# Kim-Dongjun/Soft-Truncation

Hardware: AMD Instinct MI355X
Metric: training images/sec (DDPM++ CIFAR-10 32x32) (higher is better)
Workload: dtype f32; 1 GPU; DDPM++ (VP) CIFAR-10 32x32, configs/vp/CIFAR10/ddpmpp_nll_st.py (BASELINE configs[1]); per_gpu_batch=128, global_batch=128, parallelism=dp1

## Files before the change

soft-truncation_amd/csrc/conv.hip:

```cpp
#include "igemm.h"
#include "stk_fp16.h"
#include "stk_fp16_train.h"

namespace {

using igemm::Cfg;
using igemm::MnMajor;
using igemm::keep_if;
using igemm::strip_row;

typedef __attribute__((address_space(1))) float gfloat;

struct ConvP {
  const float* x1; const float* x2; int C1, C2;
  const float* w; int w_layout;
  const float* bias; const float* temb; int temb_stride; const float* res; float inv_div; int use_div;
  float* y;
  const float* dy; float* dx1; float* dx2; float beta1, beta2, alpha;
  float* part; long part_stride;
  int N, H, W, Cin, Cout, OH, OW, KH, KW, stride, pad, sshift;
  int HW, OHW, taps;
  int ohw_shift, ow_shift;
};


template <int B, int KC, int LD>
struct RowChunk {
  static constexpr int PERQ = KC / 4, PASSES = B / 64, PER = PASSES * PERQ;
  static_assert(KC % 4 == 0 && B % 64 == 0 && PER <= 32, "bad RowChunk tile");
  const float* rowp[PASSES];
  unsigned rowbits;
  unsigned okm;
  int q, tid, Ktot;
  __device__ __forceinline__ void init(const float* base, long ld, int row0, int R, int Ktot_, int tid_) {
    tid = tid_; q = tid & 3; Ktot = Ktot_; rowbits = 0; okm = 0;
#pragma unroll
    for (int ps = 0; ps < PASSES; ++ps) {
      const int row = row0 + (tid >> 2) + 64 * ps;
      const bool ok = row < R;
      rowbits |= (ok ? 1u : 0u) << ps;
      rowp[ps] = base + (ok ? (long)row * ld : 0);
    }
  }
  __device__ __forceinline__ void load(int k0, float (&r)[PER]) {
    const int kb = k0 + q * PERQ;
    const bool kin = kb + PERQ <= Ktot;
    const int ko = kin ? kb : 0;
    okm = 0;
#pragma unroll
    for (int ps = 0; ps < PASSES; ++ps) {
      const float* s = rowp[ps] + ko;
#pragma unroll
      for (int j = 0; j < PERQ; ++j) r[ps * PERQ + j] = s[j];
      okm |= ((kin && ((rowbits >> ps) & 1u)) ? ((1u << PERQ) - 1u) : 0u) << (ps * PERQ);
    }
  }
  __device__ __forceinline__ void store(const float (&r)[PER], float* t) {
    if (okm == (PER == 32 ? 0xffffffffu : (1u << PER) - 1u)) {
#pragma unroll
      for (int ps = 0; ps < PASSES; ++ps)
#pragma unroll
        for (int j = 0; j < PERQ; ++j) t[(q * PERQ + j) * LD + (tid >> 2) + 64 * ps] = r[ps * PERQ + j];
    } else {
#pragma unroll
      for (int ps = 0; ps < PASSES; ++ps)
#pragma unroll
        for (int j = 0; j < PERQ; ++j)
          t[(q * PERQ + j) * LD + (tid >> 2) + 64 * ps] = keep_if(r[ps * PERQ + j], okm, ps * PERQ + j);
    }
  }
};

template <int B, int KC, int LD>
struct MnStrided {
  using Mp = MnMajor<B, KC>;
  static constexpr int PER = Mp::PER;
  const float* pm; long sk; int kg, tid, Ktot; bool ok;
  unsigned okm;
  __device__ __forceinline__ void init(const float* base, long smn, long sk_, int o0, int lim, int Ktot_, int tid_) {
    tid = tid_; sk = sk_; Ktot = Ktot_; okm = 0;
    const int mn = o0 + Mp::mn(tid);
    ok = mn < lim;
    pm = base + (ok ? (long)mn * smn : 0);
    kg = Mp::kgroup(tid) * PER;
  }
  __device__ __forceinline__ void load(int k0, float (&r)[PER]) {
    okm = 0;
#pragma unroll
    for (int i = 0; i < PER; ++i) {
      const int k = k0 + kg + i;
      const bool v = ok && k < Ktot;
      r[i] = pm[v ? (long)k * sk : 0];
      okm |= (v ? 1u : 0u) << i;
    }
  }
  __device__ __forceinline__ void store(const float (&r)[PER], float* t) {
#pragma unroll
    for (int i = 0; i < PER; ++i) t[(kg + i) * LD + Mp::mn(tid)] = keep_if(r[i], okm, i);
  }
};

template <class C>
struct AFwdK {
  RowChunk<C::BM, C::KC, C::LDA> rc;
  __device__ void init(const ConvP& p, int m0, int tid, int) { rc.init(p.w, (long)p.Cin * p.taps, m0, p.Cout, p.Cin * p.taps, tid); }
  __device__ void load(const ConvP&, int k0, float (&r)[C::NA]) { rc.load(k0, r); }
  __device__ void store(const float (&r)[C::NA], float* t) { rc.store(r, t); }
};
template <class C>
struct AFwdGen {
  MnStrided<C::BM, C::KC, C::LDA> ms;
  __device__ void init(const ConvP& p, int m0, int tid, int) { ms.init(p.w, (long)p.Cin * p.taps, 1, m0, p.Cout, p.Cin * p.taps, tid); }
  __device__ void load(const ConvP&, int k0, float (&r)[C::NA]) { ms.load(k0, r); }
  __device__ void store(const float (&r)[C::NA], float* t) { ms.store(r, t); }
};
template <class C>
struct AFwdNin {
  MnStrided<C::BM, C::KC, C::LDA> ms;
  __device__ void init(const ConvP& p, int m0, int tid, int) { ms.init(p.w, 1, p.Cout, m0, p.Cout, p.Cin, tid); }
  __device__ void load(const ConvP&, int k0, float (&r)[C::NA]) { ms.load(k0, r); }
  __device__ void store(const float (&r)[C::NA], float* t) { ms.store(r, t); }
};
template <class C>
struct ADgradNin {
  RowChunk<C::BM, C::KC, C::LDA> rc;
  __device__ void init(const ConvP& p, int m0, int tid, int) { rc.init(p.w, p.Cout, m0, p.Cin, p.Cout, tid); }
  __device__ void load(const ConvP&, int k0, float (&r)[C::NA]) { rc.load(k0, r); }
  __device__ void store(const float (&r)[C::NA], float* t) { rc.store(r, t); }
};
template <class C>
struct ADgradNinGen {
  MnStrided<C::BM, C::KC, C::LDA> ms;
  __device__ void init(const ConvP& p, int m0, int tid, int) { ms.init(p.w, p.Cout, 1, m0, p.Cin, p.Cout, tid); }
  __device__ void load(const ConvP&, int k0, float (&r)[C::NA]) { ms.load(k0, r); }
  __device__ void store(const float (&r)[C::NA], float* t) { ms.store(r, t); }
};
template <class C>
struct ADgrad1 {
  MnStrided<C::BM, C::KC, C::LDA> ms;
  __device__ void init(const ConvP& p, int m0, int tid, int) { ms.init(p.w, 1, p.Cin, m0, p.Cin, p.Cout, tid); }
  __device__ void load(const ConvP&, int k0, float (&r)[C::NA]) { ms.load(k0, r); }
  __device__ void store(const float (&r)[C::NA], float* t) { ms.store(r, t); }
};
template <class C>
struct ADgrad9 {
  static_assert(C::KC == 36, "3x3 chunks are 4 channels x 9 taps");
  static constexpr int PASSES = C::BM / 64;
  int m0, tid; unsigned okp;
  __device__ void init(const ConvP&, int m0_, int tid_, int) { m0 = m0_; tid = tid_; okp = 0; }
  __device__ void load(const ConvP& p, int k0, float (&r)[C::NA]) {
    const int co = k0 / 9 + (tid & 3);
    okp = 0;
#pragma unroll
    for (int ps = 0; ps < PASSES; ++ps) {
      const int m = m0 + (tid >> 2) + 64 * ps;
// ... 78 lines not shown
    cig = __builtin_amdgcn_readfirstlane(Mp::kgroup(tid) * (Mp::PER / TAPS));
    mask = 0; okm = 0; tb = 0; yp = 0; xp = 0;
    if (n < p.N * p.HW) {
      const int b = n / p.HW, hw = n - b * p.HW;
      const int y = hw / p.W, x = hw - y * p.W;
      yp = y + p.pad; xp = x + p.pad;
      const int KW = TAPS == 9 ? 3 : 1;
      const int sm = p.stride - 1;
#pragma unroll
      for (int t = 0; t < TAPS; ++t) {
        const int ty = yp - t / KW, tx = xp - t % KW;
        if (ty >= 0 && tx >= 0 && !(ty & sm) && !(tx & sm) && (ty >> p.sshift) < p.OH && (tx >> p.sshift) < p.OW)
          mask |= 1u << t;
      }
      tb = b * p.Cout * p.OHW;
    }
  }
  __device__ void load(const ConvP& p, int k0, float (&r)[C::NB]) {
    const int co0 = k0 / TAPS + cig;
    const int KW = TAPS == 9 ? 3 : 1;
    okm = 0;
#pragma unroll
    for (int c = 0; c < NCH; ++c) {
      const int co = co0 + c;
      const unsigned cm = co < p.Cout ? mask : 0u;
      const int cb = tb + co * p.OHW;
      okm |= cm << (c * TAPS);
#pragma unroll
      for (int t = 0; t < TAPS; ++t) {
        const int off = cb + ((yp - t / KW) >> p.sshift) * p.OW + ((xp - t % KW) >> p.sshift);
        r[c * TAPS + t] = p.dy[((cm >> t) & 1u) ? off : 0];
      }
    }
  }
  __device__ void store(const float (&r)[C::NB], float* t) {
    const int kg = Mp::kgroup(tid) * Mp::PER, mn = Mp::mn(tid);
#pragma unroll
    for (int i = 0; i < C::NB; ++i) t[(kg + i) * C::LDB + mn] = keep_if(r[i], okm, i);
  }
};

__device__ __forceinline__ void split_pixel(const ConvP& p, int k, int& b, int& ohw) {
  if (p.ohw_shift >= 0) { b = k >> p.ohw_shift; ohw = k & (p.OHW - 1); }
  else { b = k / p.OHW; ohw = k - b * p.OHW; }
}
__device__ __forceinline__ void split_row(const ConvP& p, int ohw, int& oy, int& ox) {
  if (p.ow_shift >= 0) { oy = ohw >> p.ow_shift; ox = ohw & (p.OW - 1); }
  else { oy = ohw / p.OW; ox = ohw - oy * p.OW; }
}

template <class C>
struct AWgrad {
  static_assert(C::KC == 32 && C::NA <= 32, "wgrad uses 32-pixel chunks");
  int roff[C::NA];
  int tid; unsigned okrows, okm;
  __device__ void init(const ConvP& p, int m0, int tid_, int) {
    tid = tid_; okm = 0; okrows = 0;
#pragma unroll
    for (int i = 0; i < C::NA; ++i) {
      const int m = m0 + (tid >> 5) + 8 * i;
      okrows |= (m < p.Cout ? 1u : 0u) << i;
      roff[i] = min(m, p.Cout - 1) * p.OHW;
    }
  }
  __device__ void load(const ConvP& p, int k0, float (&r)[C::NA]) {
    const int k = k0 + (tid & 31);
    const bool kv = k < p.N * p.OHW;
    int b, ohw;
    split_pixel(p, kv ? k : 0, b, ohw);
    const int base = b * p.Cout * p.OHW + ohw;
    okm = kv ? okrows : 0u;
#pragma unroll
    for (int i = 0; i < C::NA; ++i) r[i] = p.dy[base + roff[i]];
  }
  __device__ void store(const float (&r)[C::NA], float* t) {
#pragma unroll
    for (int i = 0; i < C::NA; ++i) t[(tid & 31) * C::LDA + (tid >> 5) + 8 * i] = keep_if(r[i], okm, i);
  }
};
template <class C, bool DUAL>
struct BWgrad {
  static_assert(C::KC == 32 && C::NB <= 32, "wgrad uses 32-pixel chunks");
  int roff[C::NB];
  int tid, kh, kw; unsigned okrows, okm, first;
  __device__ void init(const ConvP& p, int n0, int tid_, int zb) {
    tid = tid_; okm = 0; okrows = 0; first = 0;
    kh = zb / p.KW; kw = zb - kh * p.KW;
#pragma unroll
    for (int i = 0; i < C::NB; ++i) {
      const int ci = min(n0 + (tid >> 5) + 8 * i, p.Cin - 1);
      okrows |= (n0 + (tid >> 5) + 8 * i < p.Cin ? 1u : 0u) << i;
      const bool f = !DUAL || ci < p.C1;
      first |= (f ? 1u : 0u) << i;
      roff[i] = (f ? ci : ci - p.C1) * p.HW;
    }
  }
  __device__ void load(const ConvP& p, int k0, float (&r)[C::NB]) {
    const int k = k0 + (tid & 31);
    bool kv = k < p.N * p.OHW;
    int b, ohw, oy, ox;
    split_pixel(p, kv ? k : 0, b, ohw);
    split_row(p, ohw, oy, ox);
    const int iy = oy * p.stride + kh - p.pad, ix = ox * p.stride + kw - p.pad;
    kv = kv && iy >= 0 && iy < p.H && ix >= 0 && ix < p.W;
    const int pix = kv ? iy * p.W + ix : 0;
    const int b1 = b * p.C1 * p.HW + pix, b2 = b * p.C2 * p.HW + pix;
    okm = kv ? okrows : 0u;
#pragma unroll
    for (int i = 0; i < C::NB; ++i) {
      if (DUAL) {
        const bool f = (first >> i) & 1u;
        const uintptr_t tensor = f ? (uintptr_t)p.x1 : (uintptr_t)p.x2;
        r[i] = ((const gfloat*)tensor)[(f ? b1 : b2) + roff[i]];
      } else {
        r[i] = p.x1[b1 + roff[i]];
      }
    }
  }
  __device__ void store(const float (&r)[C::NB], float* t) {
#pragma unroll
    for (int i = 0; i < C::NB; ++i) t[(tid & 31) * C::LDB + (tid >> 5) + 8 * i] = keep_if(r[i], okm, i);
  }
};

struct EpFwd {
  int b; int col_off;
  static constexpr int TEMB_IMGS = 9;
  float rb; float rt[5]; int m0 = 0, b0 = 0, nimg = 0, tb = 0;
  const float* sb = nullptr; const float* stm = nullptr;
  __device__ void preload(const ConvP& p, int m0_, int n0, int tn, int M, int Nn, int tid) {
    m0 = m0_; sb = nullptr; stm = nullptr;
    b0 = n0 / p.OHW;
    nimg = min(n0 + tn - 1, Nn - 1) / p.OHW - b0 + 1;
    rb = (p.bias && tid < 128 && m0 + tid < M) ? p.bias[m0 + tid] : 0.f;
#pragma unroll
    for (int k = 0; k < 5; ++k) {
      const int idx = tid + 256 * k, img = idx >> 7, r = idx & 127;
      rt[k] = (p.temb && nimg <= TEMB_IMGS && img < nimg && m0 + r < M) ? p.temb[(long)(b0 + img) * p.temb_stride + m0 + r] : 0.f;
    }
  }
  __device__ void stage(unsigned char* lds, int tid) {
    __syncthreads();
    float* s = reinterpret_cast<float*>(lds);
    if (tid < 128) s[tid] = rb;
#pragma unroll
    for (int k = 0; k < 5; ++k) {
      const int idx = tid + 256 * k;
      if (idx < TEMB_IMGS * 128) s[128 + idx] = rt[k];
    }
    __syncthreads();
    sb = s; stm = s + 128;
  }
  __device__ void init(const ConvP&, int, int) {}
  __device__ void finish(const ConvP&, unsigned char*, int) {}
  __device__ void col(const ConvP& p, int n) {
    b = n / p.OHW;
    col_off = b * p.Cout * p.OHW + (n - b * p.OHW);
    tb = (b - b0) * 128;
  }
  __device__ void strip(const ConvP& p, int mbase, int M, bool nok, int, const floatx16& acc) {
    if (sb && (!p.temb || nimg <= TEMB_IMGS)) {
      const int ml = mbase - m0;
      float rv[16]; int idx[16];
#pragma unroll
      for (int e = 0; e < 16; ++e) {
        const int m = mbase + strip_row(e);
        const bool ok = nok && m < M;
        idx[e] = ok ? col_off + m * p.OHW : -1;
        rv[e] = (p.res && ok) ? p.res[idx[e]] : 0.f;
      }
#pragma unroll
      for (int g = 0; g < 4; ++g) {
        const float4 bb = *reinterpret_cast<const float4*>(sb + ml + 8 * g);
        const float4 tt = *reinterpret_cast<const float4*>(stm + tb + ml + 8 * g);
        const float bv[4] = {bb.x, bb.y, bb.z, bb.w}, tv[4] = {tt.x, tt.y, tt.z, tt.w};
#pragma unroll
        for (int u = 0; u < 4; ++u) {
          float v = acc[4 * g + u];
          if (p.bias) v += bv[u];
          if (p.temb) v += tv[u];
          if (p.res) v += rv[4 * g + u];
          if (p.use_div) v *= p.inv_div;
          if (idx[4 * g + u] >= 0) p.y[idx[4 * g + u]] = v;
        }
      }
      return;
    }
#pragma unroll
    for (int g = 0; g < 4; ++g) {
      float bv[4], tv[4], rv[4];
      int idx[4]; bool ok[4];
#pragma unroll
      for (int u = 0; u < 4; ++u) {
        const int m = mbase + strip_row(4 * g + u);
        ok[u] = nok && m < M;
        idx[u] = ok[u] ? col_off + m * p.OHW : 0;
        const int ms = ok[u] ? m : 0;
        bv[u] = p.bias ? p.bias[ms] : 0.f;
        tv[u] = p.temb ? p.temb[ok[u] ? (long)b * p.temb_stride + m : 0] : 0.f;
        rv[u] = p.res ? p.res[idx[u]] : 0.f;
      }
#pragma unroll
      for (int u = 0; u < 4; ++u) {
        float v = acc[4 * g + u];
        if (p.bias) v += bv[u];
        if (p.temb) v += tv[u];
        if (p.res) v += rv[u];
        if (p.use_div) v *= p.inv_div;
        if (ok[u]) p.y[idx[u]] = v;
      }
    }
  }
};
struct EpDgrad {
  int b, hw;
  __device__ void preload(const ConvP&, int, int, int, int, int, int) {}
  __device__ void stage(unsigned char*, int) {}
  __device__ void init(const ConvP&, int, int) {}
  __device__ void col(const ConvP& p, int n) { b = n / p.HW; hw = n - b * p.HW; }
  __device__ void strip(const ConvP& p, int mbase, int M, bool nok, int, const floatx16& acc) {
    const bool acc1 = p.beta1 != 0.f, acc2 = p.beta2 != 0.f;
#pragma unroll
    for (int e0 = 0; e0 < 16; e0 += 4) {
      float* d[4]; float old[4];
#pragma unroll
      for (int u = 0; u < 4; ++u) {
        const int m = mbase + strip_row(e0 + u);
        float* q = nullptr;
        if (nok && m < M) {
          if (m < p.C1) { if (p.dx1) q = p.dx1 + ((long)b * p.C1 + m) * p.HW + hw; }
          else if (p.dx2) q = p.dx2 + ((long)b * p.C2 + (m - p.C1)) * p.HW + hw;
        }
        d[u] = q;
        old[u] = 0.f;
        if (acc1 || acc2) {
          const float beta = m < p.C1 ? p.beta1 : p.beta2;
          if (q && beta != 0.f) old[u] = beta * *q;
        }
      }
#pragma unroll
      for (int u = 0; u < 4; ++u)
        if (d[u]) *d[u] = old[u] + p.alpha * acc[e0 + u];
    }
  }
  __device__ void finish(const ConvP&, unsigned char*, int) {}
};
struct EpWgrad {
  float* slab; int tap;
  __device__ void init(const ConvP& p, int zb, int zs) { slab = p.part + (long)zs * p.part_stride; tap = zb; }
  __device__ void col(const ConvP&, int) {}
  __device__ void strip(const ConvP& p, int mbase, int M, bool nok, int n, const floatx16& acc) {
#pragma unroll
    for (int e = 0; e < 16; ++e) {
      const int m = mbase + strip_row(e);
      if (nok && m < M) {
        slab[((long)tap * p.Cout + m) * p.Cin + n] = acc[e];
      }
    }
  }
};

struct EpSlab {
  float* slab; int Nn;
  __device__ void preload(const ConvP&, int, int, int, int, int, int) {}
  __device__ void stage(unsigned char*, int) {}
  __device__ void init(const ConvP& p, int, int zs) { slab = p.part + (long)zs * p.part_stride; Nn = p.N * p.HW; }
  __device__ void finish(const ConvP&, unsigned char*, int) {}
  __device__ void col(const ConvP&, int) {}
  __device__ void strip(const ConvP&, int mbase, int M, bool nok, int n, const floatx16& acc) {
#pragma unroll
    for (int e = 0; e < 16; ++e) {
      const int m = mbase + strip_row(e);
      if (nok && m < M) slab[(long)m * Nn + n] = acc[e];
    }
  }
};
template <class EP> struct OneProduct : EP {};
template <class EP> struct is_x1 { static constexpr bool value = false; };
template <class EP> struct is_x1<OneProduct<EP>> { static constexpr bool value = true; };
template <int VEC>
__global__ __launch_bounds__(256) void slab_fwd_kernel(ConvP p, int splits, int M, int Nn) {
  const long total = (long)M * Nn / VEC, gstride = (long)gridDim.x * 256;
  for (long iv = (long)blockIdx.x * 256 + threadIdx.x; iv < total; iv += gstride) {
    const long i = iv * VEC;
    const int m = (int)(i / Nn), n = (int)(i - (long)m * Nn);
    float v[VEC];
#pragma unroll
    for (int u = 0; u < VEC; ++u) v[u] = 0.f;
    for (int z = 0; z < splits; ++z) {
      const float* q = p.part + (long)z * p.part_stride + i;
      if constexpr (VEC == 4) {
        const float4 t = *reinterpret_cast<const float4*>(q);
        v[0] += t.x; v[1] += t.y; v[2] += t.z; v[3] += t.w;
      } else {
        v[0] += q[0];
      }
    }
    const int b = n / p.OHW;
    const long idx = ((long)b * p.Cout + m) * p.OHW + (n - b * p.OHW);
    float r[VEC];
#pragma unroll
    for (int u = 0; u < VEC; ++u) r[u] = 0.f;
    if (p.res) {
      if constexpr (VEC == 4) { const float4 t = *reinterpret_cast<const float4*>(p.res + idx); r[0] = t.x; r[1] = t.y; r[2] = t.z; r[3] = t.w; }
      else r[0] = p.res[idx];
    }
#pragma unroll
    for (int u = 0; u < VEC; ++u) {
      float w = v[u];
      if (p.bias) w += p.bias[m];
      if (p.temb) w += p.temb[(long)b * p.temb_stride + m];
      if (p.res) w += r[u];
      if (p.use_div) w *= p.inv_div;
      v[u] = w;
    }
    if constexpr (VEC == 4) *reinterpret_cast<float4*>(p.y + idx) = make_float4(v[0], v[1], v[2], v[3]);
    else p.y[idx] = v[0];
  }
}
template <int VEC>
__global__ __launch_bounds__(256) void slab_dgrad_kernel(ConvP p, int splits, int M, int Nn) {
  const long total = (long)M * Nn / VEC, gstride = (long)gridDim.x * 256;
  for (long iv = (long)blockIdx.x * 256 + threadIdx.x; iv < total; iv += gstride) {
    const long i = iv * VEC;
    const int m = (int)(i / Nn), n = (int)(i - (long)m * Nn);
    float v[VEC];
#pragma unroll
    for (int u = 0; u < VEC; ++u) v[u] = 0.f;
    for (int z = 0; z < splits; ++z) {
      const float* q = p.part + (long)z * p.part_stride + i;
      if constexpr (VEC == 4) {
        const float4 t = *reinterpret_cast<const float4*>(q);
        v[0] += t.x; v[1] += t.y; v[2] += t.z; v[3] += t.w;
      } else {
        v[0] += q[0];
      }
    }
    const int b = n / p.HW, hw = n - b * p.HW;
    float* d; float beta;
    if (m < p.C1) { d = p.dx1 ? p.dx1 + ((long)b * p.C1 + m) * p.HW + hw : nullptr; beta = p.beta1; }
    else { d = p.dx2 ? p.dx2 + ((long)b * p.C2 + (m - p.C1)) * p.HW + hw : nullptr; beta = p.beta2; }
    if (!d) continue;
    if constexpr (VEC == 4) {
      float4 o = make_float4(0.f, 0.f, 0.f, 0.f);
      if (beta != 0.f) { const float4 t = *reinterpret_cast<const float4*>(d); o = make_float4(beta * t.x, beta * t.y, beta * t.z, beta * t.w); }
      *reinterpret_cast<float4*>(d) = make_float4(o.x + p.alpha * v[0], o.y + p.alpha * v[1], o.z + p.alpha * v[2], o.w + p.alpha * v[3]);
    } else {
      *d = (beta != 0.f ? beta * *d : 0.f) + p.alpha * v[0];
    }
  }
}
inline void launch_slab_sum(const ConvP& p, int splits, int M, long Ng, int dgrad, hipStream_t s) {
  const bool al = stk_aligned16(p.part) && p.part_stride % 4 == 0 &&
                  (dgrad ? (p.HW % 4 == 0 && (!p.dx1 || stk_aligned16(p.dx1)) && (!p.dx2 || stk_aligned16(p.dx2)))
                         : (p.OHW % 4 == 0 && stk_aligned16(p.y) && (!p.res || stk_aligned16(p.res))));
  if (al && Ng % 4 == 0) {
    const dim3 rgrid((unsigned)stk_ew_grid((long)M * Ng / 4));
    if (dgrad) hipLaunchKernelGGL(slab_dgrad_kernel<4>, rgrid, dim3(256), 0, s, p, splits, M, (int)Ng);
    else hipLaunchKernelGGL(slab_fwd_kernel<4>, rgrid, dim3(256), 0, s, p, splits, M, (int)Ng);
  } else {
    const dim3 rgrid((unsigned)stk_ew_grid((long)M * Ng));
    if (dgrad) hipLaunchKernelGGL(slab_dgrad_kernel<1>, rgrid, dim3(256), 0, s, p, splits, M, (int)Ng);
    else hipLaunchKernelGGL(slab_fwd_kernel<1>, rgrid, dim3(256), 0, s, p, splits, M, (int)Ng);
  }
}

#include "conv_thin.h"
#include "conv_x2.h"
#include "conv_pl.h"
#include "conv_x2d.h"
#include "conv_x2w.h"

__device__ __forceinline__ long splitk_dst(long j, int layout, long CC, int Cout, int Cin, int taps) {
  if (layout == 0) {
    const int tap = (int)(j / CC);
    return (j - (long)tap * CC) * taps + tap;
  }
  const int co = (int)(j / Cin), ci = (int)(j - (long)co * Cin);
  return (long)ci * Cout + co;
}
__global__ __launch_bounds__(256) void splitk_reduce_kernel(const float* __restrict__ part, float* __restrict__ dw,
                                                            long n, int splits, long stride, float alpha, int layout,
                                                            int Cout, int Cin, int taps) {
  const long gstride = (long)gridDim.x * 256;
  const long CC = (long)Cout * Cin;
  const long n4 = ((n | stride) & 3) == 0 ? n / 4 : 0;
  for (long v = (long)blockIdx.x * 256 + threadIdx.x; v < n4; v += gstride) {
    const float4* src = reinterpret_cast<const float4*>(part) + v;
    float4 acc = {0.f, 0.f, 0.f, 0.f};
#pragma unroll 8
    for (int z = 0; z < splits; ++z) {
      const float4 t = src[(long)z * (stride / 4)];
      acc.x += t.x; acc.y += t.y; acc.z += t.z; acc.w += t.w;
    }
    const float a4[4] = {acc.x, acc.y, acc.z, acc.w};
#pragma unroll
    for (int e = 0; e < 4; ++e) dw[splitk_dst(4 * v + e, layout, CC, Cout, Cin, taps)] += alpha * a4[e];
  }
  for (long j = 4 * n4 + (long)blockIdx.x * 256 + threadIdx.x; j < n; j += gstride) {
    float sum = 0.f;
    for (int z = 0; z < splits; ++z) sum += part[(long)z * stride + j];
    dw[splitk_dst(j, layout, CC, Cout, Cin, taps)] += alpha * sum;
  }
}

__global__ __launch_bounds__(256) void splitk_reduce9_kernel(const float* __restrict__ part, float* __restrict__ dw, long CC,
                                                             int splits, long stride, float alpha) {
  __shared__ float s[256 * 9];
  const long q0 = (long)blockIdx.x * 256;
  const long q = q0 + threadIdx.x;
  const bool live = q < CC;
  float acc[9];
#pragma unroll
  for (int t = 0; t < 9; ++t) acc[t] = 0.f;
  const float* src = part + (live ? q : 0);
  int z = 0;
  for (; z + 4 <= splits; z += 4) {
    float v[4][9];
#pragma unroll
    for (int u = 0; u < 4; ++u)
// ... 159 lines not shown
  __device__ void load(const GemmP&, int k0, float (&r)[C::NB]) {
    if (K_CONTIG) rc.load(k0, r); else ms.load(k0, r);
  }
  __device__ void store(const float (&r)[C::NB], float* t) {
    if (K_CONTIG) rc.store(r, t); else ms.store(r, t);
  }
};
struct EpGemm {
  float* base;
  __device__ void init(const GemmP& p, int zb, int) { base = p.C + (long)zb * p.scb; }
  __device__ void col(const GemmP&, int) {}
  __device__ void strip(const GemmP& p, int mbase, int M, bool nok, int n, const floatx16& acc) {
    float old[16];
    if (p.beta != 0.f) {
#pragma unroll
      for (int e = 0; e < 16; ++e) {
        const int m = mbase + strip_row(e);
        const bool ok = nok && m < M;
        old[e] = base[ok ? (long)m * p.scm + (long)n * p.scn : 0];
      }
    }
#pragma unroll
    for (int e = 0; e < 16; ++e) {
      const int m = mbase + strip_row(e);
      if (nok && m < M) {
        float v = p.alpha * acc[e];
        if (p.bias_mode == 1) v += p.bias[m];
        else if (p.bias_mode == 2) v += p.bias[n];
        base[(long)m * p.scm + (long)n * p.scn] = (p.beta != 0.f ? p.beta * old[e] : 0.f) + v;
      }
    }
  }
};

inline bool use_big_tile(int M, long N, int z) {
  const long t = (long)stk_cdiv(M, 128) * stk_cdiv(N, 128) * z;
  return M >= 96 && N >= 96 && t >= 192;
}

template <class C, class P, class AL, class BL, class EP>
int launch(const P& p, int M, long Nl, int K, int k_per_split, int splits, int batch, hipStream_t s,
           bool flat = false) {
  if (Nl > 0x7fffffffL) return STK_EUNSUPPORTED;
  const int N = (int)Nl;
  const int tm = stk_cdiv(M, C::BM), tn = stk_cdiv(N, C::BN);
  if (flat) {
    const long total = (long)tm * tn * splits * batch;
    if (total > 0x7fffffffL) return STK_EUNSUPPORTED;
    hipLaunchKernelGGL((igemm::kernel<C, P, AL, BL, EP>), dim3((unsigned)total), dim3(256), 0, s, p, M, N, K, tm, tn,
                       k_per_split, batch);
  } else {
    dim3 grid((unsigned)(tm * tn), (unsigned)splits, (unsigned)batch);
    hipLaunchKernelGGL((igemm::kernel<C, P, AL, BL, EP>), grid, dim3(256), 0, s, p, M, N, K, tm, tn, k_per_split, 0);
  }
  STK_CHECK_LAUNCH();
  return STK_OK;
}

inline int fill_common(ConvP& p, int N, int H, int W, int C1, int C2, int Cout, int OH, int OW, int KH, int KW,
                       int stride, int pad) {
  if (N <= 0 || H <= 0 || W <= 0 || C1 <= 0 || C2 < 0 || Cout <= 0 || OH <= 0 || OW <= 0) return STK_EINVAL;
  if (!((KH == 3 && KW == 3) || (KH == 1 && KW == 1))) return STK_EUNSUPPORTED;
  if (stride != 1 && stride != 2) return STK_EUNSUPPORTED;
  const long lim = 0x7fffffffL;
  if ((long)N * (C1 > C2 ? C1 : C2) * H * W >= lim || (long)N * Cout * OH * OW >= lim) return STK_EUNSUPPORTED;
  p.N = N; p.H = H; p.W = W; p.C1 = C1; p.C2 = C2; p.Cin = C1 + C2; p.Cout = Cout; p.OH = OH; p.OW = OW;
  p.KH = KH; p.KW = KW; p.stride = stride; p.pad = pad; p.sshift = stride == 2 ? 1 : 0;
  p.HW = H * W; p.OHW = OH * OW; p.taps = KH * KW;
  p.ohw_shift = -1; p.ow_shift = -1;
  for (int sft = 0; sft < 31; ++sft) {
    if ((1 << sft) == p.OHW) p.ohw_shift = sft;
    if ((1 << sft) == p.OW) p.ow_shift = sft;
  }
  return STK_OK;
}

struct SplitPlan { int ok; int splits; int chunks_per_split; long slab; int t64; int gps; };
inline SplitPlan split_plan(const ConvP& p, int Kc, int S1, int S2, int M, long Ng) {
  SplitPlan r = {0, 1, 0, 0, 0, 0};
  const long big = (long)p.N * p.HW * 4 * (S1 > S2 ? S1 : S2);
  const bool geom = (p.taps == 9 && p.pad == 1) || (p.taps == 1 && p.pad == 0);
  if (!(big < 0x7fffffffL && geom && p.stride == 1 && p.OH == p.H && p.OW == p.W && Kc % 32 == 0 &&
        (S2 == 0 || S1 % 32 == 0) && M >= 96 && Ng <= 0x7fffffffL))
    return r;
  const long tiles = (long)stk_cdiv(M, 128) * stk_cdiv(Ng, 128);
  const int nch = p.taps * (Kc / 32);
  r.chunks_per_split = nch;
  if (tiles >= 192) { r.ok = 1; return r; }
  static const long target = [] { const char* e = getenv("STK_KSPLIT_WGS"); return e && atol(e) > 0 ? atol(e) : 512L; }();
  constexpr long minch = 12;
  long splits = target / tiles;
  const long mc = p.taps == 9 ? minch : (minch < 6 ? minch : 6);
  if (splits > nch / mc) splits = nch / mc;
  if ((tiles < 16 && p.taps != 9) || splits < 2) return r;
  r.chunks_per_split = (int)((nch + splits - 1) / splits);
  r.splits = (nch + r.chunks_per_split - 1) / r.chunks_per_split;
  r.slab = (long)M * Ng;
  r.ok = 1;
  return r;
}
inline SplitPlan fwd_split_plan(const ConvP& p) { return split_plan(p, p.Cin, p.C1, p.C2, p.Cout, (long)p.N * p.OHW); }
inline SplitPlan dgrad_split_plan(const ConvP& p) { return split_plan(p, p.Cout, p.Cout, 0, p.Cin, (long)p.N * p.HW); }
struct SplitWs { long xpart, part, bytes; };
inline long align256(long v) { return (v + 255) & ~255L; }
inline SplitWs split_ws(const SplitPlan& r, int M, int Kc, int taps) {
  SplitWs o;
  o.xpart = align256(x2::wp_bytes(M, Kc, taps));
  o.part = align256(o.xpart + 2L * x2::NPART * 4);
  o.bytes = r.ok ? 255 + o.part + (r.splits > 1 ? r.splits * r.slab * 4 : 0) : 0;
  return o;
}
inline void split_weight_strides(const ConvP& p, int dgrad, long& sm, long& sk) {
  if (p.w_layout == 0) { sm = dgrad ? p.taps : (long)p.Cin * p.taps; sk = dgrad ? (long)p.Cin * p.taps : p.taps; }
  else { sm = dgrad ? p.Cout : 1; sk = dgrad ? 1 : p.Cout; }
}
inline SplitPlan x1_plan(const SplitPlan& r, int nch1) {
  SplitPlan r1 = r;
  r1.chunks_per_split = (nch1 + r.splits - 1) / r.splits;
  r1.splits = (nch1 + r1.chunks_per_split - 1) / r1.chunks_per_split;
  return r1;
}

struct SplitGemm {
  ConvP p; x2::Src q; int M, Ng, tm, tn, nch, chunks_per_split; const float* xpart; int nx;
  bool dual, planes, halo; dim3 grid; hipStream_t s;
};
template <class E, int TAPS>
void split_gemm_taps(const SplitGemm& g) {
  constexpr bool X1 = is_x1<E>::value;
  if (!g.planes) {
    using A1 = std::conditional_t<X1, x2::ActLoader16<false, TAPS>, x2::ActLoader<false, TAPS>>;
    using A2 = std::conditional_t<X1, x2::ActLoader16<true, TAPS>, x2::ActLoader<true, TAPS>>;
    if (g.dual) hipLaunchKernelGGL((x2::gemm_kernel<A2, E>), g.grid, dim3(256), 0, g.s, g.p, g.q, g.M, g.Ng, g.tm, g.tn, g.nch,
                                   g.chunks_per_split, g.xpart, g.nx);
    else hipLaunchKernelGGL((x2::gemm_kernel<A1, E>), g.grid, dim3(256), 0, g.s, g.p, g.q, g.M, g.Ng, g.tm, g.tn, g.nch,
                            g.chunks_per_split, g.xpart, g.nx);
  } else if (g.halo) {
    if (g.p.W == 64)
      hipLaunchKernelGGL((x2d::gemm_halo_kernel<64, E, 1>), g.grid, dim3(256), 0, g.s, g.p, g.q, g.M, g.Ng, g.tm, g.tn, g.nch / 9, g.xpart, g.nx);
    else if (g.p.W == 32)
      hipLaunchKernelGGL((x2d::gemm_halo_kernel<32, E, 1>), g.grid, dim3(256), 0, g.s, g.p, g.q, g.M, g.Ng, g.tm, g.tn, g.nch / 9, g.xpart, g.nx);
    else
      hipLaunchKernelGGL((x2d::gemm_halo_kernel<16, E, 1>), g.grid, dim3(256), 0, g.s, g.p, g.q, g.M, g.Ng, g.tm, g.tn, g.nch / 9, g.xpart, g.nx);
  } else {
    hipLaunchKernelGGL((x2d::gemm_kernel<TAPS, 128, E>), g.grid, dim3(256), 0, g.s, g.p, g.q, g.M, g.Ng, g.tm, g.tn, g.nch,
                       g.chunks_per_split, g.xpart, g.nx);
  }
}
template <class E>
void split_gemm(const SplitGemm& g) {
  if (g.p.taps == 9) split_gemm_taps<E, 9>(g);
  else split_gemm_taps<E, 1>(g);
}

template <class EP>
int launch_split(ConvP p, const SplitPlan& r0, const float* s1, int S1, const float* s2, int S2, int M, long Ng, int dgrad,
                 void* ws, hipStream_t s, const void* wp_ready, float* amax, const void* planes, const float* planes_amax,
                 bool amax_valid, bool x1) {
  x2::Src q;
  q.s1 = s1; q.s2 = S2 > 0 ? s2 : s1; q.S1 = S1; q.S2 = S2; q.Kc = S1 + S2; q.Mpad = x2::pad128(M); q.taps = p.taps;
  q.pl = static_cast<const unsigned char*>(planes); q.pl_stride = planes ? pl::plane_bytes(p.N, S1, p.HW) : 0;
  const SplitWs lay = split_ws(r0, M, q.Kc, p.taps);
  unsigned char* base = reinterpret_cast<unsigned char*>(((uintptr_t)ws + 255) & ~(uintptr_t)255);
  float* xpart = reinterpret_cast<float*>(base + lay.xpart);
  p.part = reinterpret_cast<float*>(base + lay.part);
  p.part_stride = r0.slab;
  if (amax) xpart = amax + (dgrad ? 2 * x2::NPART : 0);
  if (planes) {
    xpart = const_cast<float*>(planes_amax);
  } else if (!(amax_valid && amax)) {
    hipLaunchKernelGGL(x2::amax_partial_kernel, dim3(x2::NPART), dim3(x2::AMAX_THREADS), 0, s, s1, (long)p.N * S1 * p.HW, xpart);
    if (S2 > 0)
      hipLaunchKernelGGL(x2::amax_partial_kernel, dim3(x2::NPART), dim3(x2::AMAX_THREADS), 0, s, s2, (long)p.N * S2 * p.HW,
                         xpart + x2::NPART);
    STK_CHECK_LAUNCH();
  }
  if (wp_ready) {
    q.wp = static_cast<const unsigned short*>(wp_ready);
  } else {
    x2::WprepDesc one = {};
    one.w = p.w; one.wp = base; one.M = M; one.Kc = q.Kc; one.Mpad = q.Mpad;
    one.taps = p.taps; one.flip = dgrad;
    split_weight_strides(p, dgrad, one.sm, one.sk);
    hipLaunchKernelGGL(x2::wamax_kernel, dim3(x2::WPART, 1), dim3(256), 0, s, nullptr, one);
    hipLaunchKernelGGL(x2::wprep_kernel, dim3((unsigned)stk_cdiv((long)q.Mpad * q.Kc, 256L)), dim3(256), 0, s, nullptr, one);
    STK_CHECK_LAUNCH();
    q.wp = reinterpret_cast<const unsigned short*>(base);
  }
  const int nch = planes && x1 ? p.taps * ((q.Kc / x2::KC + 1) / 2) : p.taps * (q.Kc / x2::KC);
  const SplitPlan r = planes && x1 ? x1_plan(r0, nch) : r0;
  SplitGemm g = {p, q, M, (int)Ng, q.Mpad / 128, stk_cdiv((int)Ng, 128), nch, r.chunks_per_split, xpart,
                 S2 > 0 ? 2 * x2::NPART : x2::NPART, S2 > 0, planes != nullptr, planes && x2d::halo_ok(p, p.taps, r0.splits),
                 dim3(), s};
  g.grid = dim3((unsigned)(g.tm * g.tn * r.splits));
  if (r0.splits == 1) {
    if (x1) split_gemm<OneProduct<EP>>(g);
    else split_gemm<EP>(g);
    STK_CHECK_LAUNCH();
    return STK_OK;
  }
  if (x1) split_gemm<OneProduct<EpSlab>>(g);
  else split_gemm<EpSlab>(g);
  STK_CHECK_LAUNCH();
  launch_slab_sum(p, r.splits, M, Ng, dgrad, s);
  STK_CHECK_LAUNCH();
  return STK_OK;
}

struct SplitWgradPlan { int ok; int splits; int chunks_per_split; long slab; int rows3; };
inline SplitWgradPlan split_wgrad_plan(int C1, int C2, int N, int Cout, int H, int W, int OH, int OW, int KH, int KW,
                                       int stride, int pad) {
  SplitWgradPlan q = {0, 0, 0, 0, 0};
  const int Cin = C1 + C2;
  const long K = (long)N * H * W;
  const int cmax = Cout > C1 ? (Cout > C2 ? Cout : C2) : (C1 > C2 ? C1 : C2);
  if (K * cmax * 4 >= 0x7fffffffL || (C2 > 0 && C1 % 32)) return q;
  const bool pow2 = (W & (W - 1)) == 0 && ((H * W) & (H * W - 1)) == 0;
  const bool geom = (KH == 3 && KW == 3 && pad == 1) || (KH == 1 && KW == 1 && pad == 0);
  if (!geom || stride != 1 || OH != H || OW != W || !pow2 || W < 4 || H * W < 16 || Cin < 64 || Cout < 64 ||
      K > 0x7fffffffL || K % 32)
    return q;
  const int taps = KH * KW;
  q.rows3 = (taps == 9 && W >= 8 && (C2 == 0 || C1 % 16 == 0)) ? 1 : 0;
  const long tiles = q.rows3 ? 3L * stk_cdiv(Cout, 128) * stk_cdiv(Cin, 64)
                             : (long)taps * stk_cdiv(Cout, 128) * stk_cdiv(Cin, 128);
  if (taps == 1 && tiles < 2) return q;
  const long chunks = K / 32;
  constexpr long w1_wgs = 256;
  long splits = (taps == 1 && tiles < 6 ? w1_wgs : 512) / tiles;
  if (splits > chunks / 8) splits = chunks / 8;
  if (splits < 1) splits = 1;
  q.chunks_per_split = (int)((chunks + splits - 1) / splits);
  q.splits = (int)((chunks + q.chunks_per_split - 1) / q.chunks_per_split);
  q.slab = (long)Cout * Cin * taps;
  q.ok = 1;
  return q;
}
template <int FORM>
void launch_x2w(const x2w::Args& a, int W, dim3 grid, hipStream_t s) {
  const dim3 block(256 * (FORM & 15));
  if (W >= 32) hipLaunchKernelGGL((x2w::wgrad_kernel<32, FORM>), grid, block, 0, s, a);
  else if (W == 16) hipLaunchKernelGGL((x2w::wgrad_kernel<16, FORM>), grid, block, 0, s, a);
  else if (W == 8) hipLaunchKernelGGL((x2w::wgrad_kernel<8, FORM>), grid, block, 0, s, a);
  else hipLaunchKernelGGL((x2w::wgrad_kernel<4, FORM>), grid, block, 0, s, a);
}
struct WgemmArgs {
  ConvP p; int tm, tn, nch, chunks_per_split; const float* dyp; const float* xp; int nx; dim3 grid; hipStream_t s;
};
template <bool X1, class BL>
void launch_wgemm_rows(const WgemmArgs& g) {
  using AL = std::conditional_t<X1, x2::RowsU16<false, false>, x2::RowsU<false, false>>;
  using E = std::conditional_t<X1, OneProduct<EpWgrad>, EpWgrad>;
  hipLaunchKernelGGL((x2::wgemm_kernel<AL, BL, E, !X1>), g.grid, dim3(256), 0, g.s, g.p, g.p.Cout, g.p.Cin, g.tm, g.tn, g.nch,
                     g.chunks_per_split, g.p.taps, g.dyp, g.xp, g.nx);
}
template <bool X1, bool DUAL>
void launch_wgemm_src(const WgemmArgs& g) {
  if (g.p.taps == 1)
    launch_wgemm_rows<X1, std::conditional_t<X1, x2::RowsU16<true, DUAL>, x2::RowsU<true, DUAL>>>(g);
  else if (g.p.W >= 16)
    launch_wgemm_rows<X1, std::conditional_t<X1, x2::RowsB16<DUAL, 16>, x2::RowsB<DUAL, 16>>>(g);
  else if (g.p.W == 8)
    launch_wgemm_rows<X1, std::conditional_t<X1, x2::RowsB16<DUAL, 8>, x2::RowsB<DUAL, 8>>>(g);
  else
    launch_wgemm_rows<X1, std::conditional_t<X1, x2::RowsB16<DUAL, 4>, x2::RowsB<DUAL, 4>>>(g);
}
template <bool X1>
void launch_wgemm(const WgemmArgs& g) {
  if (g.p.C2 > 0) launch_wgemm_src<X1, true>(g);
  else launch_wgemm_src<X1, false>(g);
}

struct WgradPlan { int big; int splits; int k_per_split; long slab; int mode9; };
inline int wgrad9_cols(int OH, int OW, int KH, int KW) {
  if (KH != 3 || KW != 3 || ((long)OH * OW) % 32 != 0) return 0;
  if (OW % 32 == 0) return 32;
  if (OW == 16 || OW == 8) return OW;
  return 0;
}
inline WgradPlan wgrad_plan(int Cin, int N, int Cout, int OH, int OW, int KH, int KW, bool allow9 = true) {
  WgradPlan q;
  q.mode9 = allow9 ? wgrad9_cols(OH, OW, KH, KW) : 0;
  if (q.mode9) {
    const long K = (long)N * OH * OW;
    const long tiles = (long)stk_cdiv(Cout, 128) * stk_cdiv(Cin, 32);
    const long chunks = K / 32;
    long splits = 256 / tiles;
    if (splits > chunks / 16) splits = chunks / 16;
    if (splits < 1) splits = 1;
    const long cps = (chunks + splits - 1) / splits;
    q.big = 1;
    q.k_per_split = (int)(cps * 32);
    q.splits = (int)((K + q.k_per_split - 1) / q.k_per_split);
    q.slab = (long)Cout * Cin * 9;
    return q;
  }
  const int taps = KH * KW;
  const long K = (long)N * OH * OW;
  const long tiles128 = (long)stk_cdiv(Cout, 128) * stk_cdiv(Cin, 128) * taps;
  q.big = (Cout >= 96 && Cin >= 96 && tiles128 >= 9) ? 1 : 0;
  const int T = q.big ? 128 : 64;
  const long tiles = (long)stk_cdiv(Cout, T) * stk_cdiv(Cin, T) * taps;
  const long chunks = (K + 31) / 32;
  long splits = (512 + tiles - 1) / tiles;
  if (splits > chunks / 16) splits = chunks / 16;
  if (splits < 1) splits = 1;
  const long cps = (chunks + splits - 1) / splits;
  q.k_per_split = (int)(cps * 32);
  q.splits = (int)((K + q.k_per_split - 1) / q.k_per_split);
  q.slab = (long)Cout * Cin * taps;
  return q;
}

}

extern "C" {

static int fwd_impl(const float* x1, int C1, const float* x2, int C2, const float* w, int w_layout,
                    const float* bias, const float* temb, int temb_stride, const float* res, float out_div,
                    float* y, int N, int H, int W, int Cout, int OH, int OW, int KH, int KW, int stride, int pad,
                    const void* wp, float* amax, void* ws, long ws_bytes, void* stream, bool x_rec_valid, bool f16x1) {
  if (!x1 || !w || !y || (C2 > 0 && !x2) || out_div == 0.f || (w_layout != 0 && w_layout != 1) ||
      (w_layout == 1 && (KH != 1 || KW != 1)))
    return STK_EINVAL;
  ConvP p = {};
  int rc = fill_common(p, N, H, W, C1, C2, Cout, OH, OW, KH, KW, stride, pad);
  if (rc) return rc;
  p.x1 = x1; p.x2 = C2 > 0 ? x2 : x1; p.w = w; p.w_layout = w_layout; p.bias = bias; p.temb = temb;
  p.temb_stride = temb_stride; p.res = res; p.inv_div = 1.f / out_div; p.use_div = out_div != 1.f; p.y = y;
  const int K = p.Cin * p.taps;
  const long Ng = (long)N * p.OHW;
  const bool big = use_big_tile(Cout, Ng, 1);
  hipStream_t s = (hipStream_t)stream;
  if (thin::geometry_ok(p) && Ng <= 0x7fffffffL) {
    const unsigned nblk = (unsigned)stk_cdiv(Ng, 256L);
    if (C2 == 0 && p.Cin <= 4) {
      thin::Args a = {x1, w, (long)p.Cin * p.taps, (long)p.taps, 0, p.Cin, Cout, p.taps, 0};
      const dim3 grid(nblk, (unsigned)stk_cdiv(Cout, thin::OB));
      if (p.taps == 9) hipLaunchKernelGGL((thin::thin_in_kernel<9>), grid, dim3(256), 0, s, p, a);
      else hipLaunchKernelGGL((thin::thin_in_kernel<1>), grid, dim3(256), 0, s, p, a);
      STK_CHECK_LAUNCH();
      return STK_OK;
    }
    if (Cout <= 4) {
      const unsigned nblk64 = (unsigned)stk_cdiv(Ng, 64L);
      if (p.taps == 9) hipLaunchKernelGGL((thin::thin_out_kernel<9>), dim3(nblk64), dim3(256), 0, s, p, Cout);
      else hipLaunchKernelGGL((thin::thin_out_kernel<1>), dim3(nblk64), dim3(256), 0, s, p, Cout);
      STK_CHECK_LAUNCH();
// ... 174 lines not shown
    if (p.taps == 9) {
      if (a.CT == 3) hipLaunchKernelGGL((thin::thin_wgrad_kernel<9, 3>), grid, dim3(256), 0, s, p, a);
      else hipLaunchKernelGGL((thin::thin_wgrad_kernel<9, 4>), grid, dim3(256), 0, s, p, a);
    } else {
      hipLaunchKernelGGL((thin::thin_wgrad_kernel<1, 4>), grid, dim3(256), 0, s, p, a);
    }
    STK_CHECK_LAUNCH();
    hipLaunchKernelGGL(splitk_reduce_kernel, dim3(stk_ew_grid((a.slab + 3) / 4)), dim3(256), 0, s, ws, dw, a.slab, S, a.slab,
                       alpha, 0, Cout, p.Cin, p.taps);
    STK_CHECK_LAUNCH();
    return STK_OK;
  }
  const SplitWgradPlan xq = split_wgrad_plan(C1, C2, N, Cout, H, W, OH, OW, KH, KW, stride, pad);
  if (xq.ok && ws_bytes >= (long)xq.splits * xq.slab * 4 + 256 + 3L * x2::NPART * 4) {
    p.x1 = x1; p.x2 = C2 > 0 ? x2 : x1; p.dy = dy; p.w_layout = w_layout; p.part = ws; p.part_stride = xq.slab;
    float* parts = reinterpret_cast<float*>(((uintptr_t)(ws + (long)xq.splits * xq.slab) + 255) & ~(uintptr_t)255);
    const dim3 ab(x2::NPART), at(x2::AMAX_THREADS);
    const float* dyp = parts;
    const float* xp = parts + x2::NPART;
    if (amax && (have & 2)) dyp = amax + 2 * x2::NPART;
    else hipLaunchKernelGGL(x2::amax_partial_kernel, ab, at, 0, s, dy, (long)N * Cout * p.OHW, parts);
    if (amax && (have & 1)) {
      xp = amax;
    } else {
      hipLaunchKernelGGL(x2::amax_partial_kernel, ab, at, 0, s, x1, (long)N * C1 * p.HW, parts + x2::NPART);
      if (C2 > 0) hipLaunchKernelGGL(x2::amax_partial_kernel, ab, at, 0, s, x2, (long)N * C2 * p.HW, parts + 2 * x2::NPART);
    }
    const int nx = C2 > 0 ? 2 * x2::NPART : x2::NPART;
    const int tm = stk_cdiv(Cout, 128), nch = (int)((long)N * p.HW / 32);
    if (xq.rows3 && !f16x1) {
      const int tn64 = stk_cdiv(p.Cin, 64);
      const dim3 grid3((unsigned)(3 * tm * tn64 * xq.splits));
      if (C2 > 0) hipLaunchKernelGGL((x2::wgrad3_kernel<true>), grid3, dim3(256), 0, s, p, tm, tn64, nch, xq.chunks_per_split,
                                     dyp, xp, nx);
      else hipLaunchKernelGGL((x2::wgrad3_kernel<false>), grid3, dim3(256), 0, s, p, tm, tn64, nch, xq.chunks_per_split,
                              dyp, xp, nx);
    } else {
      const int tn = stk_cdiv(p.Cin, 128);
      const WgemmArgs g = {p, tm, tn, nch, xq.chunks_per_split, dyp, xp, nx, dim3((unsigned)(p.taps * tm * tn * xq.splits)), s};
      if (f16x1) launch_wgemm<true>(g);
      else launch_wgemm<false>(g);
    }
    STK_CHECK_LAUNCH();
    hipLaunchKernelGGL(splitk_reduce_kernel, dim3(stk_ew_grid((xq.slab + 3) / 4)), dim3(256), 0, s, ws, dw, xq.slab, xq.splits,
                       xq.slab, alpha, w_layout, Cout, p.Cin, p.taps);
    STK_CHECK_LAUNCH();
    return STK_OK;
  }
  const bool can9 = stride == 1 && pad == 1 && C2 == 0 && OH == H && OW == W && w_layout == 0;
  const WgradPlan q = wgrad_plan(p.Cin, N, Cout, OH, OW, KH, KW, can9);
  if (ws_bytes < (long)q.splits * q.slab * 4) return STK_EINVAL;
  p.x1 = x1; p.x2 = C2 > 0 ? x2 : x1; p.dy = dy; p.w_layout = w_layout; p.part = ws; p.part_stride = q.slab;
  const long Kl = (long)N * p.OHW;
  if (Kl > 0x7fffffffL) return STK_EUNSUPPORTED;
  const int K = (int)Kl;
  using CB = Cfg<128, 128, 32>; using CS = Cfg<64, 64, 32>;
  if (q.mode9) {
    const int tm = stk_cdiv(Cout, 128), tn = stk_cdiv(p.Cin, 32);
    const dim3 grid((unsigned)(tm * tn * q.splits));
    if (q.mode9 == 32) hipLaunchKernelGGL((wgrad9_kernel<32>), grid, dim3(256), 0, s, p, tm, tn, q.k_per_split);
    else if (q.mode9 == 16) hipLaunchKernelGGL((wgrad9_kernel<16>), grid, dim3(256), 0, s, p, tm, tn, q.k_per_split);
    else hipLaunchKernelGGL((wgrad9_kernel<8>), grid, dim3(256), 0, s, p, tm, tn, q.k_per_split);
    STK_CHECK_LAUNCH();
    rc = STK_OK;
  } else if (C2 > 0) {
    if (q.big) rc = launch<CB, ConvP, AWgrad<CB>, BWgrad<CB, true>, EpWgrad>(p, Cout, p.Cin, K, q.k_per_split, q.splits, p.taps, s, true);
    else rc = launch<CS, ConvP, AWgrad<CS>, BWgrad<CS, true>, EpWgrad>(p, Cout, p.Cin, K, q.k_per_split, q.splits, p.taps, s, true);
  } else {
    if (q.big) rc = launch<CB, ConvP, AWgrad<CB>, BWgrad<CB, false>, EpWgrad>(p, Cout, p.Cin, K, q.k_per_split, q.splits, p.taps, s, true);
    else rc = launch<CS, ConvP, AWgrad<CS>, BWgrad<CS, false>, EpWgrad>(p, Cout, p.Cin, K, q.k_per_split, q.splits, p.taps, s, true);
  }
  if (rc) return rc;
  hipLaunchKernelGGL(splitk_reduce_kernel, dim3(stk_ew_grid((q.slab + 3) / 4)), dim3(256), 0, s, ws, dw, q.slab, q.splits,
                     q.slab, alpha, w_layout, Cout, p.Cin, p.taps);
  STK_CHECK_LAUNCH();
  return STK_OK;
}

int stk_conv2d_wgrad_f32(const float* x1, int C1, const float* x2, int C2, const float* dy, float* dw, int w_layout,
                         float alpha, float* ws, long ws_bytes, int N, int H, int W, int Cout, int OH, int OW, int KH,
                         int KW, int stride, int pad, void* stream) {
  return stk_conv2d_wgrad_amax_f32(x1, C1, x2, C2, dy, dw, w_layout, alpha, ws, ws_bytes, N, H, W, Cout, OH, OW, KH, KW, stride,
                                   pad, nullptr, 0, stream);
}

int stk_conv2d_wgrad_amax_f32(const float* x1, int C1, const float* x2, int C2, const float* dy, float* dw, int w_layout,
                              float alpha, float* ws, long ws_bytes, int N, int H, int W, int Cout, int OH, int OW, int KH,
                              int KW, int stride, int pad, const float* amax, int have, void* stream) {
  return wgrad_amax_impl(x1, C1, x2, C2, dy, dw, w_layout, alpha, ws, ws_bytes, N, H, W, Cout, OH, OW, KH, KW, stride, pad, amax,
                         have, stream, false);
}

int stk_conv2d_wgrad_amax_f16x1(const float* x1, int C1, const float* x2, int C2, const float* dy, float* dw, int w_layout,
                                float alpha, float* ws, long ws_bytes, int N, int H, int W, int Cout, int OH, int OW, int KH,
                                int KW, int stride, int pad, const float* amax, int have, void* stream) {
  return wgrad_amax_impl(x1, C1, x2, C2, dy, dw, w_layout, alpha, ws, ws_bytes, N, H, W, Cout, OH, OW, KH, KW, stride, pad, amax,
                         have, stream, true);
}

long stk_planes_bytes(int N, int C, int HW) {
  if (N <= 0 || C <= 0 || HW <= 0) return 0;
  return 2 * pl::plane_bytes(N, C, HW);
}

int stk_amax_partial_f32(const float* x, long n, float* part, void* stream) {
  if (!x || !part || n <= 0) return STK_EINVAL;
  hipLaunchKernelGGL(x2::amax_partial_kernel, dim3(x2::NPART), dim3(x2::AMAX_THREADS), 0, (hipStream_t)stream, x, n, part);
  STK_CHECK_LAUNCH();
  return STK_OK;
}

int stk_split_planes_f32(const float* x, int N, int C, int HW, const float* amax, int namax, void* planes, void* stream) {
  if (!x || !amax || !planes || N <= 0 || C <= 0 || HW <= 0 || namax <= 0) return STK_EINVAL;
  if (2 * pl::plane_bytes(N, C, HW) >= 0x7fffffffL) return STK_EUNSUPPORTED;
  const long blocks = (long)N * ((C + 31) / 32) * stk_cdiv(HW, pl::SP_PIX);
  hipLaunchKernelGGL(pl::split_planes_kernel, dim3((unsigned)blocks), dim3(256), 0, (hipStream_t)stream, x, N, C, HW, amax,
                     namax, static_cast<unsigned char*>(planes), pl::plane_bytes(N, C, HW));
  STK_CHECK_LAUNCH();
  return STK_OK;
}

int stk_conv2d_pl_ok(int dir, int C1, int C2, int N, int H, int W, int Cout, int KH, int KW, int stride, int pad) {
  ConvP p = {};
  if (fill_common(p, N, H, W, C1, C2, Cout, H, W, KH, KW, stride, pad)) return 0;
  if (stride != 1 || pad != KH / 2) return 0;
  if (dir == 0) {
    if (C2 > 0 || p.Cin <= 4 || Cout <= 4) return 0;
    return fwd_split_plan(p).ok;
  }
  if (dir == 1) {
    if (Cout <= 4 || p.Cin <= 4) return 0;
    return dgrad_split_plan(p).ok;
  }
  return 0;
}

int stk_conv2d_pl_ksplit(int dir, int C1, int C2, int N, int H, int W, int Cout, int KH, int KW) {
  if (!stk_conv2d_pl_ok(dir, C1, C2, N, H, W, Cout, KH, KW, 1, KH / 2)) return 0;
  ConvP p = {};
  if (fill_common(p, N, H, W, C1, C2, Cout, H, W, KH, KW, 1, KH / 2)) return 0;
  return dir == 0 ? fwd_split_plan(p).splits : dgrad_split_plan(p).splits;
}

int stk_conv2d_pl_halo(int dir, int C1, int C2, int N, int H, int W, int Cout, int KH, int KW) {
  const int ks = stk_conv2d_pl_ksplit(dir, C1, C2, N, H, W, Cout, KH, KW);
  if (ks <= 0) return 0;
  ConvP p = {};
  if (fill_common(p, N, H, W, C1, C2, Cout, H, W, KH, KW, 1, KH / 2)) return 0;
  return x2d::halo_ok(p, p.taps, ks) ? x2d::halo_cols(W) : 0;
}

static int fwd_pl_impl(const void* xpl, const float* xamax, int C, const float* w, int w_layout, const float* bias,
                       const float* temb, int temb_stride, const float* res, float out_div, float* y, int N, int H,
                       int W, int Cout, int KH, int KW, const void* wp, void* ws, long ws_bytes, void* stream, bool f16x1) {
  if (!xpl || !xamax || !w || !y || out_div == 0.f || (w_layout != 0 && w_layout != 1) || (w_layout == 1 && KH != 1))
    return STK_EINVAL;
  if (!stk_conv2d_pl_ok(0, C, 0, N, H, W, Cout, KH, KW, 1, KH / 2)) return STK_EUNSUPPORTED;
  ConvP p = {};
  fill_common(p, N, H, W, C, 0, Cout, H, W, KH, KW, 1, KH / 2);
  p.w = w; p.w_layout = w_layout; p.bias = bias; p.temb = temb; p.temb_stride = temb_stride; p.res = res;
  p.inv_div = 1.f / out_div; p.use_div = out_div != 1.f; p.y = y;
  const long Ng = (long)N * p.HW;
  const SplitPlan xr = fwd_split_plan(p);
  if (!ws || ws_bytes < split_ws(xr, Cout, C, p.taps).bytes) return STK_EINVAL;
  return launch_split<EpFwd>(p, xr, nullptr, C, nullptr, 0, Cout, Ng, 0, ws, (hipStream_t)stream, wp, nullptr, xpl, xamax, false,
                             f16x1);
}

int stk_conv2d_fwd_pl_f32(const void* xpl, const float* xamax, int C, const float* w, int w_layout, const float* bias,
                          const float* temb, int temb_stride, const float* res, float out_div, float* y, int N, int H,
                          int W, int Cout, int KH, int KW, const void* wp, void* ws, long ws_bytes, void* stream) {
  return fwd_pl_impl(xpl, xamax, C, w, w_layout, bias, temb, temb_stride, res, out_div, y, N, H, W, Cout, KH, KW, wp, ws,
                     ws_bytes, stream, false);
}

int stk_conv2d_fwd_pl_f16x1(const void* xpl, const float* xamax, int C, const float* w, int w_layout, const float* bias,
                            const float* temb, int temb_stride, const float* res, float out_div, float* y, int N, int H,
                            int W, int Cout, int KH, int KW, const void* wp, void* ws, long ws_bytes, void* stream) {
  return fwd_pl_impl(xpl, xamax, C, w, w_layout, bias, temb, temb_stride, res, out_div, y, N, H, W, Cout, KH, KW, wp, ws,
                     ws_bytes, stream, true);
}

static int dgrad_pl_impl(const void* dypl, const float* dyamax, const float* w, int w_layout, float* dx1, int C1,
                         float beta1, float* dx2, int C2, float beta2, float alpha, int N, int H, int W, int Cout,
                         int KH, int KW, const void* wp, void* ws, long ws_bytes, void* stream, bool f16x1) {
  if (!dypl || !dyamax || !w || (!dx1 && !dx2) || (w_layout != 0 && w_layout != 1) || (w_layout == 1 && KH != 1))
    return STK_EINVAL;
  if (!stk_conv2d_pl_ok(1, C1, C2, N, H, W, Cout, KH, KW, 1, KH / 2)) return STK_EUNSUPPORTED;
  ConvP p = {};
  fill_common(p, N, H, W, C1, C2, Cout, H, W, KH, KW, 1, KH / 2);
  p.w = w; p.w_layout = w_layout; p.dx1 = dx1; p.dx2 = C2 > 0 ? dx2 : nullptr;
  p.beta1 = beta1; p.beta2 = beta2; p.alpha = alpha;
  const long Ng = (long)N * p.HW;
  const SplitPlan xr = dgrad_split_plan(p);
  if (!ws || ws_bytes < split_ws(xr, p.Cin, Cout, p.taps).bytes) return STK_EINVAL;
  return launch_split<EpDgrad>(p, xr, nullptr, Cout, nullptr, 0, p.Cin, Ng, 1, ws, (hipStream_t)stream, wp, nullptr, dypl, dyamax,
                               false, f16x1);
}

int stk_conv2d_dgrad_pl_f32(const void* dypl, const float* dyamax, const float* w, int w_layout, float* dx1, int C1,
                            float beta1, float* dx2, int C2, float beta2, float alpha, int N, int H, int W, int Cout,
                            int KH, int KW, const void* wp, void* ws, long ws_bytes, void* stream) {
  return dgrad_pl_impl(dypl, dyamax, w, w_layout, dx1, C1, beta1, dx2, C2, beta2, alpha, N, H, W, Cout, KH, KW, wp, ws, ws_bytes,
                       stream, false);
}

int stk_conv2d_dgrad_pl_f16x1(const void* dypl, const float* dyamax, const float* w, int w_layout, float* dx1, int C1,
                              float beta1, float* dx2, int C2, float beta2, float alpha, int N, int H, int W, int Cout,
                              int KH, int KW, const void* wp, void* ws, long ws_bytes, void* stream) {
  return dgrad_pl_impl(dypl, dyamax, w, w_layout, dx1, C1, beta1, dx2, C2, beta2, alpha, N, H, W, Cout, KH, KW, wp, ws, ws_bytes,
                       stream, true);
}

int stk_conv2d_wgrad_pl_ok(int N, int H, int W, int Cin, int Cout) { return x2w::plan(N, H, W, Cin, Cout).ok; }

long stk_conv2d_wgrad_pl_ws_bytes(int N, int H, int W, int Cin, int Cout) {
  long m = 0;
  for (int wgs : {0, 256, 512, 768, 1024}) {
    const x2w::Plan q = x2w::plan(N, H, W, Cin, Cout, wgs);
    if (q.ok && (long)q.splits * q.slab > m) m = (long)q.splits * q.slab;
  }
  return m ? m * 4 + 256 : 0;
}

static int wgrad_pl_impl(const void* xpl, const float* xrec, const void* dypl, const float* dyrec, float* dw, float alpha,
                         float* ws, long ws_bytes, int N, int H, int W, int Cin, int Cout, int wgs, void* stream, bool f16x1) {
  if (!xpl || !xrec || !dypl || !dyrec || !dw || !ws || wgs < 0 || wgs > 1024) return STK_EINVAL;
  const x2w::Plan q = x2w::plan(N, H, W, Cin, Cout, wgs);
  if (!q.ok) return STK_EUNSUPPORTED;
  if (ws_bytes < (long)q.splits * q.slab * 4) return STK_EINVAL;
  x2w::Args a = {};
  a.dypl = static_cast<const unsigned char*>(dypl); a.dyrec = dyrec; a.dy_ps = pl::plane_bytes(N, Cout, H * W);
  a.xpl = static_cast<const unsigned char*>(xpl); a.xrec = xrec; a.x_ps = pl::plane_bytes(N, Cin, H * W);
  if (2 * a.dy_ps >= 0x7fffffffL || 2 * a.x_ps >= 0x7fffffffL) return STK_EUNSUPPORTED;
  a.part = ws; a.part_stride = q.slab;
  a.N = N; a.H = H; a.W = W; a.HW = H * W; a.Cin = Cin; a.Cout = Cout; a.Cob = Cout / 32; a.Cib = Cin / 32;
  a.tiles_co = stk_cdiv(Cout, 128); a.tiles_ci = Cin / 32;
  a.nchunks_total = (int)((long)N * H * W / 32); a.chunks_per_split = q.chunks_per_split;
  hipStream_t s = (hipStream_t)stream;
  const dim3 grid((unsigned)(a.tiles_co * a.tiles_ci * q.splits));
  if (f16x1) {
    if (q.groups == 2) launch_x2w<2 | x2w::X1_FORM>(a, W, grid, s);
    else launch_x2w<1 | x2w::X1_FORM>(a, W, grid, s);
  } else if (q.groups == 2) {
    launch_x2w<2>(a, W, grid, s);
  } else {
    launch_x2w<1>(a, W, grid, s);
  }
  STK_CHECK_LAUNCH();
  if (q.splits <= 64)
    hipLaunchKernelGGL(splitk_reduce9_kernel, dim3((unsigned)stk_cdiv((long)Cout * Cin, 256L)), dim3(256), 0, s, ws, dw, (long)Cout * Cin,
                       q.splits, q.slab, alpha);
  else
    hipLaunchKernelGGL(splitk_reduce_kernel, dim3(stk_ew_grid((q.slab + 3) / 4)), dim3(256), 0, s, ws, dw, q.slab, q.splits,
                       q.slab, alpha, 0, Cout, Cin, 9);
  STK_CHECK_LAUNCH();
  return STK_OK;
}

int stk_conv2d_wgrad_pl_f32(const void* xpl, const float* xrec, const void* dypl, const float* dyrec, float* dw,
                            float alpha, float* ws, long ws_bytes, int N, int H, int W, int Cin, int Cout, void* stream) {
  return stk_conv2d_wgrad_pl_wgs_f32(xpl, xrec, dypl, dyrec, dw, alpha, ws, ws_bytes, N, H, W, Cin, Cout, 0, stream);
}

int stk_conv2d_wgrad_pl_wgs_f32(const void* xpl, const float* xrec, const void* dypl, const float* dyrec, float* dw,
                                float alpha, float* ws, long ws_bytes, int N, int H, int W, int Cin, int Cout, int wgs, void* stream) {
  return wgrad_pl_impl(xpl, xrec, dypl, dyrec, dw, alpha, ws, ws_bytes, N, H, W, Cin, Cout, wgs, stream, false);
}

int stk_conv2d_wgrad_pl_f16x1(const void* xpl, const float* xrec, const void* dypl, const float* dyrec, float* dw,
                              float alpha, float* ws, long ws_bytes, int N, int H, int W, int Cin, int Cout, void* stream) {
  return wgrad_pl_impl(xpl, xrec, dypl, dyrec, dw, alpha, ws, ws_bytes, N, H, W, Cin, Cout, 0, stream, true);
}

int stk_conv2d_wgrad_pl_wgs_f16x1(const void* xpl, const float* xrec, const void* dypl, const float* dyrec, float* dw,
                                  float alpha, float* ws, long ws_bytes, int N, int H, int W, int Cin, int Cout, int wgs,
                                  void* stream) {
  return wgrad_pl_impl(xpl, xrec, dypl, dyrec, dw, alpha, ws, ws_bytes, N, H, W, Cin, Cout, wgs, stream, true);
}

int stk_conv2d_variant(int dir, int C1, int C2, int N, int H, int W, int Cout, int OH, int OW, int KH, int KW,
                       int stride, int pad, int w_layout) {
  ConvP p = {};
  if (fill_common(p, N, H, W, C1, C2, Cout, OH, OW, KH, KW, stride, pad)) return -1;
  const int Cin = C1 + C2;
  p.w_layout = w_layout;
  if (dir == 0) {
    const long Ng = (long)N * p.OHW;
    if (thin::geometry_ok(p) && ((C2 == 0 && Cin <= 4) || Cout <= 4)) return 4;
    if (fwd_split_plan(p).ok) return 5;
    return use_big_tile(Cout, Ng, 1) && !(p.taps == 1 && w_layout == 0 && (Cin % 8)) ? 1 : 0;
  }
  if (dir == 1) {
    const long Ng = (long)N * p.HW;
    if (thin::geometry_ok(p) && Cout <= 4) return 4;
    if (dgrad_split_plan(p).ok) return 5;
    return use_big_tile(Cin, Ng, 1) && !(p.taps == 1 && w_layout == 1 && (Cout % 8)) ? 1 : 0;
  }
  if (thin::geometry_ok(p) && ((C2 == 0 && Cin <= 4) || Cout <= 4)) return 4;
  if (split_wgrad_plan(C1, C2, N, Cout, H, W, OH, OW, KH, KW, stride, pad).ok) return 5;
  const bool can9 = stride == 1 && pad == 1 && C2 == 0 && OH == H && OW == W && w_layout == 0;
  const WgradPlan q = wgrad_plan(Cin, N, Cout, OH, OW, KH, KW, can9);
  return q.mode9 ? 3 : q.big;
}

long stk_conv2d_wp_bytes(int dir, int C1, int C2, int N, int H, int W, int Cout, int KH, int KW, int stride, int pad) {
  if (dir != 0 && dir != 1) return 0;
  if (stk_conv2d_variant(dir, C1, C2, N, H, W, Cout, H, W, KH, KW, stride, pad, 0) != 5) return 0;
  const int Cin = C1 + C2;
  return dir == 0 ? x2::wp_bytes(Cout, Cin, KH * KW) : x2::wp_bytes(Cin, Cout, KH * KW);
}

long stk_conv2d_wp_desc(int dir, const float* w, int w_layout, int Cin, int Cout, int KH, int KW, void* wp,
                        StkWprepDesc* out) {
  if (!w || !wp || !out || (dir != 0 && dir != 1) || (w_layout != 0 && w_layout != 1) || Cin <= 0 || Cout <= 0 ||
      (KH * KW != 9 && KH * KW != 1) || (w_layout == 1 && KH * KW != 1) || ((uintptr_t)wp & 255))
    return STK_EINVAL;
  ConvP p = {};
  p.Cin = Cin; p.Cout = Cout; p.taps = KH * KW; p.w_layout = w_layout;
// ... 72 lines not shown
```

soft-truncation_amd/csrc/conv_x2d.h:

```cpp
#pragma once

namespace x2d {

using x2::KC;
typedef __attribute__((address_space(3))) void lds_void;

template <int TN>
struct Geo {
  static constexpr int A_PLANE = 128 * 64, A_BYTES = 2 * A_PLANE;
  static constexpr int B_PLANE = TN * 64, B_BYTES = 2 * B_PLANE;
  static constexpr int LDS = A_BYTES + B_BYTES;
  static constexpr int NJ = TN / 64;
  static constexpr int BBLK = TN / 64;
};

__device__ __forceinline__ void dma16(__amdgpu_buffer_rsrc_t rs, unsigned char* dst, unsigned voff, unsigned soff) {
  __builtin_amdgcn_raw_ptr_buffer_load_lds(rs, (lds_void*)dst, 16, (int)voff, (int)soff, 0, 0);
}

template <int TAPS, int TN, class EP, int NBUF = 1, int ABL = 0>
__global__ __launch_bounds__(256, 2) void gemm_kernel(ConvP p, x2::Src q, int M, int Nn, int tiles_m, int tiles_n,
                                                      int nchunks_total, int chunks_per_split,
                                                      const float* __restrict__ xpart, int nxpart) {
  using G = Geo<TN>;
// ... 11 lines not shown
  const int id = xcd_remap(blockIdx.x, gridDim.x);
  const int tile = id % ntiles, zs = id / ntiles;
  const int tm = tile % tiles_m, tn = tile / tiles_m;
  const int m0 = tm * 128, n0 = tn * TN;
  const int c_begin = zs * chunks_per_split;
  const int c_last = min(nchunks_total, c_begin + chunks_per_split) - 1;

  const unsigned seg_src = (unsigned)((lane & 3) ^ ((lane >> 4) & 3)) * 16u;
  const unsigned a_plane2 = (unsigned)q.taps * q.Mpad * q.Kc * 2u;
  const unsigned a_chunk2 = (unsigned)q.Mpad * KC * 2u;
  const __amdgpu_buffer_rsrc_t a_rs = x2::make_rsrc(reinterpret_cast<const unsigned char*>(q.wp) + x2::HEADER, 2L * a_plane2);
  const unsigned a_voff = (unsigned)(m0 + 32 * wid + (lane >> 2)) * 64u + seg_src;
  const __amdgpu_buffer_rsrc_t b_rs = x2::make_rsrc(q.pl, 2L * q.pl_stride);
  const unsigned b_ps = (unsigned)q.pl_stride;
  const int Cb = q.Kc >> 5;
  unsigned b_base[G::BBLK], b_mask[G::BBLK];
  {
#pragma unroll
    for (int jb = 0; jb < G::BBLK; ++jb) {
      const int n = n0 + (TN / 4) * wid + 16 * jb + (lane >> 2);
      b_mask[jb] = 0; b_base[jb] = 0;
      if (n < Nn) {
        const int b = n / p.HW, hw = n - b * p.HW;
        const int y = hw / p.W, x = hw - y * p.W;
        if (TAPS == 1) b_mask[jb] = 1u;
#pragma unroll
        for (int t = 0; t < (TAPS == 9 ? 9 : 0); ++t) {
          const int iy = y + t / 3 - 1, ix = x + t % 3 - 1;
          if (iy >= 0 && iy < p.H && ix >= 0 && ix < p.W) b_mask[jb] |= 1u << t;
        }
        b_base[jb] = ((unsigned)(b * Cb) * p.HW + hw) * 64u + seg_src;
      }
    }
  }
  auto stage = [&](int c, int buf = 0) {
    const int cc = TAPS == 9 ? c / 9 : c, tap = c - cc * TAPS;
    const unsigned a_soff = (unsigned)c * a_chunk2;
    unsigned char* const As = lds + buf * G::LDS;
    unsigned char* const Bs = As + G::A_BYTES;
    if (X1) {
#pragma unroll
      for (int s = 0; s < 2; ++s) {
        const unsigned dead = (2 * cc + s >= Cb) ? 0x80000000u : 0u;
#pragma unroll
        for (int h = 0; h < 2; ++h)
          dma16(a_rs, As + s * G::A_PLANE + (32 * wid + 16 * h) * 64, (a_voff + h * 1024u) | dead,
                (unsigned)((2 * cc + s) * TAPS + tap) * a_chunk2);
      }
    } else if (!(ABL & 2) || c == c_begin) {
#pragma unroll
    for (int s = 0; s < 2; ++s)
#pragma unroll
      for (int h = 0; h < 2; ++h)
        dma16(a_rs, As + s * G::A_PLANE + (32 * wid + 16 * h) * 64, a_voff + h * 1024u, a_soff + s * a_plane2);
    }
    const int shift = TAPS == 9 ? ((tap / 3 - 1) * p.W + (tap % 3 - 1)) * 64 : 0;
    const unsigned b_soff = (unsigned)cc * (unsigned)p.HW * 64u;
    if ((ABL & 1) && tap != 0) return;
#pragma unroll
    for (int jb = 0; jb < G::BBLK; ++jb) {
      const unsigned dead = (((b_mask[jb] >> tap) & 1u) ^ 1u) << 31;
      const unsigned vo = (b_base[jb] + (unsigned)shift) | dead;
#pragma unroll
      for (int s = 0; s < 2; ++s) {
        if (X1)
          dma16(b_rs, Bs + s * G::B_PLANE + ((TN / 4) * wid + 16 * jb) * 64, vo | (2 * cc + s >= Cb ? 0x80000000u : 0u),
                (unsigned)(2 * cc + s) * (unsigned)p.HW * 64u);
        else
          dma16(b_rs, Bs + s * G::B_PLANE + ((TN / 4) * wid + 16 * jb) * 64, vo, b_soff + s * b_ps);
      }
    }
  };

  EP ep;
  ep.preload(p, m0, n0, TN, M, Nn, tid);

  floatx16 acc[2][G::NJ];
#pragma unroll
  for (int i = 0; i < 2; ++i)
#pragma unroll
    for (int j = 0; j < G::NJ; ++j)
#pragma unroll
      for (int e = 0; e < 16; ++e) acc[i][j][e] = 0.f;

  const int wm0 = (wid & 1) * 64, wn0 = (wid >> 1) * (TN / 2);
  const int fk = lane >> 5, fc = lane & 31;
  const int fsw = (fc >> 2) & 3;
  const unsigned char* a_rd = As + (wm0 + fc) * 64;
  const unsigned char* b_rd = Bs + (wn0 + fc) * 64;
  const int ko0 = ((0 + fk) ^ fsw) * 16, ko1 = ((2 + fk) ^ fsw) * 16;

#define STK_D_FRAGS_AT(KO, OFF)                                                                           \
  _Pragma("unroll") for (int s = 0; s < 2; ++s) {                                                          \
    _Pragma("unroll") for (int i = 0; i < 2; ++i)                                                           \
      a[i][s] = *reinterpret_cast<const halfx8*>(a_rd + (OFF) + s * G::A_PLANE + i * 32 * 64 + (KO));      \
    _Pragma("unroll") for (int j = 0; j < G::NJ; ++j)                                                       \
      b[j][s] = *reinterpret_cast<const halfx8*>(b_rd + (OFF) + s * G::B_PLANE + j * 32 * 64 + (KO));      \
  }
#define STK_D_FRAGS(KO) STK_D_FRAGS_AT(KO, 0)
  constexpr int SA[3] = {1, 0, 0}, SB[3] = {0, 1, 0};
  constexpr int NPR = X1 ? 2 : 3;
#define STK_D_MFMAS                                                                                        \
  _Pragma("unroll") for (int pr = 0; pr < NPR; ++pr) _Pragma("unroll") for (int i = 0; i < 2; ++i)           \
    _Pragma("unroll") for (int j = 0; j < G::NJ; ++j) {                                                     \
      acc[i][j] = __builtin_amdgcn_mfma_f32_32x32x16_f16(a[i][X1 ? pr : SA[pr]], b[j][X1 ? pr : SB[pr]], acc[i][j], 0, 0, 0); \
    }

  halfx8 a[2][2], b[G::NJ][2];
  stage(c_begin);
  if constexpr (NBUF == 2) {
    int cur = 0;
    for (int c = c_begin; c <= c_last; ++c) {
      asm volatile("s_waitcnt vmcnt(0)" ::: "memory");
      __syncthreads();
      if (c < c_last) stage(c + 1, cur ^ 1);
      const int off = cur * G::LDS;
      STK_D_FRAGS_AT(ko0, off)
      STK_D_MFMAS
      STK_D_FRAGS_AT(ko1, off)
      STK_D_MFMAS
      cur ^= 1;
    }
  } else {
    for (int c = c_begin; c <= c_last; ++c) {
      asm volatile("s_waitcnt vmcnt(0)" ::: "memory");
      __syncthreads();
      if (!(ABL & 4) || c == c_begin) { STK_D_FRAGS(ko0) }
      STK_D_MFMAS
      if (!(ABL & 4) || c == c_begin) { STK_D_FRAGS(ko1) }
      __syncthreads();
      if (c < c_last) stage(c + 1);
      STK_D_MFMAS
    }
  }
#undef STK_D_MFMAS
#undef STK_D_FRAGS
#undef STK_D_FRAGS_AT

  const float unscale = 1.f / (sw * x2::pow2_scale_of(xmax.reduce(red_amax, tid)));
  ep.stage(lds, tid);
  ep.init(p, 0, zs);
#pragma unroll
  for (int j = 0; j < G::NJ; ++j) {
    const int n = n0 + wn0 + j * 32 + fc;
    const bool nok = n < Nn;
    ep.col(p, nok ? n : 0);
#pragma unroll
    for (int i = 0; i < 2; ++i) {
#pragma unroll
      for (int e = 0; e < 16; ++e) acc[i][j][e] *= unscale;
      ep.strip(p, m0 + wm0 + i * 32 + 4 * fk, M, nok, nok ? n : 0, acc[i][j]);
    }
  }
  ep.finish(p, lds, tid);
}

template <int W, class EP, int NB>
__global__ __launch_bounds__(256, 2) void gemm_halo_kernel(ConvP p, x2::Src q, int M, int Nn, int tiles_m, int tiles_n,
                                                           int ngroups, const float* __restrict__ xpart, int nxpart) {
  constexpr int TN = 128, R = TN / W, TP = W + 2, HR = (R + 2) * TP, NI = (HR + 15) / 16, HRP = NI * 16;
  constexpr bool X1 = is_x1<EP>::value;
  constexpr int A_PLANE = 128 * 64, A_BYTES = 2 * A_PLANE, B_PLANE = HRP * 64, B_BYTES = 2 * B_PLANE;
  constexpr int NK = (NI + 3) / 4;
  static_assert(NB == 1 || 2 * NK <= 8, "the B pieces of a group are issued one per chunk over taps 0..7");
  __shared__ __attribute__((aligned(1024))) unsigned char lds[A_BYTES + NB * B_BYTES];
  unsigned char* const As = lds;
  unsigned char* const Bs = lds + A_BYTES;
  const int tid = threadIdx.x;
  const int lane = tid & 63, wid = __builtin_amdgcn_readfirstlane(tid >> 6);
  __shared__ float red_amax[4];
  x2::LateAmax xmax;
  xmax.load(xpart, nxpart, threadIdx.x);
  const float sw = x2::weight_scale(q.wp);
  const int ntiles = tiles_m * tiles_n;
  const int id = xcd_remap(blockIdx.x, gridDim.x);
  const int tile = id % ntiles;
  const int tm = tile % tiles_m, tn = tile / tiles_m;
  const int m0 = tm * 128, n0 = tn * TN;
  const int nchunks = 9 * ngroups;

  const unsigned seg_src = (unsigned)((lane & 3) ^ ((lane >> 4) & 3)) * 16u;
  const unsigned a_plane2 = (unsigned)q.taps * q.Mpad * q.Kc * 2u;
  const unsigned a_chunk2 = (unsigned)q.Mpad * KC * 2u;
  const __amdgpu_buffer_rsrc_t a_rs = x2::make_rsrc(reinterpret_cast<const unsigned char*>(q.wp) + x2::HEADER, 2L * a_plane2);
  const unsigned a_voff = (unsigned)(m0 + 32 * wid + (lane >> 2)) * 64u + seg_src;
  const __amdgpu_buffer_rsrc_t b_rs = x2::make_rsrc(q.pl, 2L * q.pl_stride);
  const unsigned b_ps = (unsigned)q.pl_stride;
  const int Cb = q.Kc >> 5;
  unsigned b_voff[NK];
  {
    const int b = n0 / p.HW, hw0 = n0 - b * p.HW, y0 = hw0 / p.W, x0 = hw0 - y0 * p.W;
#pragma unroll
    for (int k = 0; k < NK; ++k) {
      const int row = 16 * (wid + 4 * k) + (lane >> 2);
      const int ty = row / TP, tx = row - ty * TP;
      const int y = y0 - 1 + ty, x = x0 + tx - 1;
      const bool ok = row < HR && y >= 0 && y < p.H && x >= 0 && x < p.W;
      b_voff[k] = ok ? ((unsigned)(b * Cb) * p.HW + (unsigned)(y * p.W + x)) * 64u + seg_src : 0x80000000u;
    }
  }
  auto stage_a = [&](int c) {
    if (X1) {
      const int cc = c / 9, tap = c - 9 * cc;
#pragma unroll
      for (int s = 0; s < 2; ++s) {
        const unsigned dead = (2 * cc + s >= Cb) ? 0x80000000u : 0u;
#pragma unroll
        for (int h = 0; h < 2; ++h)
          dma16(a_rs, As + s * A_PLANE + (32 * wid + 16 * h) * 64, (a_voff + h * 1024u) | dead,
                (unsigned)((2 * cc + s) * 9 + tap) * a_chunk2);
      }
      return;
    }
    const unsigned a_soff = (unsigned)c * a_chunk2;
#pragma unroll
    for (int s = 0; s < 2; ++s)
#pragma unroll
      for (int h = 0; h < 2; ++h)
        dma16(a_rs, As + s * A_PLANE + (32 * wid + 16 * h) * 64, a_voff + h * 1024u, a_soff + s * a_plane2);
  };
  auto stage_b = [&](int cc, int buf, int k, int s) {
    if (wid + 4 * k >= NI) return;
    if (X1) {
      dma16(b_rs, Bs + buf * B_BYTES + s * B_PLANE + (wid + 4 * k) * 1024, b_voff[k] | (2 * cc + s >= Cb ? 0x80000000u : 0u),
            (unsigned)(2 * cc + s) * (unsigned)p.HW * 64u);
      return;
    }
    dma16(b_rs, Bs + buf * B_BYTES + s * B_PLANE + (wid + 4 * k) * 1024, b_voff[k],
          (unsigned)cc * (unsigned)p.HW * 64u + s * b_ps);
  };

  EP ep;
  ep.preload(p, m0, n0, TN, M, Nn, tid);

  floatx16 acc[2][2];
#pragma unroll
  for (int i = 0; i < 2; ++i)
#pragma unroll
    for (int j = 0; j < 2; ++j)
#pragma unroll
      for (int e = 0; e < 16; ++e) acc[i][j][e] = 0.f;

  const int wm0 = (wid & 1) * 64, wn0 = (wid >> 1) * 64;
  const int fk = lane >> 5, fc = lane & 31;
  const int fsw = (fc >> 2) & 3;
  const unsigned char* a_rd = As + (wm0 + fc) * 64;
  const int ka0 = ((0 + fk) ^ fsw) * 16, ka1 = ((2 + fk) ^ fsw) * 16;
  int b_row[2];
#pragma unroll
  for (int j = 0; j < 2; ++j) {
    const int pt = wn0 + 32 * j + fc;
    b_row[j] = (pt / W + 1) * TP + (pt % W) + 1;
  }

  halfx8 a[2][2], b[2][2];
  constexpr int SA[3] = {1, 0, 0}, SB[3] = {0, 1, 0};
  constexpr int NPR = X1 ? 2 : 3;
#define STK_H_MFMAS                                                                                        \
  _Pragma("unroll") for (int pr = 0; pr < NPR; ++pr) _Pragma("unroll") for (int i = 0; i < 2; ++i)           \
    _Pragma("unroll") for (int j = 0; j < 2; ++j) {                                                         \
      acc[i][j] = __builtin_amdgcn_mfma_f32_32x32x16_f16(a[i][X1 ? pr : SA[pr]], b[j][X1 ? pr : SB[pr]], acc[i][j], 0, 0, 0); \
    }
#define STK_H_FRAGS(KA, KSEG)                                                                              \
  _Pragma("unroll") for (int s = 0; s < 2; ++s) {                                                          \
    _Pragma("unroll") for (int i = 0; i < 2; ++i)                                                           \
      a[i][s] = *reinterpret_cast<const halfx8*>(a_rd + s * A_PLANE + i * 32 * 64 + (KA));                 \
    _Pragma("unroll") for (int j = 0; j < 2; ++j)                                                           \
      b[j][s] = *reinterpret_cast<const halfx8*>(bbase + s * B_PLANE + brow[j] * 64 + ((((KSEG) + fk) ^ (brow[j] >> 2)) & 3) * 16); \
  }

#pragma unroll
  for (int k = 0; k < NK; ++k)
#pragma unroll
    for (int s = 0; s < 2; ++s) stage_b(0, 0, k, s);
  stage_a(0);
  int c = 0;
  for (int cc = 0; cc < ngroups; ++cc) {
    const unsigned char* bbase = Bs + (NB == 2 ? (cc & 1) * B_BYTES : 0);
    const bool more = cc + 1 < ngroups;
#pragma unroll
    for (int tap = 0; tap < 9; ++tap, ++c) {
      const int toff = (tap / 3 - 1) * TP + (tap % 3 - 1);
      int brow[2] = {b_row[0] + toff, b_row[1] + toff};
      asm volatile("s_waitcnt vmcnt(0)" ::: "memory");
      __syncthreads();
      STK_H_FRAGS(ka0, 0)
      STK_H_MFMAS
      STK_H_FRAGS(ka1, 2)
      __syncthreads();
      if (c + 1 < nchunks) stage_a(c + 1);
      if (NB == 2) {
        if (tap < 2 * NK && more) stage_b(cc + 1, (cc + 1) & 1, tap >> 1, tap & 1);
      } else if (tap == 8 && more) {
#pragma unroll
        for (int k = 0; k < NK; ++k)
#pragma unroll
          for (int s = 0; s < 2; ++s) stage_b(cc + 1, 0, k, s);
      }
      STK_H_MFMAS
    }
  }
#undef STK_H_MFMAS
#undef STK_H_FRAGS

  const float unscale = 1.f / (sw * x2::pow2_scale_of(xmax.reduce(red_amax, tid)));
  ep.stage(lds, tid);
  ep.init(p, 0, 0);
#pragma unroll
  for (int j = 0; j < 2; ++j) {
    const int n = n0 + wn0 + j * 32 + fc;
    ep.col(p, n);
#pragma unroll
    for (int i = 0; i < 2; ++i) {
#pragma unroll
      for (int e = 0; e < 16; ++e) acc[i][j][e] *= unscale;
      ep.strip(p, m0 + wm0 + i * 32 + 4 * fk, M, true, n, acc[i][j]);
    }
  }
  ep.finish(p, lds, tid);
}

inline int halo_cols(int W) { return (W == 16 || W == 32 || W == 64) ? W : 0; }
inline bool halo_ok(const ConvP& p, int taps, int splits) {
  return taps == 9 && splits == 1 && halo_cols(p.W) != 0 && p.HW % 128 == 0 && p.H * p.W == p.HW;
}

}
```

soft-truncation_amd/csrc/groupnorm.hip:

```cpp
#include "common.h"

namespace {

struct GnArgs {
  const float* x1; const float* x2;
  int C1, C2;
  const float* gamma; const float* beta;
  int N, HW, G, cpg;
  int act; float drop_p; float keep_scale; unsigned drop_thr;
  unsigned long long seed; const unsigned long long* seed_dev;
};

struct GnBwdOut {
  float* sum; float* temb; int temb_stride; float scale; float* amax;
  const float* add; float add_scale;
};

struct Seg {
  const float* p; int len; int c_first;
};
__device__ __forceinline__ void group_segments(const GnArgs& a, int n, int g, Seg (&s)[2]) {
  const int c0 = g * a.cpg, c1 = c0 + a.cpg;
  const int e1 = min(c1, a.C1);
  if (c0 < a.C1) {
    s[0].p = a.x1 + ((long)n * a.C1 + c0) * a.HW;
    s[0].len = (e1 - c0) * a.HW;
    s[0].c_first = c0;
  } else {
    s[0].p = nullptr; s[0].len = 0; s[0].c_first = c0;
  }
  const int b2 = max(c0, a.C1);
  if (c1 > a.C1) {
    s[1].p = a.x2 + ((long)n * a.C2 + (b2 - a.C1)) * a.HW;
    s[1].len = (c1 - b2) * a.HW;
    s[1].c_first = b2;
  } else {
    s[1].p = nullptr; s[1].len = 0; s[1].c_first = c1;
  }
}

__device__ __forceinline__ float silu_f(float u) {
#ifdef STK_SILU_LIBM
  return u / (1.f + expf(-u));
#else
  const float NL2E_HI = -1.44269502162933349609375f, NL2E_LO = -1.925963033500011e-8f;
  const float t = u * NL2E_HI;
  float r = __fmaf_rn(u, NL2E_HI, -t);
  r = __fmaf_rn(u, NL2E_LO, r);
  const float p = __builtin_amdgcn_exp2f(t);
  const float e = fminf(__fmaf_rn(p, r * 0.693147182464599609375f, p), 3.0e38f);
  const float d = 1.f + e;
  float rc = __builtin_amdgcn_rcpf(d);
  rc = __fmaf_rn(rc, __fmaf_rn(-d, rc, 1.f), rc);
  const float q = u * rc;
  return __fmaf_rn(__fmaf_rn(-q, d, u), rc, q);
#endif
}

__device__ __forceinline__ float sigmoid_f(float u) {
#ifdef STK_SILU_LIBM
  return 1.f / (1.f + expf(-u));
#else
  const float NL2E_HI = -1.44269502162933349609375f, NL2E_LO = -1.925963033500011e-8f;
  const float t = u * NL2E_HI;
  float r = __fmaf_rn(u, NL2E_HI, -t);
  r = __fmaf_rn(u, NL2E_LO, r);
  const float p = __builtin_amdgcn_exp2f(t);
  const float e = fminf(__fmaf_rn(p, r * 0.693147182464599609375f, p), 3.0e38f);
  const float d = 1.f + e;
  float rc = __builtin_amdgcn_rcpf(d);
  return __fmaf_rn(rc, __fmaf_rn(-d, rc, 1.f), rc);
#endif
}

__device__ __forceinline__ float act_f(int act, float u) {
  if (act == STK_ACT_SILU) return silu_f(u);
  if (act == STK_ACT_RELU) return u > 0.f ? u : 0.f;
  if (act == STK_ACT_LRELU) return u > 0.f ? u : 0.2f * u;
  if (act == STK_ACT_ELU) return u > 0.f ? u : expm1f(u);
  return u;
}
__device__ __forceinline__ float act_slope_f(int act, float u) {
  if (act == STK_ACT_SILU) { const float sg = sigmoid_f(u); return sg * (1.f + u * (1.f - sg)); }
  if (act == STK_ACT_RELU) return u > 0.f ? 1.f : 0.f;
  if (act == STK_ACT_LRELU) return u > 0.f ? 1.f : 0.2f;
  if (act == STK_ACT_ELU) return u > 0.f ? 1.f : expf(u);
  return 1.f;
}

template <int IPT>
__global__ __launch_bounds__(1024) void gn_fwd_flat_kernel(GnArgs a, float* __restrict__ y, float* __restrict__ mean_out,
                                                           float* __restrict__ rstd_out, float eps) {
  __shared__ float red[32];
  const int ng = blockIdx.x;
  const int n = ng / a.G, g = ng - n * a.G;
  Seg seg[2];
  group_segments(a, n, g, seg);
  const int L = a.cpg * a.HW, L4 = L >> 2, n0 = seg[0].len >> 2;
  const float shift = seg[0].len ? seg[0].p[0] : seg[1].p[0];
  const float4* p0 = reinterpret_cast<const float4*>(seg[0].p);
  const float4* p1 = reinterpret_cast<const float4*>(seg[1].p);
  float4 v[IPT];
  float s[2] = {0.f, 0.f};
#pragma unroll
  for (int k = 0; k < IPT; ++k) {
    const int idx = threadIdx.x + k * blockDim.x;
    v[k] = make_float4(shift, shift, shift, shift);
    if (idx < L4) v[k] = idx < n0 ? p0[idx] : p1[idx - n0];
    const float d0 = v[k].x - shift, d1 = v[k].y - shift, d2 = v[k].z - shift, d3 = v[k].w - shift;
    s[0] += (d0 + d1) + (d2 + d3);
    s[1] += (d0 * d0 + d1 * d1) + (d2 * d2 + d3 * d3);
  }
  block_sum<2>(s, red);
  const float inv_l = 1.f / (float)L;
  const float md = s[0] * inv_l;
  const float var = fmaxf(s[1] * inv_l - md * md, 0.f);
  const float mean = shift + md;
  const float rstd = 1.f / sqrtf(var + eps);
  if (threadIdx.x == 0) {
    mean_out[ng] = mean;
    rstd_out[ng] = rstd;
  }
  unsigned long long seed = a.seed;
  if (a.drop_p > 0.f && a.seed_dev) seed += *a.seed_dev;
  const int C = a.C1 + a.C2;
#pragma unroll
  for (int k = 0; k < IPT; ++k) {
    const int idx = threadIdx.x + k * blockDim.x;
    if (idx >= L4) continue;
    const int q = idx < n0 ? 0 : 1, i = idx < n0 ? idx : idx - n0;
    const int c_first = q ? seg[1].c_first : seg[0].c_first;
    float4* o4 = reinterpret_cast<float4*>(y + ((long)n * C + c_first) * a.HW);
    const unsigned long long flat0 = ((unsigned long long)n * C + c_first) * a.HW;
    const int c = c_first + (i * 4) / a.HW;
    const float ga = a.gamma[c], be = a.beta[c];
    float r[4] = {v[k].x, v[k].y, v[k].z, v[k].w};
#pragma unroll
    for (int j = 0; j < 4; ++j) {
      float u = ga * ((r[j] - mean) * rstd) + be;
      float t = a.act ? act_f(a.act, u) : u;
      if (a.drop_p > 0.f) t = stk_drop_field(stk_mix64(seed, (flat0 + (unsigned long long)(i * 4)) >> 2), j) >= a.drop_thr ? t * a.keep_scale : 0.f;
      r[j] = t;
    }
    o4[i] = make_float4(r[0], r[1], r[2], r[3]);
  }
}

template <int VEC>
__global__ __launch_bounds__(256) void gn_fwd_kernel(GnArgs a, float* __restrict__ y, float* __restrict__ mean_out,
                                                     float* __restrict__ rstd_out, float eps) {
  __shared__ float red[16];
  const int ng = blockIdx.x;
  const int n = ng / a.G, g = ng - n * a.G;
// ... 532 lines not shown
#pragma unroll
    for (int k = 0; k < PASSES; ++k)
#pragma unroll
      for (int j = 0; j < 8; ++j) m = fmaxf(m, fabsf(v[k][j]));
    m = wave_max(m);
    if (lane == 0) xm[wave] = m;
  }
  __syncthreads();
  if (xmax1 && tid == 0) {
    float m = 0.f;
    for (int w = 0; w < nw; ++w) m = fmaxf(m, xm[w]);
    float* rec = c0 < a.C1 ? xmax1 : xmax2;
    if (rec) atomicMax(reinterpret_cast<unsigned*>(rec) + (blockIdx.x & 255), __float_as_uint(m));
  }
  if (tid < gb) {
    float s0 = 0.f, s1 = 0.f;
    for (int qq = 0; qq < 4; ++qq)
      for (int h = 0; h < 2; ++h)
        if ((8 * qq + 4 * h) / a.cpg == tid)
          for (int w = 0; w < nw; ++w) { s0 += red[(w * 4 + qq) * 4 + 2 * h]; s1 += red[(w * 4 + qq) * 4 + 2 * h + 1]; }
    const float inv_l = 1.f / ((float)a.cpg * (float)a.HW);
    const float shift = src[(long)(tid * a.cpg) * a.HW];
    const float md = s0 * inv_l;
    const float var = fmaxf(s1 * inv_l - md * md, 0.f);
    const float mean = shift + md, rstd = 1.f / sqrtf(var + eps);
    gst[2 * tid] = mean; gst[2 * tid + 1] = rstd;
    const int g = (c0 / a.cpg) + tid;
    mean_out[n * a.G + g] = mean;
    rstd_out[n * a.G + g] = rstd;
  }
  __syncthreads();
  float gmax = 0.f, bmax = 0.f;
  for (int w = 0; w < nw; ++w) { gmax = fmaxf(gmax, bnd[w]); bmax = fmaxf(bmax, bnd[16 + w]); }
  const float bound = __fmaf_rn(gmax, sqrt_lm1, bmax) * a.keep_scale;
  if (blockIdx.x == 0)
    for (int i = tid; i < 256; i += T) rec[i] = i == 0 ? bound : 0.f;
  float sc = 1.f;
  {
    const int be = (int)((__float_as_uint(bound) >> 23) & 0xffu);
    if (be != 0) sc = __uint_as_float((unsigned)min(max(127 + 13 - (be - 127), 1), 254) << 23);
  }
  const float m_lo = gst[2 * g_lo], r_lo = gst[2 * g_lo + 1], m_hi = gst[2 * g_hi], r_hi = gst[2 * g_hi + 1];
  float ga[8], be8[8];
#pragma unroll
  for (int j = 0; j < 8; ++j) { ga[j] = a.gamma[c0 + 8 * q + j]; be8[j] = a.beta[c0 + 8 * q + j]; }
  unsigned long long seed = a.seed;
  if (a.drop_p > 0.f && a.seed_dev) seed += *a.seed_dev;
  float* yo = y ? y + ((long)n * C + c0) * a.HW : nullptr;
  unsigned char* po = planes + ((long)n * Cb + cb) * a.HW * 64 + q * 16;
#pragma unroll
  for (int k = 0; k < PASSES; ++k) {
    const int px = (tid + T * k) >> 2;
    unsigned keep = 0xffu;
    if (a.drop_p > 0.f) {
      const int r = (tid >> 2) & 3;
      const unsigned long long fa = ((unsigned long long)n * C + (c0 + 8 * q + 2 * r)) * a.HW + px;
      const unsigned long long za = stk_mix64(seed, fa >> 2), zb = stk_mix64(seed, (fa + a.HW) >> 2);
      keep = 0u;
#pragma unroll
      for (int rot = 0; rot < 4; ++rot) {
        const unsigned rd = (unsigned)((r - rot) & 3);
        const unsigned send = stk_drop_field(za, rd) | (stk_drop_field(zb, rd) << 16);
        const int pr = (r + rot) & 3;
        const unsigned got = rot == 0 ? send : (unsigned)__shfl((int)send, (lane & ~12) | (pr << 2), 64);
        keep |= ((got & 0xffffu) >= a.drop_thr ? 1u : 0u) << (2 * pr);
        keep |= ((got >> 16) >= a.drop_thr ? 1u : 0u) << (2 * pr + 1);
      }
    }
    float t[8];
#pragma unroll
    for (int j = 0; j < 8; ++j) {
      const float mean = j < 4 ? m_lo : m_hi, rstd = j < 4 ? r_lo : r_hi;
      const float u = ga[j] * ((v[k][j] - mean) * rstd) + be8[j];
      float r = a.act ? act_f(a.act, u) : u;
      if (a.drop_p > 0.f) r = ((keep >> j) & 1u) ? r * a.keep_scale : 0.f;
      t[j] = r;
      if (yo) yo[(long)(8 * q + j) * a.HW + px] = r;
    }
    unsigned hi[4], lo[4];
#pragma unroll
    for (int j = 0; j < 4; ++j) {
      const float v0 = sc * t[2 * j], v1 = sc * t[2 * j + 1];
      const _Float16 h0 = (_Float16)v0, h1 = (_Float16)v1;
      const _Float16 l0 = (_Float16)(v0 - (float)h0), l1 = (_Float16)(v1 - (float)h1);
      typedef _Float16 h2 __attribute__((ext_vector_type(2)));
      hi[j] = __builtin_bit_cast(unsigned, h2{h0, h1});
      lo[j] = __builtin_bit_cast(unsigned, h2{l0, l1});
    }
    typedef unsigned u4 __attribute__((ext_vector_type(4)));
    *reinterpret_cast<u4*>(po + (long)px * 64) = u4{hi[0], hi[1], hi[2], hi[3]};
    *reinterpret_cast<u4*>(po + plane_stride + (long)px * 64) = u4{lo[0], lo[1], lo[2], lo[3]};
  }
}

__global__ __launch_bounds__(256) void gn_stats_kernel(GnArgs a, float* __restrict__ mean_out, float* __restrict__ rstd_out,
                                                       float eps, float sqrt_lm1, float* __restrict__ rec) {
  __shared__ float red[16];
  const int ng = blockIdx.x;
  const int n = ng / a.G, g = ng - n * a.G;
  Seg seg[2];
  group_segments(a, n, g, seg);
  const float* p = seg[0].len ? seg[0].p : seg[1].p;
  const int L = a.cpg * a.HW, L4 = L >> 2;
  const float shift = p[0];
  const float4* p4 = reinterpret_cast<const float4*>(p);
  float s[2] = {0.f, 0.f};
  for (int i = threadIdx.x; i < L4; i += 256) {
    const float4 v = p4[i];
    const float d0 = v.x - shift, d1 = v.y - shift, d2 = v.z - shift, d3 = v.w - shift;
    s[0] += (d0 + d1) + (d2 + d3);
    s[1] += (d0 * d0 + d1 * d1) + (d2 * d2 + d3 * d3);
  }
  block_sum<2>(s, red);
  const float inv_l = 1.f / (float)L;
  const float md = s[0] * inv_l;
  const float var = fmaxf(s[1] * inv_l - md * md, 0.f);
  const float rstd_v = 1.f / sqrtf(var + eps);
  if (threadIdx.x == 0) {
    mean_out[ng] = shift + md;
    rstd_out[ng] = rstd_v;
  }
  if (rec && ng == 0) {
    const int C = a.C1 + a.C2;
    float gm = 0.f, bm = 0.f;
    for (int c = threadIdx.x; c < C; c += 256) { gm = fmaxf(gm, fabsf(a.gamma[c])); bm = fmaxf(bm, fabsf(a.beta[c])); }
    gm = wave_max(gm); bm = wave_max(bm);
    if ((threadIdx.x & 63) == 0) { red[threadIdx.x >> 6] = gm; red[4 + (threadIdx.x >> 6)] = bm; }
    __syncthreads();
    gm = fmaxf(fmaxf(red[0], red[1]), fmaxf(red[2], red[3]));
    bm = fmaxf(fmaxf(red[4], red[5]), fmaxf(red[6], red[7]));
    rec[threadIdx.x] = threadIdx.x == 0 ? __fmaf_rn(gm, sqrt_lm1, bm) * a.keep_scale : 0.f;
  }
}

__global__ __launch_bounds__(256) void gn_fold_stats_kernel(GnArgs a, const float* __restrict__ part, int Sc,
                                                            float* __restrict__ mean_out, float* __restrict__ rstd_out,
                                                            float eps) {
  __shared__ float red[16];
  const int ng = blockIdx.x;
  const int n = ng / a.G, g = ng - n * a.G;
  const int C = a.C1 + a.C2;
  const float shift = gn_chan(a, n, g * a.cpg)[0];
  float s[2] = {0.f, 0.f};
  const long pbase = ((long)n * C + g * a.cpg) * Sc;
  for (int i = threadIdx.x; i < a.cpg * Sc; i += 256) { s[0] += part[(pbase + i) * 2]; s[1] += part[(pbase + i) * 2 + 1]; }
  block_sum<2>(s, red);
  const float inv_l = 1.f / ((float)a.cpg * (float)a.HW);
  const float md = s[0] * inv_l;
  const float var = fmaxf(s[1] * inv_l - md * md, 0.f);
  if (threadIdx.x == 0) { mean_out[ng] = shift + md; rstd_out[ng] = 1.f / sqrtf(var + eps); }
}

constexpr int AP_PIX = 128;
__global__ __launch_bounds__(256) void gn_apply_pl_kernel(GnArgs a, const float* __restrict__ mean_in,
                                                          const float* __restrict__ rstd_in, const float* __restrict__ rec,
                                                          float* __restrict__ y, unsigned char* __restrict__ planes,
                                                          long plane_stride, float* __restrict__ xmax1,
                                                          float* __restrict__ xmax2) {
  __shared__ float t[32 * 129];
  __shared__ float xm[4];
  const int tid = threadIdx.x;
  const int C = a.C1 + a.C2, Cb = C >> 5;
  const int tiles = a.HW / AP_PIX;
  const int tile = blockIdx.x % tiles, rest = blockIdx.x / tiles;
  const int cb = rest % Cb, n = rest / Cb;
  const int c0 = cb * 32, p0 = tile * AP_PIX;
  const float* src = c0 < a.C1 ? a.x1 + ((long)n * a.C1 + c0) * a.HW : a.x2 + ((long)n * a.C2 + (c0 - a.C1)) * a.HW;
  float sc = 1.f;
  {
    const int be = (int)((__float_as_uint(rec[0]) >> 23) & 0xffu);
    if (be != 0) sc = __uint_as_float((unsigned)min(max(127 + 13 - (be - 127), 1), 254) << 23);
  }
  unsigned long long seed = a.seed;
  if (a.drop_p > 0.f && a.seed_dev) seed += *a.seed_dev;
  float amax_l = 0.f;
#pragma unroll
  for (int k = 0; k < 4; ++k) {
    const int i = tid + 256 * k;
    const int c = i >> 5, q4 = i & 31;
    const int ch = c0 + c, px = p0 + 4 * q4;
    const float4 v = *reinterpret_cast<const float4*>(src + (long)c * a.HW + px);
    const int g = ch / a.cpg;
    const float mean = mean_in[n * a.G + g], rstd = rstd_in[n * a.G + g];
    const float ga = a.gamma[ch], be = a.beta[ch];
    float r[4] = {v.x, v.y, v.z, v.w};
    if (xmax1) amax_l = fmaxf(amax_l, fmaxf(fmaxf(fabsf(r[0]), fabsf(r[1])), fmaxf(fabsf(r[2]), fabsf(r[3]))));
    const unsigned long long flat = ((unsigned long long)n * C + ch) * a.HW + px;
    unsigned long long z = 0;
    if (a.drop_p > 0.f) z = stk_mix64(seed, flat >> 2);
#pragma unroll
    for (int j = 0; j < 4; ++j) {
      const float u = ga * ((r[j] - mean) * rstd) + be;
      float o = a.act ? act_f(a.act, u) : u;
      if (a.drop_p > 0.f) o = stk_drop_field(z, j) >= a.drop_thr ? o * a.keep_scale : 0.f;
      r[j] = o;
    }
    if (y) *reinterpret_cast<float4*>(y + ((long)n * C + ch) * a.HW + px) = make_float4(r[0], r[1], r[2], r[3]);
    float* d = t + c * 129 + 4 * q4;
    d[0] = sc * r[0]; d[1] = sc * r[1]; d[2] = sc * r[2]; d[3] = sc * r[3];
  }
  if (xmax1) {
    const float m = wave_max(amax_l);
    if ((tid & 63) == 0) xm[tid >> 6] = m;
  }
  __syncthreads();
  if (xmax1 && tid == 0) {
    float* dst = c0 < a.C1 ? xmax1 : xmax2;
    if (dst) atomicMax(reinterpret_cast<unsigned*>(dst) + (blockIdx.x & 255),
                       __float_as_uint(fmaxf(fmaxf(xm[0], xm[1]), fmaxf(xm[2], xm[3]))));
  }
#pragma unroll
  for (int r2 = 0; r2 < 2; ++r2) {
    const int id = tid + 256 * r2;
    const int px = id >> 2, q = id & 3;
    unsigned hi[4], lo[4];
#pragma unroll
    for (int j = 0; j < 4; ++j) {
      const float v0 = t[(8 * q + 2 * j) * 129 + px], v1 = t[(8 * q + 2 * j + 1) * 129 + px];
      const _Float16 h0 = (_Float16)v0, h1 = (_Float16)v1;
      const _Float16 l0 = (_Float16)(v0 - (float)h0), l1 = (_Float16)(v1 - (float)h1);
      typedef _Float16 h2 __attribute__((ext_vector_type(2)));
      hi[j] = __builtin_bit_cast(unsigned, h2{h0, h1});
      lo[j] = __builtin_bit_cast(unsigned, h2{l0, l1});
    }
    typedef unsigned u4 __attribute__((ext_vector_type(4)));
    unsigned char* o = planes + (((long)n * Cb + cb) * a.HW + p0 + px) * 64 + q * 16;
    *reinterpret_cast<u4*>(o) = u4{hi[0], hi[1], hi[2], hi[3]};
    *reinterpret_cast<u4*>(o + plane_stride) = u4{lo[0], lo[1], lo[2], lo[3]};
  }
}

static inline bool gn_pl_2k_ok(int C1, int C2, int HW, int G) {
  const int C = C1 + C2;
  if (C % 32 || C1 % 32 || C % G || HW % AP_PIX) return false;
  const int cpg = C / G;
  if (cpg > 32 || 32 % cpg) return false;
  const long L = (long)cpg * HW;
  return L <= 16384 || gn_split_ok(HW, cpg);
}

static inline bool gn_pl_fused_ok(int C1, int C2, int HW, int G) {
  const int C = C1 + C2;
  if (C % 32 || C1 % 32 || C % G) return false;
  const int cpg = C / G;
  if (cpg > 32 || 32 % cpg || cpg < 4) return false;
  return HW == 16 || HW == 64 || HW == 256 || HW == 1024;
}

static inline float gn_bound_sqrt(long L) { return sqrtf((float)L - 1.f) * (1.f + 0x1p-16f); }

extern "C" {

int stk_gn_bound_f32(const float* gamma, const float* beta, int C, int G, int HW, float drop_p, float* rec, void* stream) {
  if (!gamma || !beta || !rec || C <= 0 || G <= 0 || C % G || HW <= 0 || drop_p < 0.f || drop_p >= 1.f) return STK_EINVAL;
  hipLaunchKernelGGL(gn_bound_kernel, dim3(1), dim3(256), 0, (hipStream_t)stream, gamma, beta, C, gn_bound_sqrt((long)(C / G) * HW),
                     1.f / (1.f - drop_p), rec);
  STK_CHECK_LAUNCH();
  return STK_OK;
}

int stk_gn_fwd_f32(const float* x1, int C1, const float* x2, int C2, const float* gamma, const float* beta, float* y,
                   float* mean, float* rstd, int N, int HW, int G, float eps, int act, float drop_p,
                   unsigned long long seed, const unsigned long long* seed_dev, float* ws, void* stream) {
  const int C = C1 + C2;
  if (!x1 || !gamma || !beta || !y || !mean || !rstd || N <= 0 || HW <= 0 || G <= 0 || C1 <= 0 || C2 < 0 || C % G ||
      (C2 > 0 && !x2) || drop_p < 0.f || drop_p >= 1.f || act < 0 || act > STK_ACT_ELU)
    return STK_EINVAL;
  GnArgs a;
  a.x1 = x1; a.x2 = x2; a.C1 = C1; a.C2 = C2; a.gamma = gamma; a.beta = beta;
  a.N = N; a.HW = HW; a.G = G; a.cpg = C / G; a.act = act; a.drop_p = drop_p; a.keep_scale = 1.f / (1.f - drop_p); a.drop_thr = stk_drop_threshold(drop_p);
  a.seed = seed; a.seed_dev = seed_dev;
  const bool vec = (HW & 3) == 0 && stk_aligned16(x1) && stk_aligned16(y) && (!x2 || stk_aligned16(x2));
  if (ws && vec && gn_split_ok(HW, a.cpg)) {
    const int Sc = HW / GN_CHUNK;
    const dim3 grid((unsigned)((long)N * C * Sc));
    hipLaunchKernelGGL(gn_split_stats_kernel, grid, dim3(256), 0, (hipStream_t)stream, a, ws, Sc);
    STK_CHECK_LAUNCH();
    hipLaunchKernelGGL(gn_split_fwd_kernel, grid, dim3(256), 0, (hipStream_t)stream, a, ws, Sc, y, mean, rstd, eps);
    STK_CHECK_LAUNCH();
    return STK_OK;
  }
  const long L = (long)a.cpg * HW;
  if (vec && L <= 16384) {
    const int L4 = (int)(L >> 2);
    int T = 64;
    while (T < 1024 && T * 4 < L4) T <<= 1;
    const int ipt = stk_cdiv(L4, T);
#define STK_GN_FWD_FLAT(IPT)                                                                                     \
  hipLaunchKernelGGL((gn_fwd_flat_kernel<IPT>), dim3(N * G), dim3(T), 0, (hipStream_t)stream, a, y, mean, rstd, eps)
    if (ipt <= 1) STK_GN_FWD_FLAT(1);
    else if (ipt <= 2) STK_GN_FWD_FLAT(2);
    else if (ipt <= 3) STK_GN_FWD_FLAT(3);
    else STK_GN_FWD_FLAT(4);
#undef STK_GN_FWD_FLAT
  } else if (vec)
    hipLaunchKernelGGL((gn_fwd_kernel<4>), dim3(N * G), dim3(256), 0, (hipStream_t)stream, a, y, mean, rstd, eps);
  else
    hipLaunchKernelGGL((gn_fwd_kernel<1>), dim3(N * G), dim3(256), 0, (hipStream_t)stream, a, y, mean, rstd, eps);
  STK_CHECK_LAUNCH();
  return STK_OK;
}

static int gn_fwd_pl_impl(const float* x1, int C1, const float* x2, int C2, const float* gamma, const float* beta, float* y,
                          void* planes, float* rec, float* mean, float* rstd, int N, int HW, int G, float eps, int act,
                          float drop_p, unsigned long long seed, const unsigned long long* seed_dev, float* ws, void* stream,
                          float* xmax1, float* xmax2);

int stk_gn_fwd_pl_f32(const float* x1, int C1, const float* x2, int C2, const float* gamma, const float* beta, float* y,
                      void* planes, float* rec, float* mean, float* rstd, int N, int HW, int G, float eps, int act,
                      float drop_p, unsigned long long seed, const unsigned long long* seed_dev, float* ws, void* stream) {
  return gn_fwd_pl_impl(x1, C1, x2, C2, gamma, beta, y, planes, rec, mean, rstd, N, HW, G, eps, act, drop_p, seed, seed_dev, ws,
                        stream, nullptr, nullptr);
}

int stk_gn_fwd_pl_max_f32(const float* x1, int C1, const float* x2, int C2, const float* gamma, const float* beta, float* y,
                          void* planes, float* rec, float* mean, float* rstd, int N, int HW, int G, float eps, int act,
                          float drop_p, unsigned long long seed, const unsigned long long* seed_dev, float* ws,
                          float* xmax1, float* xmax2, void* stream) {
  if (!xmax1 || (C2 > 0 && !xmax2) || !(gn_pl_fused_ok(C1, C2, HW, G) || gn_pl_2k_ok(C1, C2, HW, G))) return STK_EINVAL;
  return gn_fwd_pl_impl(x1, C1, x2, C2, gamma, beta, y, planes, rec, mean, rstd, N, HW, G, eps, act, drop_p, seed, seed_dev, ws,
                        stream, xmax1, xmax2);
}

static int gn_fwd_pl_impl(const float* x1, int C1, const float* x2, int C2, const float* gamma, const float* beta, float* y,
                          void* planes, float* rec, float* mean, float* rstd, int N, int HW, int G, float eps, int act,
                          float drop_p, unsigned long long seed, const unsigned long long* seed_dev, float* ws, void* stream,
                          float* xmax1, float* xmax2) {
  const int C = C1 + C2;
  if (!x1 || !gamma || !beta || !planes || !rec || !mean || !rstd || N <= 0 || HW <= 0 || G <= 0 || C1 <= 0 || C2 < 0 ||
      C % G || (C2 > 0 && !x2) || drop_p < 0.f || drop_p >= 1.f || act < 0 || act > STK_ACT_ELU)
    return STK_EINVAL;
  const long plane_stride = (long)N * ((C + 31) / 32) * HW * 64;
  if (2 * plane_stride >= 0x7fffffffL) return STK_EUNSUPPORTED;
  if (gn_pl_2k_ok(C1, C2, HW, G) && stk_aligned16(x1) && (!x2 || stk_aligned16(x2)) && (!y || stk_aligned16(y))) {
    GnArgs a;
    a.x1 = x1; a.x2 = x2; a.C1 = C1; a.C2 = C2; a.gamma = gamma; a.beta = beta;
    a.N = N; a.HW = HW; a.G = G; a.cpg = C / G; a.act = act; a.drop_p = drop_p; a.keep_scale = 1.f / (1.f - drop_p); a.drop_thr = stk_drop_threshold(drop_p);
    a.seed = seed; a.seed_dev = seed_dev;
    const float sq = gn_bound_sqrt((long)a.cpg * HW);
    hipStream_t s = (hipStream_t)stream;
    if ((long)a.cpg * HW <= 16384) {
      hipLaunchKernelGGL(gn_stats_kernel, dim3(N * G), dim3(256), 0, s, a, mean, rstd, eps, sq, rec);
    } else {
      if (!ws) return STK_EINVAL;
      const int Sc = HW / GN_CHUNK;
      hipLaunchKernelGGL(gn_split_stats_kernel, dim3((unsigned)((long)N * C * Sc)), dim3(256), 0, s, a, ws, Sc);
      hipLaunchKernelGGL(gn_fold_stats_kernel, dim3(N * G), dim3(256), 0, s, a, ws, Sc, mean, rstd, eps);
      hipLaunchKernelGGL(gn_bound_kernel, dim3(1), dim3(256), 0, s, gamma, beta, C, sq, a.keep_scale, rec);
    }
    STK_CHECK_LAUNCH();
    hipLaunchKernelGGL(gn_apply_pl_kernel, dim3((unsigned)((long)N * (C / 32) * (HW / AP_PIX))), dim3(256), 0, s, a, mean, rstd, rec, y,
                       static_cast<unsigned char*>(planes), plane_stride, xmax1, xmax2);
    STK_CHECK_LAUNCH();
    return STK_OK;
  }
  if (gn_pl_fused_ok(C1, C2, HW, G)) {
    GnArgs a;
    a.x1 = x1; a.x2 = x2; a.C1 = C1; a.C2 = C2; a.gamma = gamma; a.beta = beta;
    a.N = N; a.HW = HW; a.G = G; a.cpg = C / G; a.act = act; a.drop_p = drop_p; a.keep_scale = 1.f / (1.f - drop_p); a.drop_thr = stk_drop_threshold(drop_p);
    a.seed = seed; a.seed_dev = seed_dev;
    constexpr int tmax = 512;
    int T = HW * 4 < 1024 ? HW * 4 : 1024;
    if (HW * 4 > 1024 && tmax < T) T = tmax;
    const int items = HW * 4, passes = items / T;
    const float sq = gn_bound_sqrt((long)a.cpg * HW);
    const dim3 grid((unsigned)(N * (C / 32)));
#define STK_GN_PL(P)                                                                                               \
  hipLaunchKernelGGL((gn_fwd_pl_kernel<P>), grid, dim3(T), 0, (hipStream_t)stream, a, y, static_cast<unsigned char*>(planes), \
                     plane_stride, rec, mean, rstd, eps, sq, xmax1, xmax2)
    if (passes == 1) STK_GN_PL(1); else if (passes == 2) STK_GN_PL(2); else if (passes == 4) STK_GN_PL(4); else if (passes == 8) STK_GN_PL(8); else return STK_EUNSUPPORTED;
#undef STK_GN_PL
    STK_CHECK_LAUNCH();
    return STK_OK;
  }
  if (!y || xmax1 || xmax2) return STK_EINVAL;
  int rc = stk_gn_fwd_f32(x1, C1, x2, C2, gamma, beta, y, mean, rstd, N, HW, G, eps, act, drop_p, seed, seed_dev, ws, stream);
  if (rc) return rc;
  rc = stk_gn_bound_f32(gamma, beta, C, G, HW, drop_p, rec, stream);
  if (rc) return rc;
  return stk_split_planes_f32(y, N, C, HW, rec, 256, planes, stream);
}

int stk_gn_fwd_pl_fused(int C1, int C2, int HW, int G) { return gn_pl_fused_ok(C1, C2, HW, G) || gn_pl_2k_ok(C1, C2, HW, G) ? 1 : 0; }

static inline bool gn_bwd_flat_shape(int C, int HW, int G) {
  if (C <= 0 || G <= 0 || C % G || HW < 16 || (HW & (HW - 1))) return false;
  const long L = (long)(C / G) * HW;
  return L <= 16384 && C / G <= 512 && !gn_split_ok(HW, C / G);
}
int stk_gn_bwd_out_ok(int C1, int C2, int HW, int G) { return C1 > 0 && C2 >= 0 && gn_bwd_flat_shape(C1 + C2, HW, G) ? 1 : 0; }

static int gn_bwd_impl(const float* dy, const float* x1, int C1, const float* x2, int C2, const float* gamma,
                       const float* beta, const float* mean, const float* rstd, float* dx1, float dx1_beta, float* dx2,
                       float dx2_beta, float* dgamma, float* dbeta, float* ws, int N, int HW, int G, int act, float drop_p,
                       unsigned long long seed, const unsigned long long* seed_dev, void* stream, GnBwdOut out);

int stk_gn_bwd_f32(const float* dy, const float* x1, int C1, const float* x2, int C2, const float* gamma,
                   const float* beta, const float* mean, const float* rstd, float* dx1, float dx1_beta, float* dx2,
                   float dx2_beta, float* dgamma, float* dbeta, float* ws, int N, int HW, int G, int act, float drop_p,
                   unsigned long long seed, const unsigned long long* seed_dev, void* stream) {
  const GnBwdOut none = {nullptr, nullptr, 0, 1.f, nullptr, nullptr, 0.f};
  return gn_bwd_impl(dy, x1, C1, x2, C2, gamma, beta, mean, rstd, dx1, dx1_beta, dx2, dx2_beta, dgamma, dbeta, ws, N, HW, G, act,
                     drop_p, seed, seed_dev, stream, none);
}

int stk_gn_bwd_out_f32(const float* dy, const float* x1, int C1, const float* x2, int C2, const float* gamma,
                       const float* beta, const float* mean, const float* rstd, float* dx1, float dx1_beta, float* dx2,
                       float dx2_beta, float* dgamma, float* dbeta, float* ws, int N, int HW, int G, int act, float drop_p,
                       unsigned long long seed, const unsigned long long* seed_dev, const float* dx1_add, float add_scale,
                       float* dx_sum, float out_scale, float* dtemb, int temb_stride, float* dx_amax, void* stream) {
  if (!dx1 || !stk_gn_bwd_out_ok(C1, C2, HW, G) || (dtemb && temb_stride < C1) || (C2 > 0 && !x2)) return STK_EINVAL;
  if (!(stk_aligned16(x1) && stk_aligned16(dy) && stk_aligned16(dx1) && (!x2 || stk_aligned16(x2)) &&
        (!dx2 || stk_aligned16(dx2)) && (!dx1_add || stk_aligned16(dx1_add))))
    return STK_EUNSUPPORTED;
  const GnBwdOut out = {dx_sum, dtemb, temb_stride, out_scale, dx_amax, dx1_add, add_scale};
  return gn_bwd_impl(dy, x1, C1, x2, C2, gamma, beta, mean, rstd, dx1, dx1_beta, dx2, dx2_beta, dgamma, dbeta, ws, N, HW, G,
                     act, drop_p, seed, seed_dev, stream, out);
}

static int gn_bwd_impl(const float* dy, const float* x1, int C1, const float* x2, int C2, const float* gamma,
                       const float* beta, const float* mean, const float* rstd, float* dx1, float dx1_beta, float* dx2,
                       float dx2_beta, float* dgamma, float* dbeta, float* ws, int N, int HW, int G, int act, float drop_p,
                       unsigned long long seed, const unsigned long long* seed_dev, void* stream, GnBwdOut out) {
  const int C = C1 + C2;
  if (!dy || !x1 || !gamma || !beta || !mean || !rstd || !ws || N <= 0 || HW <= 0 || G <= 0 || C1 <= 0 || C2 < 0 ||
      C % G || (C2 > 0 && !x2) || drop_p < 0.f || drop_p >= 1.f || act < 0 || act > STK_ACT_ELU)
    return STK_EINVAL;
  GnArgs a;
  a.x1 = x1; a.x2 = x2; a.C1 = C1; a.C2 = C2; a.gamma = gamma; a.beta = beta;
  a.N = N; a.HW = HW; a.G = G; a.cpg = C / G; a.act = act; a.drop_p = drop_p; a.keep_scale = 1.f / (1.f - drop_p); a.drop_thr = stk_drop_threshold(drop_p);
  a.seed = seed; a.seed_dev = seed_dev;
  const long L = (long)a.cpg * HW;
  int hw_log2 = 0;
  while ((1 << hw_log2) < HW) ++hw_log2;
  const bool flat = (1 << hw_log2) == HW && HW >= 16 && L <= 16384 && a.cpg <= 512 && stk_aligned16(x1) &&
                    stk_aligned16(dy) && (!x2 || stk_aligned16(x2)) && (!dx1 || stk_aligned16(dx1)) &&
                    (!dx2 || stk_aligned16(dx2));
  const bool al16 = stk_aligned16(x1) && stk_aligned16(dy) && (!x2 || stk_aligned16(x2)) && (!dx1 || stk_aligned16(dx1)) &&
                    (!dx2 || stk_aligned16(dx2));
  if (al16 && gn_split_ok(HW, a.cpg)) {
    const int Sc = HW / GN_CHUNK;
    float* part = ws + 2L * N * C;
    const dim3 grid((unsigned)((long)N * C * Sc));
    hipLaunchKernelGGL(gn_split_bwd_part_kernel, grid, dim3(256), 0, (hipStream_t)stream, a, dy, mean, rstd, part, Sc);
    STK_CHECK_LAUNCH();
    hipLaunchKernelGGL(gn_split_bwd_kernel, grid, dim3(256), 0, (hipStream_t)stream, a, dy, mean, rstd, part, Sc, dx1,
                       dx1_beta, dx2, dx2_beta, ws);
  } else if (flat) {
    const int L4 = (int)(L >> 2);
    const int tgt = 4;
    int T = 64;
    while (T < 1024 && T * tgt < L4) T <<= 1;
    const int ipt = stk_cdiv(L4, T);
#define STK_GN_FLAT(IPT)                                                                                          \
  do {                                                                                                            \
    if (out.sum || out.temb || out.amax || out.add)                                                               \
      hipLaunchKernelGGL((gn_bwd_flat_kernel<IPT, true>), dim3(N * G), dim3(T), 0, (hipStream_t)stream, a, dy, mean, rstd, dx1, \
                         dx1_beta, dx2, dx2_beta, ws, hw_log2, out);                                               \
    else                                                                                                          \
      hipLaunchKernelGGL((gn_bwd_flat_kernel<IPT, false>), dim3(N * G), dim3(T), 0, (hipStream_t)stream, a, dy, mean, rstd, dx1, \
                         dx1_beta, dx2, dx2_beta, ws, hw_log2, out);                                               \
  } while (0)
    if (ipt <= 1) STK_GN_FLAT(1);
    else if (ipt <= 2) STK_GN_FLAT(2);
    else if (ipt <= 3) STK_GN_FLAT(3);
    else STK_GN_FLAT(4);
#undef STK_GN_FLAT
  } else {
    hipLaunchKernelGGL(gn_bwd_kernel, dim3(N * G), dim3(256), 0, (hipStream_t)stream, a, dy, mean, rstd, dx1, dx1_beta,
                       dx2, dx2_beta, ws);
  }
  STK_CHECK_LAUNCH();
  if (dgamma || dbeta) {
    hipLaunchKernelGGL(gn_param_grad_kernel, dim3(stk_cdiv(C, 32)), dim3(256), 0, (hipStream_t)stream, ws, dgamma,
                       dbeta, N, C, (const StkGnFoldDesc*)nullptr);
    STK_CHECK_LAUNCH();
  }
  return STK_OK;
}

int stk_gn_param_grad_batch(const StkGnFoldDesc* descs_dev, int count, int max_C, void* stream) {
  if (!descs_dev || count <= 0 || max_C <= 0) return STK_EINVAL;
  hipLaunchKernelGGL(gn_param_grad_kernel, dim3(stk_cdiv(max_C, 32), (unsigned)count), dim3(256), 0, (hipStream_t)stream,
                     (const float*)nullptr, (float*)nullptr, (float*)nullptr, 0, 0, descs_dev);
  STK_CHECK_LAUNCH();
  return STK_OK;
}

long stk_gn_ws_bytes(int N, int C, int HW, int G) {
  if (N <= 0 || C <= 0 || HW <= 0 || G <= 0 || C % G) return 0;
  long f = 2L * N * C;
  if (gn_split_ok(HW, C / G)) f += 2L * N * C * (HW / GN_CHUNK);
  return f * 4;
}

}
```

soft-truncation_amd/engine/graph.py:

```python
import math
import os

import numpy as np

SQRT2 = float(np.float32(np.sqrt(2.)))
_X2W_WGS_ALONE = int(os.environ.get('STK_X2W_WGS_ALONE', '0'))
_SIDE_DELAY = 0
_SIDE_DELAY_FILTER = None
_ALIGN = 64
AMAX = 768


def _round_up(n, a=_ALIGN):
  return (n + a - 1) // a * a


class Tensor:
  __slots__ = ('shape', 'numel', 'space', 'off', 'goff', 'needs_grad', 'name', 'seen', 'external_grad',
               'producer', 'pl_off', 'pl_rec', 'pl_maker', 'f32_fwd', 'f32_bwd')

  def __init__(self, shape, space, off, needs_grad, name):
    self.shape = tuple(int(s) for s in shape)
    self.numel = int(np.prod(self.shape)) if len(self.shape) else 1
    self.space = space
    self.off = off
    self.goff = None
    self.needs_grad = needs_grad
    self.name = name
    self.seen = 0
    self.external_grad = False
    self.producer = None
    self.pl_off = None
    self.pl_rec = None
    self.pl_maker = None
    self.f32_fwd = True
    self.f32_bwd = True

  def __repr__(self):
    return f'T({self.name}{list(self.shape)}@{self.space}+{self.off})'


class Runtime:

  def __init__(self, lib, stream, act, gact, param, gparam, const, ws, ws_bytes, training, seed,
               seed_dev=None):
    self.lib = lib
    self.stream = stream
    self.base = {'act': act, 'param': param, 'const': const}
    self.gbase = {'act': gact, 'param': gparam}
    self.ws = ws
    self.ws_bytes = ws_bytes
    self.training = training
    self.seed = seed
    self.seed_dev = seed_dev
    self.wp = 0
    self.with_backward = True
    self.f16 = False
    self.f16_bwd = False
    self.pl = 0
    self.dypl = 0
    self.prof = None
    self.param_grads = True
    self.gnpart = 0
    self.gn_table = 0
    self.gn_maxc = 0
    self._fold_lo = None
    self._fold_hi = None
    self.side = None
    self.ws2 = 0
    self._cur = None

  def side_launch(self, fn, *args):
    s = self.side.begin()
    if _SIDE_DELAY and (_SIDE_DELAY_FILTER is None or _SIDE_DELAY_FILTER(self._cur)):
      import torch
      with torch.cuda.stream(self.side.stream):
        torch.cuda._sleep(_SIDE_DELAY)
    fn(*args, s)
    self.side.end()

  def join_side(self):
    if self.side is not None:
      self.side.join()

  def defer_fold(self, index):
    if self._fold_hi is not None and index != self._fold_hi:
      assert index > self._fold_hi, 'folds must be deferred in table order'
      self.flush_folds()
    if self._fold_lo is None:
      self._fold_lo = index
    self._fold_hi = index + 1

  def flush_folds(self):
    if self._fold_lo is None:
      return
    lo, hi = self._fold_lo, self._fold_hi
    self._fold_lo = self._fold_hi = None
    self.lib.gn_param_grad_batch(self.gn_table + 32 * lo, hi - lo, self.gn_maxc, self.stream)

  def timed(self, kind, flops, fn, *args):
    if self.prof is None:
      fn(*args)
    else:
      self.prof.launch(kind, flops, fn, args)

  def v(self, t):
    return None if t is None else self.base[t.space] + 4 * t.off

  def g(self, t):
    if t is None or not t.needs_grad or t.goff is None:
      return None
    if t.space == 'param' and not self.param_grads:
      return None
    return self.gbase[t.space] + 4 * t.goff

  def planes(self, t):
    return self.pl + t.pl_off

  def rec(self, t):
    rt, off = t.pl_rec
    return self.v(rt) + 4 * off

  def make_planes(self, t):
    n = t.shape[0]
    c = t.shape[1]
    hw = t.numel // (n * c)
    self.lib.amax_partial_f32(self.v(t), t.numel, self.rec(t), self.stream)
    self.lib.split_planes_f32(self.v(t), n, c, hw, self.rec(t), 256, self.planes(t), self.stream)


class Op:
  inputs = ()

  def plan_backward(self):
    self.beta = {}
    for t in self.inputs:
      if t is None or not t.needs_grad or t.space != 'act':
        continue
      if id(t) in self.beta:
        continue
      self.beta[id(t)] = 1.0 if (t.seen > 0 or t.external_grad) else 0.0
      t.seen += 1

  def b(self, t):
    return self.beta.get(id(t), 1.0)

  def forward(self, rt):
    raise NotImplementedError

  def backward(self, rt):
    raise NotImplementedError

  def ws_bytes(self, lib):
    return 0

  def bwd_launches(self):
    xs = [t for t in self.inputs if t is not None]
    return not xs or any(t.needs_grad for t in xs) or any(
      isinstance(v, Tensor) and v.space == 'param' and v.needs_grad for v in vars(self).values())


class GroupNormAct(Op):

  def __init__(self, g, x1, x2, gamma, beta_t, groups, eps, act, drop_p, name):
    self.x1, self.x2, self.gamma, self.beta_t = x1, x2, gamma, beta_t
    N, C1, H, W = x1.shape
    C2 = x2.shape[1] if x2 is not None else 0
    self.N, self.C1, self.C2, self.HW, self.G = N, C1, C2, H * W, groups
    self.eps, self.act, self.drop_p = eps, int(act), float(drop_p)
    self.y = g.new((N, C1 + C2, H, W), name=name)
    self.mean = g.new((N * groups,), needs_grad=False, name=name + '.mean')
    self.rstd = g.new((N * groups,), needs_grad=False, name=name + '.rstd')
    self.inputs = (x1, x2)
    self.op_id = g.next_id()
    self.fused = False
    self.fold_off = None
    self.fold_index = None
    self.dy_cons = None
    self.add_from = None
    self.xmax_for = None

  def _p(self, rt):
    return self.drop_p if rt.training else 0.0

  def forward(self, rt):
    seed = (rt.seed + 0x9E3779B1 * self.op_id) & 0xFFFFFFFFFFFFFFFF
    y = self.y
    if y.pl_maker is self:
      need_f32 = y.f32_fwd or (rt.with_backward and y.f32_bwd) or not self.fused
      cv = self.xmax_for
      if cv is not None:
        rt.lib.gn_fwd_pl_max_f32(rt.v(self.x1), self.C1, rt.v(self.x2), self.C2, rt.v(self.gamma), rt.v(self.beta_t),
                                 rt.v(y) if need_f32 else None, rt.planes(y), rt.rec(y), rt.v(self.mean), rt.v(self.rstd),
                                 self.N, self.HW, self.G, self.eps, self.act, self._p(rt), seed, rt.seed_dev, rt.ws,
                                 rt.v(cv.amax), rt.v(cv.amax) + 4 * 256 if self.x2 is not None else None, rt.stream)
        return
      rt.lib.gn_fwd_pl_f32(rt.v(self.x1), self.C1, rt.v(self.x2), self.C2, rt.v(self.gamma), rt.v(self.beta_t),
                           rt.v(y) if need_f32 else None, rt.planes(y), rt.rec(y), rt.v(self.mean), rt.v(self.rstd), self.N, self.HW, self.G,
                           self.eps, self.act, self._p(rt), seed, rt.seed_dev, rt.ws, rt.stream)
      return
    rt.lib.gn_fwd_f32(rt.v(self.x1), self.C1, rt.v(self.x2), self.C2, rt.v(self.gamma), rt.v(self.beta_t),
                      rt.v(self.y), rt.v(self.mean), rt.v(self.rstd), self.N, self.HW, self.G, self.eps,
                      self.act, self._p(rt), seed, rt.seed_dev, rt.ws, rt.stream)

  def backward(self, rt):
    dgamma, dbeta, ws = rt.g(self.gamma), rt.g(self.beta_t), rt.ws
    cons = self.dy_cons
    if rt.gn_table and self.fold_index is not None and (dgamma is not None or dbeta is not None):
      dgamma = dbeta = None
      ws = rt.gnpart + 4 * self.fold_off
      rt.defer_fold(self.fold_index)
    adder = self.add_from
    if cons is not None or adder is not None:
      dsum = dtemb = damax = add = None
      out_scale = add_scale = 1.0
      tstride = 0
      if cons is not None:
        assert rt.gn_table, 'the by-products of the GroupNorm backward ride on the batched folds'
        out_scale = 1.0 / cons.out_div
        if cons.bsum_index is not None and rt.param_grads:
          dsum = rt.gnpart + 4 * cons.bsum_off
          rt.defer_fold(cons.bsum_index)
        if cons.temb is not None and cons.temb.needs_grad:
          dtemb, tstride = rt.g(cons.temb) + 4 * cons.temb_col, cons.temb_stride
        damax = rt.v(cons.dy_peer.amax if cons.dy_peer is not None else cons.amax) + 4 * 512
      if adder is not None:
        add, add_scale = rt.g(adder.y), 1.0 / adder.out_div
      rt.lib.gn_bwd_out_f32(rt.g(self.y), rt.v(self.x1), self.C1, rt.v(self.x2), self.C2, rt.v(self.gamma), rt.v(self.beta_t),
                            rt.v(self.mean), rt.v(self.rstd), rt.g(self.x1), self.b(self.x1), rt.g(self.x2),
                            self.b(self.x2) if self.x2 is not None else 0.0, dgamma, dbeta, ws, self.N, self.HW, self.G,
                            self.act, self._p(rt), (rt.seed + 0x9E3779B1 * self.op_id) & 0xFFFFFFFFFFFFFFFF, rt.seed_dev,
                            add, add_scale, dsum, out_scale, dtemb, tstride, damax, rt.stream)
      return
    rt.lib.gn_bwd_f32(rt.g(self.y), rt.v(self.x1), self.C1, rt.v(self.x2), self.C2,
                      rt.v(self.gamma), rt.v(self.beta_t), rt.v(self.mean), rt.v(self.rstd),
                      rt.g(self.x1), self.b(self.x1), rt.g(self.x2), self.b(self.x2) if self.x2 is not None else 0.0,
                      dgamma, dbeta, ws,
                      self.N, self.HW, self.G, self.act, self._p(rt),
                      (rt.seed + 0x9E3779B1 * self.op_id) & 0xFFFFFFFFFFFFFFFF, rt.seed_dev, rt.stream)

  def ws_bytes(self, lib):
    return max(int(lib.gn_ws_bytes(self.N, self.C1 + self.C2, self.HW, self.G)), 4 * 2 * self.N * (self.C1 + self.C2))


class Conv(Op):

  def __init__(self, g, x1, x2, w, bias, w_layout, Cout, KH, KW, stride, pad, OH, OW,
               temb=None, temb_col=0, res=None, out_div=1.0, name='conv'):
    self.x1, self.x2, self.w, self.bias = x1, x2, w, bias
    N, C1, H, W = x1.shape
    C2 = x2.shape[1] if x2 is not None else 0
    self.N, self.C1, self.C2, self.H, self.W = N, C1, C2, H, W
    self.Cout, self.KH, self.KW, self.stride, self.pad, self.OH, self.OW = Cout, KH, KW, stride, pad, OH, OW
    self.w_layout = w_layout
    self.temb, self.temb_col = temb, temb_col
    self.temb_stride = temb.shape[1] if temb is not None else 0
    self.res, self.out_div = res, float(out_div)
    self.y = g.new((N, Cout, OH, OW), name=name)
    self.amax = Tensor((AMAX,), 'act', None, False, name + '.amax')
    g.conv_amax.append(self.amax)
    self.inputs = (x1, x2, res)
    self.flops = 2.0 * N * OH * OW * Cout * (C1 + C2) * KH * KW

  _VARIANT = {0: 't64', 1: 't128', 3: 't128', 4: 'thin', 5: 'x2'}

  def _kind(self, lib, direction):
    key = '_kind_' + direction
    k = getattr(self, key, None)
    if k is None:
      v = int(lib.conv2d_variant({'fwd': 0, 'dgrad': 1, 'wgrad': 2}[direction], self.C1, self.C2, self.N, self.H,
                                 self.W, self.Cout, self.OH, self.OW, self.KH, self.KW, self.stride, self.pad,
                                 self.w_layout))
      k = f'conv{self.KH}x{self.KW}.{direction}.{self._VARIANT.get(v, "t64")}'
      setattr(self, key, k)
    return k

  def _label_pl(self, lib, direction):
    key = '_label_' + direction
    k = getattr(self, key, None)
    if k is None:
      k = self._kind(lib, direction) + 'p'
      if direction == 'wgrad':
        k += f'.w{min(self.W, 32)}'
      elif hasattr(lib, 'conv2d_pl_ksplit'):
        d = 0 if direction == 'fwd' else 1
        c2 = 0 if d == 0 else self.C2
        if int(lib.conv2d_pl_ksplit(d, self.C1, c2, self.N, self.H, self.W, self.Cout, self.KH, self.KW)) > 1:
          k += '.k'
        elif hasattr(lib, 'conv2d_pl_halo'):
          hw = int(lib.conv2d_pl_halo(d, self.C1, c2, self.N, self.H, self.W, self.Cout, self.KH, self.KW))
          if hw:
            k += f'.h{hw}'
      setattr(self, key, k)
    return k

  def _dims(self):
    return (self.N, self.H, self.W, self.Cout, self.OH, self.OW, self.KH, self.KW, self.stride, self.pad)

  def f16_form(self, lib):
    return self.pl_fwd or self._kind(lib, 'fwd').endswith('.x2')

  wp_off = (None, None)

  def plan_wp(self, lib, offset):
    shape = (self.C1, self.C2, self.N, self.H, self.W, self.Cout, self.KH, self.KW, self.stride, self.pad)
    offs = []
    for direction in (0, 1):
      nb = int(lib.conv2d_wp_bytes(direction, *shape)) if self.OH == self.H and self.OW == self.W else 0
      if nb > 0:
        offs.append(offset)
        offset = _round_up(offset + nb, 256)
      else:
        offs.append(None)
    self.wp_off = tuple(offs)
    return offset

  def _wp(self, rt, direction):
    off = self.wp_off[direction]
    return rt.wp + off if (rt.wp and off is not None) else None

  dy_peer = None
  dy_from = None
  dy_prod = None
  bsum_off = None
  bsum_index = None
  res_via = None
  x_from = None
  peer_planes = None

  dypl_off = None
  pl_fwd = False
  pl_dgrad = False
  pl_wgrad = False
  x_rec_own = False

  def plan_planes(self, g, lib):
    same = self.stride == 1 and self.OH == self.H and self.OW == self.W and self.pad == self.KH // 2
    if not same:
      return
    dims = (self.N, self.H, self.W, self.Cout, self.KH, self.KW, 1, self.pad)
    t = self.x1
    by_gn = isinstance(t.producer, GroupNormAct)
    if self.x2 is None and (self.KH == 3 or by_gn) and int(lib.conv2d_pl_ok(0, self.C1, 0, *dims)):
      if t.pl_off is None:
        t.pl_off = g.pl_bytes
        g.pl_bytes += _round_up(int(lib.planes_bytes(self.N, self.C1, self.H * self.W)), 256)
        t.pl_rec = (self.amax, 0)
        t.pl_maker = t.producer if by_gn else self
        self.x_rec_own = True
      self.pl_fwd = True
    needs_dx = (self.x1.needs_grad and self.x1.space == 'act') or (self.x2 is not None and self.x2.needs_grad)
    if needs_dx and self.KH == 3 and int(lib.conv2d_pl_ok(1, self.C1, self.C2, *dims)):
      self.pl_dgrad = True
    if (self.pl_fwd and self.KH == 3 and self.w_layout == 0 and self.w.needs_grad and
        os.environ.get('STK_PLANES_WGRAD', '1') != '0' and hasattr(lib, 'conv2d_wgrad_pl_ok') and
        int(lib.conv2d_wgrad_pl_ok(self.N, self.H, self.W, self.C1, self.Cout))):
      self.pl_wgrad = True
    if self.pl_dgrad or self.pl_wgrad:
      nb = _round_up(int(lib.planes_bytes(self.N, self.Cout, self.OH * self.OW)), 256)
      g.dypl_bytes = max(g.dypl_bytes, nb)
      if self.pl_wgrad and g.own_dypl:
        self.dypl_off = g.pl_bytes
        g.pl_bytes += nb

  def plan_backward(self):
    if self.dy_peer is not None or self.res_via is not None:
      saved, self.inputs = self.inputs, (self.x1, self.x2)
      Op.plan_backward(self)
      self.inputs = saved
    else:
      Op.plan_backward(self)

  def forward(self, rt):
    temb = rt.v(self.temb) + 4 * self.temb_col if self.temb is not None else None
    f16 = rt.f16 and self.f16_form(rt.lib)
    if self.pl_fwd:
      t = self.x1
      if t.pl_maker is self:
        rt.make_planes(t)
      label = self._label_pl(rt.lib, 'fwd')
      rt.timed(label + '.f16' if f16 else label, self.flops, rt.lib.conv2d_fwd_pl_f16x1 if f16 else rt.lib.conv2d_fwd_pl_f32,
               rt.planes(t), rt.rec(t), self.C1, rt.v(self.w), self.w_layout, rt.v(self.bias), temb, self.temb_stride,
               rt.v(self.res), self.out_div, rt.v(self.y), self.N, self.H, self.W, self.Cout, self.KH, self.KW,
               self._wp(rt, 0), rt.ws, rt.ws_bytes, rt.stream)
      return
    if f16:
      fn = rt.lib.conv2d_fwd_rec_f16x1 if self.x_from is not None else rt.lib.conv2d_fwd_wp_f16x1
    else:
      fn = rt.lib.conv2d_fwd_rec_f32 if self.x_from is not None else rt.lib.conv2d_fwd_wp_f32
    rt.timed(self._kind(rt.lib, 'fwd') + ('.f16' if f16 else ''), self.flops, fn,
             rt.v(self.x1), self.C1, rt.v(self.x2), self.C2, rt.v(self.w), self.w_layout,
             rt.v(self.bias), temb, self.temb_stride, rt.v(self.res), self.out_div,
             rt.v(self.y), *self._dims(), self._wp(rt, 0), rt.v(self.amax), rt.ws, rt.ws_bytes, rt.stream)

  def backward(self, rt):
    gy = rt.g(self.y)
    alpha = 1.0 / self.out_div
    lib = rt.lib
    src = self.dy_from
    if src is not None:
      gy = rt.g(src.y)
      alpha = alpha / src.out_div
    dtemb = None
    if self.temb is not None and self.temb.needs_grad:
      dtemb = rt.g(self.temb) + 4 * self.temb_col
    gb = rt.g(self.bias)
    g1, g2 = rt.g(self.x1), rt.g(self.x2)
    gw = rt.g(self.w)
    pl_dgrad = self.pl_dgrad and (g1 is not None or g2 is not None)
    pl_wgrad = self.pl_wgrad and gw is not None
    dy_rec = rt.v(self.amax) + 4 * 512
    rec_done = False
    fuse_rec = (pl_dgrad or pl_wgrad) and self.Cout <= 256 and (dtemb is not None or gb is not None)
    res_grad = self.res is not None and self.res.needs_grad
    peer = self.dy_peer
    if self.res_via is not None:
      res_grad = False
    if self.dy_prod is not None:
      gb = dtemb = None
      fuse_rec = False
      rec_done = True
      if peer is not None:
        dy_rec = rt.v(peer.amax) + 4 * 512
        res_grad = False
    elif src is not None:
      gb = dtemb = None
      fuse_rec = False
      rec_done = True
    elif peer is not None:
      lib.bias_grad_amax_dual_f32(gy, self.N, self.Cout, self.OH * self.OW, alpha, dtemb, self.temb_stride, gb, dy_rec,
                                  rt.g(peer.bias), rt.v(peer.amax) + 4 * 512, rt.ws, rt.stream)
      rec_done = True
      res_grad = fuse_rec = False
    if res_grad and fuse_rec and hasattr(lib, 'bias_grad_amax_res_f32'):
      lib.bias_grad_amax_res_f32(gy, self.N, self.Cout, self.OH * self.OW, alpha, dtemb, self.temb_stride, gb, dy_rec,
                                 rt.g(self.res), self.b(self.res), rt.ws, rt.stream)
      rec_done = True
      res_grad = fuse_rec = False
    if res_grad:
      gr = rt.g(self.res)
      lib.axpby_f32(gy, alpha, gr, self.b(self.res), gr, self.y.numel, rt.stream)
    if fuse_rec:
      lib.bias_grad_amax_f32(gy, self.N, self.Cout, self.OH * self.OW, alpha, dtemb, self.temb_stride, gb, dy_rec,
                             rt.ws, rt.stream)
      rec_done = True
    elif not rec_done and (dtemb is not None or gb is not None):
      lib.bias_grad_f32(gy, self.N, self.Cout, self.OH * self.OW, alpha, dtemb, self.temb_stride, gb,
                        rt.ws, rt.stream)
    sfx = '_f16x1' if rt.f16_bwd else '_f32'
    f16 = '.f16' if rt.f16_bwd else ''
    have = 1 if self._kind(lib, 'fwd').endswith('.x2') else 0
    if self.pl_fwd and not self.x_rec_own:
      have = 0
    if src is not None or self.dy_prod is not None:
      have |= 2
    if pl_dgrad or pl_wgrad:
      rec = dy_rec
      if not rec_done:
        lib.amax_partial_f32(gy, self.y.numel, rec, rt.stream)
      dypl = rt.pl + self.dypl_off if self.dypl_off is not None else rt.dypl
      lib.split_planes_f32(gy, self.N, self.Cout, self.OH * self.OW, rec, 256, dypl, rt.stream)
      have |= 2
    if src is not None and self.peer_planes is not None and (g1 is not None or g2 is not None):
      ppl = rt.pl + src.dypl_off if self.peer_planes == 'own' else rt.dypl
      rt.timed(self._label_pl(lib, 'dgrad') + f16, self.flops, getattr(lib, 'conv2d_dgrad_pl' + sfx),
               ppl, rt.v(self.amax) + 4 * 512, rt.v(self.w), self.w_layout, g1, self.C1, self.b(self.x1),
               g2, self.C2, self.b(self.x2) if self.x2 is not None else 0.0,
               alpha, self.N, self.H, self.W, self.Cout, self.KH, self.KW, self._wp(rt, 1), rt.ws, rt.ws_bytes, rt.stream)
    elif pl_dgrad:
      rt.timed(self._label_pl(lib, 'dgrad') + f16, self.flops, getattr(lib, 'conv2d_dgrad_pl' + sfx),
               dypl, rec, rt.v(self.w), self.w_layout, g1, self.C1, self.b(self.x1),
               g2, self.C2, self.b(self.x2) if self.x2 is not None else 0.0,
               alpha, self.N, self.H, self.W, self.Cout, self.KH, self.KW, self._wp(rt, 1), rt.ws, rt.ws_bytes, rt.stream)
      have |= 2
    elif g1 is not None or g2 is not None:
      kind = self._kind(lib, 'dgrad')
      rt.timed(kind + (f16 if kind.endswith('.x2') else ''), self.flops,
               getattr(lib, ('conv2d_dgrad_rec' if (src is not None or self.dy_prod is not None) else 'conv2d_dgrad_wp') + sfx),
               gy, rt.v(self.w), self.w_layout, g1, self.C1, self.b(self.x1),
               g2, self.C2, self.b(self.x2) if self.x2 is not None else 0.0,
               alpha, *self._dims(), self._wp(rt, 1), rt.v(self.amax), rt.ws, rt.ws_bytes, rt.stream)
      if self._kind(lib, 'dgrad').endswith('.x2'):
        have |= 2
    rt._cur = self.y.name
    if pl_wgrad and rt.side is not None and rt.prof is None and self.dypl_off is not None:
      rt.side_launch(getattr(lib, 'conv2d_wgrad_pl' + sfx), rt.planes(self.x1), rt.rec(self.x1), dypl, dy_rec, gw, alpha, rt.ws2,
                     rt.ws_bytes, self.N, self.H, self.W, self.C1, self.Cout)
    elif pl_wgrad:
      rt.timed(self._label_pl(lib, 'wgrad') + f16, self.flops, getattr(lib, 'conv2d_wgrad_pl_wgs' + sfx),
               rt.planes(self.x1), rt.rec(self.x1), dypl, dy_rec, gw, alpha, rt.ws, rt.ws_bytes,
               self.N, self.H, self.W, self.C1, self.Cout, _X2W_WGS_ALONE, rt.stream)
    elif gw is not None and rt.side is not None and rt.prof is None:
      rt.side_launch(getattr(lib, 'conv2d_wgrad_amax' + sfx), rt.v(self.x1), self.C1, rt.v(self.x2), self.C2, gy, gw, self.w_layout, alpha,
                     rt.ws2, rt.ws_bytes, *self._dims(), rt.v(self.amax), have)
    elif gw is not None:
      kind = self._kind(lib, 'wgrad')
      rt.timed(kind + (f16 if kind.endswith('.x2') else ''), self.flops, getattr(lib, 'conv2d_wgrad_amax' + sfx),
               rt.v(self.x1), self.C1, rt.v(self.x2), self.C2, gy, gw, self.w_layout, alpha,
               rt.ws, rt.ws_bytes, *self._dims(), rt.v(self.amax), have, rt.stream)

  def ws_bytes(self, lib):
    shape = (self.C1, self.C2, self.N, self.H, self.W, self.Cout, self.KH, self.KW, self.stride, self.pad)
    pw = int(lib.conv2d_wgrad_pl_ws_bytes(self.N, self.H, self.W, self.C1, self.Cout)) \
        if (self.C2 == 0 and self.KH == 3 and hasattr(lib, 'conv2d_wgrad_pl_ws_bytes')) else 0
    return max(pw, int(lib.conv2d_wgrad_ws_bytes(self.C1, self.C2, self.N, self.Cout, self.OH, self.OW,
                                                 self.KH, self.KW)),
               int(lib.conv2d_fwd_ws_bytes(*shape)), int(lib.conv2d_dgrad_ws_bytes(*shape)),
               4 * self.N * self.Cout)


class Linear(Op):

  KSLICE = 256
  KSPLIT_MIN = 2048

  def __init__(self, g, x, w, bias, name='linear'):
    self.x, self.w, self.bias = x, w, bias
    self.B, self.fin = x.shape
    self.fout = w.shape[0]
    self.y = g.new((self.B, self.fout), name=name)
    self.inputs = (x,)
    self.kslice = next((k for k in (self.KSLICE, 128, 64, 32) if self.fout % k == 0), 0)
    self.ksplit = self.fout // self.kslice if (self.fout >= self.KSPLIT_MIN and self.kslice and x.needs_grad) else 0
    self.ones = g.const(np.ones(self.ksplit, dtype=np.float32)) if self.ksplit else None

  def forward(self, rt):
    B, fin, fout = self.B, self.fin, self.fout
    rt.lib.gemm_f32(rt.v(self.x), fin, 1, 0, rt.v(self.w), 1, fin, 0, rt.v(self.y), fout, 1, 0,
                    rt.v(self.bias), 2 if self.bias is not None else 0, B, fout, fin, 1, 1.0, 0.0, rt.stream)

  def backward(self, rt):
    B, fin, fout = self.B, self.fin, self.fout
    gy = rt.g(self.y)
# ... 362 lines not shown
    self.block, self.count = block, count
    self.y = block

  def forward(self, rt):
    rt.lib.fill_strided_f32(rt.v(self.block), 0.0, self.count, 512, AMAX, rt.stream)

  def backward(self, rt):
    pass

  def bwd_launches(self):
    return False


class ZeroRecords(Op):

  def __init__(self, block, count):
    self.block, self.count = block, count
    self.y = block

  def forward(self, rt):
    pass

  def backward(self, rt):
    rt.lib.fill_strided_f32(rt.v(self.block) + 4 * 512, 0.0, self.count, AMAX - 512, AMAX, rt.stream)


class Graph:

  def __init__(self, flat, lib=None):
    self.flat = flat
    self.lib = lib
    self.precision = 'fp32'
    self.ops = []
    self.tensors = []
    self.conv_amax = []
    self.act_size = 0
    self.gact_size = 0
    self.const_chunks = []
    self.const_size = 0
    self.inputs = {}
    self.output = None
    self._id = 0
    self._params = {}

  def next_id(self):
    self._id += 1
    return self._id

  def new(self, shape, needs_grad=True, name=''):
    t = Tensor(shape, 'act', self.act_size, needs_grad, name)
    self.act_size += _round_up(t.numel)
    self.tensors.append(t)
    return t

  def input(self, key, shape, needs_grad=False):
    t = self.new(shape, needs_grad=needs_grad, name='in.' + key)
    self.inputs[key] = t
    return t

  def const(self, array):
    array = np.ascontiguousarray(array, dtype=np.float32)
    t = Tensor(array.shape, 'const', self.const_size, False, 'const')
    self.const_chunks.append((self.const_size, array.reshape(-1)))
    self.const_size += _round_up(array.size)
    return t

  def param(self, p):
    if p is None:
      return None
    t = self._params.get(id(p))
    if t is None:
      off, trainable = self.flat.offset_of(p)
      t = Tensor(tuple(p.shape), 'param', off, trainable, 'param')
      t.goff = off if trainable else None
      self._params[id(p)] = t
    return t

  def add(self, op):
    self.ops.append(op)
    if op.y.producer is None:
      op.y.producer = op
    return op.y

  act_code = 1

  def gn_act(self, x1, x2, gn, act=True, drop_p=0.0, name='gn'):
    op = GroupNormAct(self, x1, x2, self.param(gn.weight), self.param(gn.bias), gn.num_groups, gn.eps,
                      self.act_code if act else 0, drop_p, name)
    return self.add(op)

  def conv(self, x1, x2, weight, bias, w_layout=0, stride=1, pad=None, out_hw=None,
           temb=None, temb_col=0, res=None, out_div=1.0, name='conv'):
    if w_layout == 0:
      Cout, _, KH, KW = weight.shape
    else:
      _, Cout = weight.shape
      KH = KW = 1
    if pad is None:
      pad = KH // 2
    cin_w = weight.shape[1] if w_layout == 0 else weight.shape[0]
    cin_x = x1.shape[1] + (x2.shape[1] if x2 is not None else 0)
    if cin_w != cin_x:
      raise RuntimeError(f'{name}: expected input with {cin_w} channels (weight {tuple(weight.shape)}), got {cin_x}')
    H, W = x1.shape[2], x1.shape[3]
    if out_hw is None:
      OH = (H + 2 * pad - KH) // stride + 1
      OW = (W + 2 * pad - KW) // stride + 1
    else:
      OH, OW = out_hw
    op = Conv(self, x1, x2, self.param(weight), self.param(bias), w_layout, Cout, KH, KW, stride, pad, OH, OW,
              temb=temb, temb_col=temb_col, res=res, out_div=out_div, name=name)
    return self.add(op)

  def conv1x1_t(self, x1, w_tensor, b_tensor, Cout, name='conv'):
    H, W = x1.shape[2], x1.shape[3]
    if w_tensor.shape[0] != x1.shape[1]:
      raise RuntimeError(f'{name}: expected input with {w_tensor.shape[0]} channels, got {x1.shape[1]}')
    return self.add(Conv(self, x1, None, w_tensor, b_tensor, 1, Cout, 1, 1, 1, 0, H, W, name=name))

  def linear(self, x, weight, bias, name='linear'):
    return self.add(Linear(self, x, self.param(weight), self.param(bias), name))

  def linear_t(self, x, w_tensor, b_tensor, name='linear'):
    return self.add(Linear(self, x, w_tensor, b_tensor, name))

  def silu(self, x, name='silu'):
    return self.add(SiLU(self, x, name, self.act_code))

  def finalize(self, output, lib):
    self.output = output
    output.external_grad = True
    self.amax_block = self.new((AMAX * max(len(self.conv_amax), 1),), needs_grad=False, name='conv.amax')
    for i, t in enumerate(self.conv_amax):
      t.off = self.amax_block.off + AMAX * i
    for t in self.tensors:
      if t.needs_grad:
        t.goff = self.gact_size
        self.gact_size += _round_up(t.numel)
    self.ws_bytes = max([256] + [op.ws_bytes(lib) for op in self.ops])
    self.ws_bytes = _round_up(self.ws_bytes, 256)
    self.wp_bytes = 0
    for op in self.ops:
      if isinstance(op, Conv):
        self.wp_bytes = op.plan_wp(lib, self.wp_bytes)
    self.pl_bytes = 0
    self.dypl_bytes = 0
    self.own_dypl = os.environ.get('STK_WGRAD_STREAM', '1') != '0' and bool(getattr(lib, 'is_device', False))
    if os.environ.get('STK_PLANES', '1') != '0' and hasattr(lib, 'conv2d_pl_ok'):
      for op in self.ops:
        if isinstance(op, Conv):
          op.plan_planes(self, lib)
      self._plan_f32_copies(lib)
      self._plan_x_records(lib)
    self._plan_shared_dy(lib)
    fold_batch = os.environ.get('STK_GN_FOLD_BATCH', '1') != '0' and hasattr(lib, 'gn_param_grad_batch')
    if hasattr(lib, 'gn_bwd_out_f32'):
      self._plan_res_via(lib)
      if fold_batch:
        self._plan_dy_producers(lib)
    self.gnpart_size = 0
    self.gn_folds = []
    if fold_batch:
      for op in reversed(self.ops):
        if not isinstance(op, GroupNormAct):
          continue
        cons = op.dy_cons
        if op.gamma.needs_grad or op.beta_t.needs_grad or cons is not None:
          op.fold_off = self.gnpart_size
          op.fold_index = len(self.gn_folds)
          self.gnpart_size += _round_up(max(int(lib.gn_ws_bytes(op.N, op.C1 + op.C2, op.HW, op.G)) // 4,
                                            2 * op.N * (op.C1 + op.C2)))
          self.gn_folds.append((op.fold_off, op.gamma.goff if op.gamma.needs_grad else None,
                                op.beta_t.goff if op.beta_t.needs_grad else None, op.N, op.C1 + op.C2))
        if cons is not None:
          own = cons.bias.goff if cons.bias is not None and cons.bias.needs_grad else None
          peer = cons.dy_peer
          other = peer.bias.goff if peer is not None and peer.bias is not None and peer.bias.needs_grad else None
          if own is not None or other is not None:
            cons.bsum_off = self.gnpart_size
            cons.bsum_index = len(self.gn_folds)
            self.gnpart_size += _round_up(2 * cons.N * cons.Cout)
            self.gn_folds.append((cons.bsum_off, other, own, cons.N, cons.Cout))
    for op in reversed(self.ops):
      op.plan_backward()
    return self

  def _plan_x_records(self, lib):
    if os.environ.get('STK_X_RECORDS', '1') == '0' or not hasattr(lib, 'gn_fwd_pl_max_f32'):
      return
    index = {id(op): i for i, op in enumerate(self.ops)}
    found = False
    for op in self.ops:
      if not isinstance(op, Conv) or op.pl_fwd or op.x_from is not None or not op._kind(lib, 'fwd').endswith('.x2'):
        continue
      for gn in self.ops:
        if (isinstance(gn, GroupNormAct) and gn.x1 is op.x1 and gn.x2 is op.x2 and gn.fused and gn.y.pl_maker is gn and
            gn.xmax_for is None and index[id(gn)] < index[id(op)]):
          gn.xmax_for, op.x_from = op, gn
          found = True
          break
    if found:
      self.ops.insert(0, ZeroXRecords(self.amax_block, len(self.conv_amax)))

  def _grad_writers(self):
    w = {}
    for op in self.ops:
      ins = op.inputs
      if isinstance(op, Conv) and (op.dy_peer is not None or op.res_via is not None):
        ins = (op.x1, op.x2)
      seen = set()
      for t in ins:
        if t is not None and t.space == 'act' and t.needs_grad and id(t) not in seen:
          seen.add(id(t))
          w.setdefault(id(t), []).append(op)
    return w

  def _plan_res_via(self, lib):
    if os.environ.get('STK_RES_VIA', '1') == '0':
      return
    index = {id(op): i for i, op in enumerate(self.ops)}
    for op in self.ops:
      if not isinstance(op, Conv) or op.res is None or not op.res.needs_grad or op.dy_peer is not None:
        continue
      r = op.res
      if r.shape != op.y.shape or r is op.x1 or r is op.x2 or op.y is self.output:
        continue
      for gn in self.ops:
        if (isinstance(gn, GroupNormAct) and gn.x1 is r and gn.add_from is None and index[id(gn)] < index[id(op)] and
            int(lib.gn_bwd_out_ok(gn.C1, gn.C2, gn.HW, gn.G))):
          gn.add_from, op.res_via = op, gn
          break

  def _plan_dy_producers(self, lib):
    if os.environ.get('STK_DY_PRODUCER', '1') == '0':
      return
    writers = self._grad_writers()
    for op in self.ops:
      if not isinstance(op, Conv) or op.Cout > 256:
        continue
      if not (op.pl_dgrad or op.pl_wgrad) and not (op.dy_peer is None and op._kind(lib, 'dgrad').endswith('.x2')):
        continue
      if op.dy_from is not None or op.y is self.output or not op.y.needs_grad:
        continue
      if op.res is not None and op.res.needs_grad and op.dy_peer is None and op.res_via is None:
        continue
      if op.bias is None and (op.temb is None or not op.temb.needs_grad):
        continue
      if op.pl_dgrad and op.w.needs_grad and not op.pl_wgrad and op.dy_peer is not None:
        continue
      ws = writers.get(id(op.y), [])
      if not ws or not isinstance(ws[0], GroupNormAct):
        continue
      gn = ws[0]
      if gn.x1 is not op.y or gn.x2 is op.y or gn.dy_cons is not None:
        continue
      if not int(lib.gn_bwd_out_ok(gn.C1, gn.C2, gn.HW, gn.G)):
        continue
      gn.dy_cons, op.dy_prod = op, gn
    if any(isinstance(op, GroupNormAct) and op.dy_cons is not None for op in self.ops):
      self.ops.append(ZeroRecords(self.amax_block, len(self.conv_amax)))

  def _plan_shared_dy(self, lib):
    if os.environ.get('STK_SHARED_DY', '1') == '0' or not hasattr(lib, 'bias_grad_amax_dual_f32'):
      return
    readers = {}
    for op in self.ops:
      for v in vars(op).values():
        if isinstance(v, Tensor) and v.space == 'act' and v.producer is not op:
          readers.setdefault(id(v), []).append(op)
    for op in self.ops:
      if not isinstance(op, Conv) or op.res is None or not op.res.needs_grad:
        continue
      r = op.res
      P = r.producer
      if not isinstance(P, Conv) or P is op or r is self.output or readers.get(id(r), []) != [op]:
        continue
      if r is op.x1 or r is op.x2 or op.temb is r:
        continue
      if not ((op.pl_dgrad or op.pl_wgrad) and op.Cout <= 256 and op.OH * op.OW < 4096 and op.bias is not None):
        continue
      if P.temb is not None or P.res is not None or P.bias is None or P.dy_from is not None or P.dy_peer is not None:
        continue
      if P.pl_dgrad or P.pl_wgrad or P.Cout != op.Cout:
        continue
      op.dy_peer, P.dy_from = P, op
      if ((P.x1.needs_grad or (P.x2 is not None and P.x2.needs_grad)) and
          hasattr(lib, 'conv2d_pl_ok') and
          int(lib.conv2d_pl_ok(1, P.C1, P.C2, P.N, P.H, P.W, P.Cout, P.KH, P.KW, 1, P.pad))):
        if op.dypl_off is not None:
          P.peer_planes = 'own'
        elif not self.own_dypl and self.ops.index(P) + 1 == self.ops.index(op):
          P.peer_planes = 'scratch'

  def _plan_f32_copies(self, lib):
    readers = {}
    for op in self.ops:
      for v in vars(op).values():
        if isinstance(v, Tensor) and v.space == 'act' and v.producer is not op:
          readers.setdefault(id(v), []).append(op)
    for op in self.ops:
      if not isinstance(op, GroupNormAct) or op.y.pl_maker is not op:
        continue
      op.fused = bool(int(lib.gn_fwd_pl_fused(op.C1, op.C2, op.HW, op.G))) if hasattr(lib, 'gn_fwd_pl_fused') else False
      y = op.y
      fwd = bwd = y is self.output
      for r in readers.get(id(y), []):
        as_x1 = isinstance(r, Conv) and r.x1 is y and r.x2 is not y and r.res is not y and r.temb is not y
        if not (as_x1 and r.pl_fwd):
          fwd = True
        if not as_x1 or (r.w.needs_grad and not r.pl_wgrad) or not r.pl_fwd:
          bwd = True
      y.f32_fwd, y.f32_bwd = fwd, bwd
```

soft-truncation_amd/engine/lib.py:

```python
import ctypes
import os
import threading
from ctypes import c_char_p, c_float, c_int, c_long, c_ulonglong, c_void_p

_PKG_DIR = os.path.dirname(os.path.dirname(os.path.abspath(__file__)))
PRODUCT_LIB = os.path.join(_PKG_DIR, 'csrc', 'libstk.so')

P = c_void_p
S = c_void_p
I = c_int
L = c_long
F = c_float
U64 = c_ulonglong

SIGNATURES = {
  'stk_strerror': [I],
  'stk_backend': [],
  'stk_version': [],
  'stk_upfirdn2d_f32': [P, P, P, I, I, I, I, I, I, I, I, I, I, I, I, I, I, S],
  'stk_upfirdn2d_acc_f32': [P, P, P, F, I, I, I, I, I, I, I, I, I, I, I, I, I, I, S],
  'stk_fused_bias_act_f32': [P, P, P, P, L, I, I, I, I, F, F, S],
  'stk_fused_bias_act_f16': [P, P, P, P, L, I, I, I, I, F, F, S],
  'stk_fused_bias_act_f64': [P, P, P, P, L, I, I, I, I, F, F, S],
  'stk_upfirdn2d_f16': [P, P, P, I, I, I, I, I, I, I, I, I, I, I, I, I, I, S],
  'stk_upfirdn2d_f64': [P, P, P, I, I, I, I, I, I, I, I, I, I, I, I, I, I, S],
  'stk_gn_fwd_f32': [P, I, P, I, P, P, P, P, P, I, I, I, F, I, F, U64, P, P, S],
  'stk_gn_ws_bytes': [I, I, I, I],
  'stk_gn_bwd_f32': [P, P, I, P, I, P, P, P, P, P, F, P, F, P, P, P, I, I, I, I, F, U64, P, S],
  'stk_gn_bwd_out_ok': [I, I, I, I],
  'stk_conv2d_pl_ksplit': [I, I, I, I, I, I, I, I, I],
  'stk_conv2d_pl_halo': [I, I, I, I, I, I, I, I, I],
  'stk_gn_bwd_out_f32': [P, P, I, P, I, P, P, P, P, P, F, P, F, P, P, P, I, I, I, I, F, U64, P, P, F, P, F, P, I, P, S],
  'stk_gn_param_grad_batch': [P, I, I, S],
  'stk_conv2d_variant': [I, I, I, I, I, I, I, I, I, I, I, I, I, I],
  'stk_conv2d_fwd_ws_bytes': [I, I, I, I, I, I, I, I, I, I],
  'stk_conv2d_dgrad_ws_bytes': [I, I, I, I, I, I, I, I, I, I],
  'stk_conv2d_fwd_f32': [P, I, P, I, P, I, P, P, I, P, F, P, I, I, I, I, I, I, I, I, I, I, P, L, S],
  'stk_conv2d_dgrad_f32': [P, P, I, P, I, F, P, I, F, F, I, I, I, I, I, I, I, I, I, I, P, L, S],
  'stk_conv2d_wp_bytes': [I, I, I, I, I, I, I, I, I, I, I],
  'stk_conv2d_wp_desc': [I, P, I, I, I, I, I, P, P],
  'stk_conv2d_wprep_batch': [P, I, L, S],
  'stk_conv2d_fwd_wp_f32': [P, I, P, I, P, I, P, P, I, P, F, P, I, I, I, I, I, I, I, I, I, I, P, P, P, L, S],
  'stk_conv2d_fwd_rec_f32': [P, I, P, I, P, I, P, P, I, P, F, P, I, I, I, I, I, I, I, I, I, I, P, P, P, L, S],
  'stk_conv2d_dgrad_wp_f32': [P, P, I, P, I, F, P, I, F, F, I, I, I, I, I, I, I, I, I, I, P, P, P, L, S],
  'stk_conv2d_dgrad_rec_f32': [P, P, I, P, I, F, P, I, F, F, I, I, I, I, I, I, I, I, I, I, P, P, P, L, S],
  'stk_conv2d_wgrad_ws_bytes': [I, I, I, I, I, I, I, I],
  'stk_conv2d_wgrad_f32': [P, I, P, I, P, P, I, F, P, L, I, I, I, I, I, I, I, I, I, I, S],
  'stk_conv2d_wgrad_amax_f32': [P, I, P, I, P, P, I, F, P, L, I, I, I, I, I, I, I, I, I, I, P, I, S],
  'stk_gn_bound_f32': [P, P, I, I, I, F, P, S],
  'stk_gn_fwd_pl_f32': [P, I, P, I, P, P, P, P, P, P, P, I, I, I, F, I, F, U64, P, P, S],
  'stk_gn_fwd_pl_fused': [I, I, I, I],
  'stk_gn_fwd_pl_max_f32': [P, I, P, I, P, P, P, P, P, P, P, I, I, I, F, I, F, U64, P, P, P, P, S],
  'stk_planes_bytes': [I, I, I],
  'stk_amax_partial_f32': [P, L, P, S],
  'stk_split_planes_f32': [P, I, I, I, P, I, P, S],
  'stk_conv2d_pl_ok': [I, I, I, I, I, I, I, I, I, I, I],
  'stk_conv2d_fwd_pl_f32': [P, P, I, P, I, P, P, I, P, F, P, I, I, I, I, I, I, P, P, L, S],
  'stk_conv2d_dgrad_pl_f32': [P, P, P, I, P, I, F, P, I, F, F, I, I, I, I, I, I, P, P, L, S],
  'stk_conv2d_wgrad_pl_ok': [I, I, I, I, I],
  'stk_conv2d_wgrad_pl_ws_bytes': [I, I, I, I, I],
  'stk_conv2d_wgrad_pl_f32': [P, P, P, P, P, F, P, L, I, I, I, I, I, S],
  'stk_conv2d_wgrad_pl_wgs_f32': [P, P, P, P, P, F, P, L, I, I, I, I, I, I, S],
  'stk_bias_grad_f32': [P, I, I, I, F, P, I, P, P, S],
  'stk_bias_grad_amax_f32': [P, I, I, I, F, P, I, P, P, P, S],
  'stk_bias_grad_amax_res_f32': [P, I, I, I, F, P, I, P, P, P, F, P, S],
  'stk_bias_grad_amax_dual_f32': [P, I, I, I, F, P, I, P, P, P, P, P, S],
  'stk_gemm_f32': [P, L, L, L, P, L, L, L, P, L, L, L, P, I, I, I, I, I, F, F, S],
  'stk_softmax_fwd_f32': [P, P, L, I, F, S],
  'stk_softmax_bwd_f32': [P, P, P, L, I, F, S],
  'stk_attention_ok': [I, I, I],
  'stk_attention_fwd_f32': [P, P, P, L, P, P, P, I, I, I, F, S],
  'stk_attention_bwd_f32': [P, P, P, L, P, P, P, P, P, F, P, F, P, F, L, I, I, I, F, S],
  'stk_silu_fwd_f32': [P, P, L, S],
  'stk_silu_bwd_f32': [P, P, P, F, L, S],
  'stk_act_fwd_f32': [P, P, L, I, S],
  'stk_act_bwd_f32': [P, P, P, F, L, I, S],
  'stk_axpby_f32': [P, F, P, F, P, L, S],
  'stk_add_div_f32': [P, P, F, P, L, S],
  'stk_concat_f32': [P, I, P, I, P, I, I, S],
  'stk_concat_bwd_f32': [P, P, F, I, P, F, I, I, I, S],
  'stk_fixed_fourier_fwd_f32': [P, P, I, I, I, S],
  'stk_fixed_fourier_bwd_f32': [P, P, P, F, I, I, I, S],
  'stk_affine_f32': [P, F, F, P, L, S],
  'stk_fill_f32': [P, F, L, S],
  'stk_fill_strided_f32': [P, F, L, L, L, S],
  'stk_resample_naive_f32': [P, P, L, I, I, I, F, F, S],
  'stk_rowscale_f32': [P, P, P, I, L, I, S],
  'stk_timestep_embedding_f32': [P, P, P, I, I, S],
  'stk_fourier_embedding_f32': [P, P, P, I, I, S],
  'stk_perturb_f32': [P, P, P, P, P, I, L, S],
  'stk_sm_loss_fwd_f32': [P, P, P, P, P, I, L, I, I, I, S],
  'stk_sm_loss_bwd_f32': [P, P, P, P, P, P, I, L, I, I, I, S],
  'stk_sumsq_f32': [P, L, P, P, S],
  'stk_adam_f32': [P, P, P, P, L, F, F, F, F, F, I, F, F, P, F, S],
  'stk_adam_amsgrad_f32': [P, P, P, P, P, L, F, F, F, F, F, I, F, F, P, F, S],
  'stk_ema_f32': [P, P, L, F, S],
  'stk_dropout_mask_f32': [P, L, F, U64, S],
  'stk_samples_to_uint8': [P, P, I, I, L, S],
  'stk_preprocess_u8': [P, P, I, I, I, I, I, I, I, U64, S],
}
SIGNATURES_FP16 = {
  'stk_conv2d_fwd_pl_f16x1': SIGNATURES['stk_conv2d_fwd_pl_f32'],
  'stk_conv2d_fwd_rec_f16x1': SIGNATURES['stk_conv2d_fwd_rec_f32'],
  'stk_conv2d_fwd_wp_f16x1': SIGNATURES['stk_conv2d_fwd_wp_f32'],
}
SIGNATURES_FP16_TRAIN = {
  'stk_conv2d_dgrad_pl_f16x1': SIGNATURES['stk_conv2d_dgrad_pl_f32'],
  'stk_conv2d_dgrad_rec_f16x1': SIGNATURES['stk_conv2d_dgrad_rec_f32'],
  'stk_conv2d_dgrad_wp_f16x1': SIGNATURES['stk_conv2d_dgrad_wp_f32'],
  'stk_conv2d_wgrad_pl_f16x1': SIGNATURES['stk_conv2d_wgrad_pl_f32'],
  'stk_conv2d_wgrad_pl_wgs_f16x1': SIGNATURES['stk_conv2d_wgrad_pl_wgs_f32'],
  'stk_conv2d_wgrad_amax_f16x1': SIGNATURES['stk_conv2d_wgrad_amax_f32'],
}
SIGNATURES_BLOCKS = {
  'stk_fourier_embedding_bwd_f32': [P, P, P, P, F, I, I, S],
}
SIGNATURES_ATTN_LONG = {
  'stk_attention_long_ok': [I, I, I],
  'stk_attention_long_ws_bytes': [I, I, I],
  'stk_attention_long_fwd_f32': [P, P, P, L, P, P, P, I, I, I, F, P, L, S],
  'stk_attention_long_bwd_f32': [P, P, P, L, P, P, P, P, P, P, F, P, F, P, F, L, I, I, I, F, P, L, S],
}
_RESTYPE = {'stk_strerror': c_char_p, 'stk_backend': c_char_p, 'stk_conv2d_wgrad_ws_bytes': c_long,
            'stk_conv2d_fwd_ws_bytes': c_long, 'stk_conv2d_dgrad_ws_bytes': c_long, 'stk_gn_ws_bytes': c_long,
            'stk_conv2d_wp_bytes': c_long, 'stk_conv2d_wp_desc': c_long, 'stk_planes_bytes': c_long, 'stk_conv2d_wgrad_pl_ws_bytes': c_long}
_RESTYPE_ATTN_LONG = {'stk_attention_long_ws_bytes': c_long}
_NO_CHECK_ATTN_LONG = set(_RESTYPE_ATTN_LONG) | {'stk_attention_long_ok'}
_NO_CHECK = set(_RESTYPE) | {'stk_version', 'stk_conv2d_variant', 'stk_conv2d_pl_ok', 'stk_gn_fwd_pl_fused', 'stk_conv2d_wgrad_pl_ok', 'stk_attention_ok', 'stk_gn_bwd_out_ok', 'stk_conv2d_pl_ksplit', 'stk_conv2d_pl_halo'}


class StkMissingError(RuntimeError):
  """The HIP library is not built / not loadable.  The product path never falls back."""


class StkError(RuntimeError):
  """A C-ABI entry returned a negative status."""


class StkLib:

  def __init__(self, path):
    self.path = path
    self._cdll = ctypes.CDLL(path)
    for name, argtypes in SIGNATURES.items():
      try:
        fn = getattr(self._cdll, name)
      except AttributeError as e:
        raise StkMissingError(f'{path} does not export {name}') from e
      fn.argtypes = argtypes
      fn.restype = _RESTYPE.get(name, c_int)
      if name in _NO_CHECK:
        setattr(self, name[4:], fn)
      else:
        setattr(self, name[4:], self._checked(name, fn))
    self.has_fp16 = self._bind_optional(SIGNATURES_FP16, 'include/stk_fp16.h')
    self.has_fp16_train = self._bind_optional(SIGNATURES_FP16_TRAIN, 'include/stk_fp16_train.h')
    self.has_blocks = self._bind_optional(SIGNATURES_BLOCKS, 'include/stk_blocks.h')
    self.has_attention_long = self._bind_optional(SIGNATURES_ATTN_LONG, 'include/stk_attention_long.h',
                                                  restype=_RESTYPE_ATTN_LONG, unchecked=_NO_CHECK_ATTN_LONG)
    self.backend = self._cdll.stk_backend().decode()
    self.is_device = self.backend.startswith('hip')

  def _bind_optional(self, table, header, restype=None, unchecked=()):
    present = [name for name in table if hasattr(self._cdll, name)]
    if present and len(present) != len(table):
      raise StkMissingError(f'{self.path} exports only part of {header}: {present}')
    for name in present:
      fn = getattr(self._cdll, name)
      fn.argtypes = table[name]
      fn.restype = (restype or {}).get(name, c_int)
      setattr(self, name[4:], fn if name in unchecked else self._checked(name, fn))
    return bool(present)

  def _checked(self, name, fn):
    strerror = self._cdll.stk_strerror

    def call(*args):
      rc = fn(*args)
      if rc != 0:
        raise StkError(f'{name} failed: {strerror(rc).decode()} (rc={rc})')
    call.__name__ = name
    call.raw = fn
    return call


_lock = threading.Lock()
_cache = {}


def load_path(path):
  path = os.path.abspath(path)
  with _lock:
    lib = _cache.get(path)
    if lib is None:
      if not os.path.exists(path):
        raise StkMissingError(f'{path} not found')
      lib = _cache[path] = StkLib(path)
    return lib


def load():
  alt = os.environ.get('STK_LIBSTK')
  if alt:
    lib = load_path(alt)
    if not lib.is_device:
      raise StkMissingError(f'STK_LIBSTK={alt} is not a HIP build of include/stk.h (backend {lib.backend}): refused')
    return lib
  if not os.path.exists(PRODUCT_LIB):
    raise StkMissingError(
      f'{PRODUCT_LIB} is not built. Run `python -c "import __graft_entry__ as g; g.build()"` '
      f'(or `make -C soft-truncation_amd/csrc`). The HIP library is mandatory: this package has '
      f'no CPU or PyTorch fallback for the score-network path.')
  return load_path(PRODUCT_LIB)


class _NoGuard:
  def __enter__(self):
    return self

  def __exit__(self, *exc):
    return False


_NO_GUARD = _NoGuard()


def device_guard(device):
  import torch
  if device.type != 'cuda':
    return _NO_GUARD
  idx = device.index if device.index is not None else torch.cuda.current_device()
  if idx == torch.cuda.current_device():
    return _NO_GUARD
  return torch.cuda.device(idx)


def stream_ptr(device):
  import torch
  if device.type != 'cuda':
    return 0
  return torch.cuda.current_stream(device).cuda_stream
```

Before: 3496 images/s.

## Fuse GroupNorm moment computation into preceding conv forward epilogue

Adds an EpFwdMom epilogue so the conv forward kernel writes per-tile shifted mean/variance partials for each output channel alongside y. A new gn_apply_pl_kernel<true> variant combines these partials per group inside the apply kernel and also computes the bound record. This lets the graph drop the separate GroupNorm statistics and bound passes when the producer is a non-split pl conv. The cost is an extra LDS reduction in the conv epilogue and a small moments buffer, and the statistics are now computed with different floating-point ordering.

```diff
diff --git a/include/stk_gn_moments.h b/include/stk_gn_moments.h
--- /dev/null
+++ b/include/stk_gn_moments.h
@@ -0,0 +1,26 @@
+#ifndef STK_GN_MOMENTS_H
+#define STK_GN_MOMENTS_H
+
+#include "stk.h"
+
+#ifdef __cplusplus
+extern "C" {
+#endif
+
+int stk_conv2d_moments_ok(int C, int N, int H, int W, int Cout, int KH, int KW);
+int stk_gn_moments_ok(int C1, int C2, int HW, int G);
+long stk_gn_moments_bytes(int N, int C, int HW);
+int stk_conv2d_fwd_pl_mom_f32(const void* xpl, const float* xamax, int C, const float* w, int w_layout, const float* bias,
+                              const float* temb, int temb_stride, const float* res, float out_div, float* y, int N, int H,
+                              int W, int Cout, int KH, int KW, const void* wp, void* ws, long ws_bytes, float* mom,
+                              void* stream);
+int stk_gn_fwd_pl_mom_f32(const float* x1, int C1, const float* mom1, const float* x2, int C2, const float* mom2,
+                          const float* gamma, const float* beta, float* y, void* planes, float* rec, float* mean,
+                          float* rstd, int N, int HW, int G, float eps, int act, float drop_p, unsigned long long seed,
+                          const unsigned long long* seed_dev, float* xmax1, float* xmax2, void* stream);
+
+#ifdef __cplusplus
+}
+#endif
+
+#endif
diff --git a/soft-truncation_amd/csrc/conv.hip b/soft-truncation_amd/csrc/conv.hip
--- a/soft-truncation_amd/csrc/conv.hip
+++ b/soft-truncation_amd/csrc/conv.hip
@@ -1,6 +1,7 @@
 #include "igemm.h"
 #include "stk_fp16.h"
 #include "stk_fp16_train.h"
+#include "stk_gn_moments.h"
 
 namespace {
 
@@ -385,13 +386,15 @@
     sb = s; stm = s + 128;
   }
   __device__ void init(const ConvP&, int, int) {}
-  __device__ void finish(const ConvP&, unsigned char*, int) {}
+  template <class ACC> __device__ void finish(const ConvP&, unsigned char*, int, ACC&, int, int) {}
   __device__ void col(const ConvP& p, int n) {
     b = n / p.OHW;
     col_off = b * p.Cout * p.OHW + (n - b * p.OHW);
     tb = (b - b0) * 128;
   }
-  __device__ void strip(const ConvP& p, int mbase, int M, bool nok, int, const floatx16& acc) {
+  __device__ void strip(const ConvP& p, int mbase, int M, bool nok, int, const floatx16& acc) { strip_t<false>(p, mbase, M, nok, acc); }
+  template <bool KEEP, class ACC>
+  __device__ __forceinline__ void strip_t(const ConvP& p, int mbase, int M, bool nok, ACC& acc) {
     if (sb && (!p.temb || nimg <= TEMB_IMGS)) {
       const int ml = mbase - m0;
       float rv[16]; int idx[16];
@@ -415,6 +418,7 @@
           if (p.res) v += rv[4 * g + u];
           if (p.use_div) v *= p.inv_div;
           if (idx[4 * g + u] >= 0) p.y[idx[4 * g + u]] = v;
+          if constexpr (KEEP) acc[4 * g + u] = v;
         }
       }
       return;
@@ -441,7 +445,68 @@
         if (p.res) v += rv[u];
         if (p.use_div) v *= p.inv_div;
         if (ok[u]) p.y[idx[u]] = v;
+        if constexpr (KEEP) acc[4 * g + u] = v;
       }
+    }
+  }
+};
+struct EpFwdMom : EpFwd {
+  __device__ void strip(const ConvP& p, int mbase, int M, bool nok, int, floatx16& acc) { strip_t<true>(p, mbase, M, nok, acc); }
+  template <int NJ>
+  __device__ void finish(const ConvP& p, unsigned char* lds, int tid, floatx16 (&acc)[2][NJ], int n0, int M) {
+    static_assert(NJ == 2, "moments: 128 x 128 tiles, two 32-pixel column blocks per wave");
+    __shared__ __attribute__((aligned(16))) float mu[128];
+    float* part = reinterpret_cast<float*>(lds);
+    const int lane = tid & 63, wid = tid >> 6, fk = lane >> 5, fc = lane & 31;
+    const int r0 = (wid & 1) * 64 + 4 * fk, slot = (wid >> 1) * 32 + fc;
+    __syncthreads();
+#pragma unroll
+    for (int i = 0; i < 2; ++i)
+#pragma unroll
+      for (int e = 0; e < 16; ++e) {
+        part[(r0 + 32 * i + strip_row(e)) * 64 + slot] = acc[i][0][e] + acc[i][1][e];
+      }
+    __syncthreads();
+    float mean = 0.f;
+    if (tid < 128) {
+      const float p0 = part[tid * 64 + (tid & 63)];
+      float s[4] = {0.f, 0.f, 0.f, 0.f};
+#pragma unroll 8
+      for (int k = 0; k < 64; ++k) s[k & 3] += part[tid * 64 + ((k + tid) & 63)] - p0;
+      mean = __fmaf_rn((s[0] + s[1]) + (s[2] + s[3]), 1.f / 128.f, 0.5f * p0);
+      mu[tid] = mean;
+    }
+    __syncthreads();
+    const int slot2 = (fc & 1) * 32 + (slot >> 1);
+#pragma unroll
+    for (int i = 0; i < 2; ++i)
+#pragma unroll
+      for (int g = 0; g < 4; ++g) {
+        const float4 m4 = *reinterpret_cast<const float4*>(mu + r0 + 32 * i + 8 * g);
+        const float mv[4] = {m4.x, m4.y, m4.z, m4.w};
+#pragma unroll
+        for (int u = 0; u < 4; ++u) {
+          const float d0 = acc[i][0][4 * g + u] - mv[u], d1 = acc[i][1][4 * g + u] - mv[u];
+          float r = d0 + d1, q = d0 * d0 + d1 * d1;
+          r += __shfl_xor(r, 1, 64);
+          q += __shfl_xor(q, 1, 64);
+          part[(r0 + 32 * i + 8 * g + u) * 64 + slot2] = (fc & 1) ? q : r;
+        }
+      }
+    __syncthreads();
+    if (tid < 128 && m0 + tid < M) {
+      float sr[2] = {0.f, 0.f}, sq[2] = {0.f, 0.f};
+#pragma unroll 8
+      for (int k = 0; k < 32; ++k) {
+        sr[k & 1] += part[tid * 64 + ((k + tid) & 31)];
+        sq[k & 1] += part[tid * 64 + 32 + ((k + tid) & 31)];
+      }
+      const float lo = (sr[0] + sr[1]) * (1.f / 128.f);
+      const int bi = n0 / p.OHW, t = (n0 - bi * p.OHW) >> 7, T = p.OHW >> 7;
+      float* o = p.part + (((long)bi * p.Cout + m0 + tid) * T + t) * 3;
+      o[0] = mean;
+      o[1] = lo;
+      o[2] = __fmaf_rn(-128.f * lo, lo, sq[0] + sq[1]);
     }
   }
 };
@@ -476,7 +541,7 @@
         if (d[u]) *d[u] = old[u] + p.alpha * acc[e0 + u];
     }
   }
-  __device__ void finish(const ConvP&, unsigned char*, int) {}
+  template <class ACC> __device__ void finish(const ConvP&, unsigned char*, int, ACC&, int, int) {}
 };
 struct EpWgrad {
   float* slab; int tap;
@@ -498,7 +563,7 @@
   __device__ void preload(const ConvP&, int, int, int, int, int, int) {}
   __device__ void stage(unsigned char*, int) {}
   __device__ void init(const ConvP& p, int, int zs) { slab = p.part + (long)zs * p.part_stride; Nn = p.N * p.HW; }
-  __device__ void finish(const ConvP&, unsigned char*, int) {}
+  template <class ACC> __device__ void finish(const ConvP&, unsigned char*, int, ACC&, int, int) {}
   __device__ void col(const ConvP&, int) {}
   __device__ void strip(const ConvP&, int mbase, int M, bool nok, int n, const floatx16& acc) {
 #pragma unroll
@@ -964,11 +1029,28 @@
   if (g.p.taps == 9) split_gemm_taps<E, 9>(g);
   else split_gemm_taps<E, 1>(g);
 }
+void split_gemm_mom(const SplitGemm& g) {
+  using E = EpFwdMom;
+  if (g.halo) {
+    if (g.p.W == 64)
+      hipLaunchKernelGGL((x2d::gemm_halo_kernel<64, E, 1>), g.grid, dim3(256), 0, g.s, g.p, g.q, g.M, g.Ng, g.tm, g.tn, g.nch / 9, g.xpart, g.nx);
+    else if (g.p.W == 32)
+      hipLaunchKernelGGL((x2d::gemm_halo_kernel<32, E, 1>), g.grid, dim3(256), 0, g.s, g.p, g.q, g.M, g.Ng, g.tm, g.tn, g.nch / 9, g.xpart, g.nx);
+    else
+      hipLaunchKernelGGL((x2d::gemm_halo_kernel<16, E, 1>), g.grid, dim3(256), 0, g.s, g.p, g.q, g.M, g.Ng, g.tm, g.tn, g.nch / 9, g.xpart, g.nx);
+  } else if (g.p.taps == 9) {
+    hipLaunchKernelGGL((x2d::gemm_kernel<9, 128, E>), g.grid, dim3(256), 0, g.s, g.p, g.q, g.M, g.Ng, g.tm, g.tn, g.nch,
+                       g.chunks_per_split, g.xpart, g.nx);
+  } else {
+    hipLaunchKernelGGL((x2d::gemm_kernel<1, 128, E>), g.grid, dim3(256), 0, g.s, g.p, g.q, g.M, g.Ng, g.tm, g.tn, g.nch,
+                       g.chunks_per_split, g.xpart, g.nx);
+  }
+}
 
 template <class EP>
 int launch_split(ConvP p, const SplitPlan& r0, const float* s1, int S1, const float* s2, int S2, int M, long Ng, int dgrad,
                  void* ws, hipStream_t s, const void* wp_ready, float* amax, const void* planes, const float* planes_amax,
-                 bool amax_valid, bool x1) {
+                 bool amax_valid, bool x1, float* mom = nullptr) {
   x2::Src q;
   q.s1 = s1; q.s2 = S2 > 0 ? s2 : s1; q.S1 = S1; q.S2 = S2; q.Kc = S1 + S2; q.Mpad = x2::pad128(M); q.taps = p.taps;
   q.pl = static_cast<const unsigned char*>(planes); q.pl_stride = planes ? pl::plane_bytes(p.N, S1, p.HW) : 0;
@@ -1006,6 +1088,14 @@
                  dim3(), s};
   g.grid = dim3((unsigned)(g.tm * g.tn * r.splits));
   if (r0.splits == 1) {
+    if constexpr (std::is_same_v<EP, EpFwd>) {
+      if (mom) {
+        g.p.part = mom;
+        split_gemm_mom(g);
+        STK_CHECK_LAUNCH();
+        return STK_OK;
+      }
+    }
     if (x1) split_gemm<OneProduct<EP>>(g);
     else split_gemm<EP>(g);
     STK_CHECK_LAUNCH();
@@ -1486,7 +1576,8 @@
 
 static int fwd_pl_impl(const void* xpl, const float* xamax, int C, const float* w, int w_layout, const float* bias,
                        const float* temb, int temb_stride, const float* res, float out_div, float* y, int N, int H,
-                       int W, int Cout, int KH, int KW, const void* wp, void* ws, long ws_bytes, void* stream, bool f16x1) {
+                       int W, int Cout, int KH, int KW, const void* wp, void* ws, long ws_bytes, void* stream, bool f16x1,
+                       float* mom = nullptr) {
   if (!xpl || !xamax || !w || !y || out_div == 0.f || (w_layout != 0 && w_layout != 1) || (w_layout == 1 && KH != 1))
     return STK_EINVAL;
   if (!stk_conv2d_pl_ok(0, C, 0, N, H, W, Cout, KH, KW, 1, KH / 2)) return STK_EUNSUPPORTED;
@@ -1498,7 +1589,22 @@
   const SplitPlan xr = fwd_split_plan(p);
   if (!ws || ws_bytes < split_ws(xr, Cout, C, p.taps).bytes) return STK_EINVAL;
   return launch_split<EpFwd>(p, xr, nullptr, C, nullptr, 0, Cout, Ng, 0, ws, (hipStream_t)stream, wp, nullptr, xpl, xamax, false,
-                             f16x1);
+                             f16x1, mom);
+}
+
+int stk_conv2d_moments_ok(int C, int N, int H, int W, int Cout, int KH, int KW) {
+  if (H <= 0 || W <= 0 || ((long)H * W) % 128) return 0;
+  return stk_conv2d_pl_ksplit(0, C, 0, N, H, W, Cout, KH, KW) == 1 ? 1 : 0;
+}
+
+int stk_conv2d_fwd_pl_mom_f32(const void* xpl, const float* xamax, int C, const float* w, int w_layout, const float* bias,
+                              const float* temb, int temb_stride, const float* res, float out_div, float* y, int N, int H,
+                              int W, int Cout, int KH, int KW, const void* wp, void* ws, long ws_bytes, float* mom,
+                              void* stream) {
+  if (!mom) return STK_EINVAL;
+  if (!stk_conv2d_moments_ok(C, N, H, W, Cout, KH, KW)) return STK_EUNSUPPORTED;
+  return fwd_pl_impl(xpl, xamax, C, w, w_layout, bias, temb, temb_stride, res, out_div, y, N, H, W, Cout, KH, KW, wp, ws,
+                     ws_bytes, stream, false, mom);
 }
 
 int stk_conv2d_fwd_pl_f32(const void* xpl, const float* xamax, int C, const float* w, int w_layout, const float* bias,
diff --git a/soft-truncation_amd/csrc/conv_x2d.h b/soft-truncation_amd/csrc/conv_x2d.h
--- a/soft-truncation_amd/csrc/conv_x2d.h
+++ b/soft-truncation_amd/csrc/conv_x2d.h
@@ -187,7 +187,7 @@
       ep.strip(p, m0 + wm0 + i * 32 + 4 * fk, M, nok, nok ? n : 0, acc[i][j]);
     }
   }
-  ep.finish(p, lds, tid);
+  ep.finish(p, lds, tid, acc, n0, M);
 }
 
 template <int W, class EP, int NB>
@@ -352,7 +352,7 @@
       ep.strip(p, m0 + wm0 + i * 32 + 4 * fk, M, true, n, acc[i][j]);
     }
   }
-  ep.finish(p, lds, tid);
+  ep.finish(p, lds, tid, acc, n0, M);
 }
 
 inline int halo_cols(int W) { return (W == 16 || W == 32 || W == 64) ? W : 0; }
diff --git a/soft-truncation_amd/csrc/groupnorm.hip b/soft-truncation_amd/csrc/groupnorm.hip
--- a/soft-truncation_amd/csrc/groupnorm.hip
+++ b/soft-truncation_amd/csrc/groupnorm.hip
@@ -1,4 +1,5 @@
 #include "common.h"
+#include "stk_gn_moments.h"
 
 namespace {
 
@@ -837,11 +838,17 @@
 }
 
 constexpr int AP_PIX = 128;
+struct GnMom {
+  const float* m1; const float* m2;
+  float* mean_out; float* rstd_out; float* rec_out;
+  float eps, sqrt_lm1;
+};
+template <bool MOMENTS>
 __global__ __launch_bounds__(256) void gn_apply_pl_kernel(GnArgs a, const float* __restrict__ mean_in,
                                                           const float* __restrict__ rstd_in, const float* __restrict__ rec,
                                                           float* __restrict__ y, unsigned char* __restrict__ planes,
                                                           long plane_stride, float* __restrict__ xmax1,
-                                                          float* __restrict__ xmax2) {
+                                                          float* __restrict__ xmax2, GnMom mom) {
   __shared__ float t[32 * 129];
   __shared__ float xm[4];
   const int tid = threadIdx.x;
@@ -851,9 +858,56 @@
   const int cb = rest % Cb, n = rest / Cb;
   const int c0 = cb * 32, p0 = tile * AP_PIX;
   const float* src = c0 < a.C1 ? a.x1 + ((long)n * a.C1 + c0) * a.HW : a.x2 + ((long)n * a.C2 + (c0 - a.C1)) * a.HW;
+  __shared__ float chs[MOMENTS ? 96 : 1], gst[MOMENTS ? 64 : 1], bnd[MOMENTS ? 8 : 1];
+  float bound = 0.f;
+  if constexpr (MOMENTS) {
+    float gm = 0.f, bm = 0.f;
+    for (int c = tid; c < C; c += 256) { gm = fmaxf(gm, fabsf(a.gamma[c])); bm = fmaxf(bm, fabsf(a.beta[c])); }
+    gm = wave_max(gm); bm = wave_max(bm);
+    if ((tid & 63) == 0) { bnd[tid >> 6] = gm; bnd[4 + (tid >> 6)] = bm; }
+    if (tid < 32) {
+      const int ch = c0 + tid;
+      const float* m = ch < a.C1 ? mom.m1 + ((long)n * a.C1 + ch) * tiles * 3 : mom.m2 + ((long)n * a.C2 + (ch - a.C1)) * tiles * 3;
+      const float h0 = m[0];
+      float s = 0.f;
+      for (int k = 0; k < tiles; ++k) s += (m[3 * k] - h0) + m[3 * k + 1];
+      const float xc = s * (1.f / (float)tiles);
+      float q = 0.f, d2 = 0.f;
+      for (int k = 0; k < tiles; ++k) { const float d = ((m[3 * k] - h0) + m[3 * k + 1]) - xc; q += m[3 * k + 2]; d2 = __fmaf_rn(d, d, d2); }
+      chs[3 * tid] = h0;
+      chs[3 * tid + 1] = xc;
+      chs[3 * tid + 2] = __fmaf_rn((float)AP_PIX, d2, q);
+    }
+    __syncthreads();
+    if (tid < 32 / a.cpg) {
+      const float* cs = chs + 3 * tid * a.cpg;
+      const float h0 = cs[0];
+      float s = 0.f;
+      for (int k = 0; k < a.cpg; ++k) s += (cs[3 * k] - h0) + cs[3 * k + 1];
+      const float xg = s * (1.f / (float)a.cpg);
+      float q = 0.f, d2 = 0.f;
+      for (int k = 0; k < a.cpg; ++k) { const float d = ((cs[3 * k] - h0) + cs[3 * k + 1]) - xg; q += cs[3 * k + 2]; d2 = __fmaf_rn(d, d, d2); }
+      const float mean = h0 + xg;
+      const float var = __fmaf_rn((float)a.HW, d2, q) * (1.f / ((float)a.cpg * (float)a.HW));
+      const float rstd = 1.f / sqrtf(var + mom.eps);
+      gst[2 * tid] = mean; gst[2 * tid + 1] = rstd;
+      if (tile == 0) {
+        const int g = c0 / a.cpg + tid;
+        mom.mean_out[n * a.G + g] = mean;
+        mom.rstd_out[n * a.G + g] = rstd;
+      }
+    }
+    __syncthreads();
+    gm = fmaxf(fmaxf(bnd[0], bnd[1]), fmaxf(bnd[2], bnd[3]));
+    bm = fmaxf(fmaxf(bnd[4], bnd[5]), fmaxf(bnd[6], bnd[7]));
+    bound = __fmaf_rn(gm, mom.sqrt_lm1, bm) * a.keep_scale;
+    if (blockIdx.x == 0) mom.rec_out[tid] = tid == 0 ? bound : 0.f;
+  } else {
+    bound = rec[0];
+  }
   float sc = 1.f;
   {
-    const int be = (int)((__float_as_uint(rec[0]) >> 23) & 0xffu);
+    const int be = (int)((__float_as_uint(bound) >> 23) & 0xffu);
     if (be != 0) sc = __uint_as_float((unsigned)min(max(127 + 13 - (be - 127), 1), 254) << 23);
   }
   unsigned long long seed = a.seed;
@@ -866,7 +920,9 @@
     const int ch = c0 + c, px = p0 + 4 * q4;
     const float4 v = *reinterpret_cast<const float4*>(src + (long)c * a.HW + px);
     const int g = ch / a.cpg;
-    const float mean = mean_in[n * a.G + g], rstd = rstd_in[n * a.G + g];
+    float mean, rstd;
+    if constexpr (MOMENTS) { mean = gst[2 * (c / a.cpg)]; rstd = gst[2 * (c / a.cpg) + 1]; }
+    else { mean = mean_in[n * a.G + g]; rstd = rstd_in[n * a.G + g]; }
     const float ga = a.gamma[ch], be = a.beta[ch];
     float r[4] = {v.x, v.y, v.z, v.w};
     if (xmax1) amax_l = fmaxf(amax_l, fmaxf(fmaxf(fabsf(r[0]), fabsf(r[1])), fmaxf(fabsf(r[2]), fabsf(r[3]))));
@@ -1034,8 +1090,8 @@
       hipLaunchKernelGGL(gn_bound_kernel, dim3(1), dim3(256), 0, s, gamma, beta, C, sq, a.keep_scale, rec);
     }
     STK_CHECK_LAUNCH();
-    hipLaunchKernelGGL(gn_apply_pl_kernel, dim3((unsigned)((long)N * (C / 32) * (HW / AP_PIX))), dim3(256), 0, s, a, mean, rstd, rec, y,
-                       static_cast<unsigned char*>(planes), plane_stride, xmax1, xmax2);
+    hipLaunchKernelGGL(gn_apply_pl_kernel<false>, dim3((unsigned)((long)N * (C / 32) * (HW / AP_PIX))), dim3(256), 0, s, a, mean, rstd, rec, y,
+                       static_cast<unsigned char*>(planes), plane_stride, xmax1, xmax2, GnMom{});
     STK_CHECK_LAUNCH();
     return STK_OK;
   }
@@ -1064,6 +1120,40 @@
   rc = stk_gn_bound_f32(gamma, beta, C, G, HW, drop_p, rec, stream);
   if (rc) return rc;
   return stk_split_planes_f32(y, N, C, HW, rec, 256, planes, stream);
+}
+
+int stk_gn_moments_ok(int C1, int C2, int HW, int G) {
+  if (C1 <= 0 || C2 < 0 || G <= 0 || HW <= 0 || !gn_pl_2k_ok(C1, C2, HW, G)) return 0;
+  return (long)((C1 + C2) / G) * HW <= 16384 && HW / AP_PIX <= 8 ? 1 : 0;
+}
+
+long stk_gn_moments_bytes(int N, int C, int HW) {
+  if (N <= 0 || C <= 0 || HW <= 0 || HW % AP_PIX) return 0;
+  return (long)N * C * (HW / AP_PIX) * 3 * 4;
+}
+
+int stk_gn_fwd_pl_mom_f32(const float* x1, int C1, const float* mom1, const float* x2, int C2, const float* mom2,
+                          const float* gamma, const float* beta, float* y, void* planes, float* rec, float* mean,
+                          float* rstd, int N, int HW, int G, float eps, int act, float drop_p, unsigned long long seed,
+                          const unsigned long long* seed_dev, float* xmax1, float* xmax2, void* stream) {
+  if (!x1 || !mom1 || !gamma || !beta || !planes || !rec || !mean || !rstd || N <= 0 || (C2 > 0 && (!x2 || !mom2)) ||
+      drop_p < 0.f || drop_p >= 1.f || act < 0 || act > STK_ACT_ELU || (xmax2 && !xmax1) || (xmax1 && C2 > 0 && !xmax2))
+    return STK_EINVAL;
+  if (!stk_gn_moments_ok(C1, C2, HW, G)) return STK_EUNSUPPORTED;
+  const int C = C1 + C2;
+  const long plane_stride = (long)N * (C / 32) * HW * 64;
+  if (2 * plane_stride >= 0x7fffffffL || !stk_aligned16(x1) || (x2 && !stk_aligned16(x2)) || (y && !stk_aligned16(y)))
+    return STK_EUNSUPPORTED;
+  GnArgs a;
+  a.x1 = x1; a.x2 = x2; a.C1 = C1; a.C2 = C2; a.gamma = gamma; a.beta = beta;
+  a.N = N; a.HW = HW; a.G = G; a.cpg = C / G; a.act = act; a.drop_p = drop_p; a.keep_scale = 1.f / (1.f - drop_p); a.drop_thr = stk_drop_threshold(drop_p);
+  a.seed = seed; a.seed_dev = seed_dev;
+  const GnMom m = {mom1, mom2, mean, rstd, rec, eps, gn_bound_sqrt((long)a.cpg * HW)};
+  hipLaunchKernelGGL(gn_apply_pl_kernel<true>, dim3((unsigned)((long)N * (C / 32) * (HW / AP_PIX))), dim3(256), 0, (hipStream_t)stream,
+                     a, (const float*)nullptr, (const float*)nullptr, (const float*)nullptr, y, static_cast<unsigned char*>(planes),
+                     plane_stride, xmax1, xmax2, m);
+  STK_CHECK_LAUNCH();
+  return STK_OK;
 }
 
 int stk_gn_fwd_pl_fused(int C1, int C2, int HW, int G) { return gn_pl_fused_ok(C1, C2, HW, G) || gn_pl_2k_ok(C1, C2, HW, G) ? 1 : 0; }
diff --git a/soft-truncation_amd/engine/graph.py b/soft-truncation_amd/engine/graph.py
--- a/soft-truncation_amd/engine/graph.py
+++ b/soft-truncation_amd/engine/graph.py
@@ -17,7 +17,7 @@
 
 class Tensor:
   __slots__ = ('shape', 'numel', 'space', 'off', 'goff', 'needs_grad', 'name', 'seen', 'external_grad',
-               'producer', 'pl_off', 'pl_rec', 'pl_maker', 'f32_fwd', 'f32_bwd')
+               'producer', 'pl_off', 'pl_rec', 'pl_maker', 'f32_fwd', 'f32_bwd', 'mom')
 
   def __init__(self, shape, space, off, needs_grad, name):
     self.shape = tuple(int(s) for s in shape)
@@ -35,6 +35,7 @@
     self.pl_maker = None
     self.f32_fwd = True
     self.f32_bwd = True
+    self.mom = None
 
   def __repr__(self):
     return f'T({self.name}{list(self.shape)}@{self.space}+{self.off})'
@@ -179,6 +180,7 @@
     self.dy_cons = None
     self.add_from = None
     self.xmax_for = None
+    self.moments = False
 
   def _p(self, rt):
     return self.drop_p if rt.training else 0.0
@@ -189,6 +191,14 @@
     if y.pl_maker is self:
       need_f32 = y.f32_fwd or (rt.with_backward and y.f32_bwd) or not self.fused
       cv = self.xmax_for
+      if self.moments:
+        x2 = self.x2
+        rt.lib.gn_fwd_pl_mom_f32(rt.v(self.x1), self.C1, rt.v(self.x1.mom), rt.v(x2), self.C2, rt.v(x2.mom) if x2 is not None else None,
+                                 rt.v(self.gamma), rt.v(self.beta_t), rt.v(y) if need_f32 else None, rt.planes(y), rt.rec(y),
+                                 rt.v(self.mean), rt.v(self.rstd), self.N, self.HW, self.G, self.eps, self.act, self._p(rt), seed,
+                                 rt.seed_dev, rt.v(cv.amax) if cv is not None else None,
+                                 rt.v(cv.amax) + 4 * 256 if cv is not None and x2 is not None else None, rt.stream)
+        return
       if cv is not None:
         rt.lib.gn_fwd_pl_max_f32(rt.v(self.x1), self.C1, rt.v(self.x2), self.C2, rt.v(self.gamma), rt.v(self.beta_t),
                                  rt.v(y) if need_f32 else None, rt.planes(y), rt.rec(y), rt.v(self.mean), rt.v(self.rstd),
@@ -333,6 +343,7 @@
   pl_dgrad = False
   pl_wgrad = False
   x_rec_own = False
+  mom_out = None
 
   def plan_planes(self, g, lib):
     same = self.stride == 1 and self.OH == self.H and self.OW == self.W and self.pad == self.KH // 2
@@ -379,6 +390,12 @@
       if t.pl_maker is self:
         rt.make_planes(t)
       label = self._label_pl(rt.lib, 'fwd')
+      if self.mom_out is not None:
+        rt.timed(label, self.flops, rt.lib.conv2d_fwd_pl_mom_f32,
+                 rt.planes(t), rt.rec(t), self.C1, rt.v(self.w), self.w_layout, rt.v(self.bias), temb, self.temb_stride,
+                 rt.v(self.res), self.out_div, rt.v(self.y), self.N, self.H, self.W, self.Cout, self.KH, self.KW,
+                 self._wp(rt, 0), rt.ws, rt.ws_bytes, rt.v(self.mom_out), rt.stream)
+        return
       rt.timed(label + '.f16' if f16 else label, self.flops, rt.lib.conv2d_fwd_pl_f16x1 if f16 else rt.lib.conv2d_fwd_pl_f32,
                rt.planes(t), rt.rec(t), self.C1, rt.v(self.w), self.w_layout, rt.v(self.bias), temb, self.temb_stride,
                rt.v(self.res), self.out_div, rt.v(self.y), self.N, self.H, self.W, self.Cout, self.KH, self.KW,
@@ -1047,6 +1064,7 @@
           op.plan_planes(self, lib)
       self._plan_f32_copies(lib)
       self._plan_x_records(lib)
+      self._plan_gn_moments(lib)
     self._plan_shared_dy(lib)
     fold_batch = os.environ.get('STK_GN_FOLD_BATCH', '1') != '0' and hasattr(lib, 'gn_param_grad_batch')
     if hasattr(lib, 'gn_bwd_out_f32'):
@@ -1097,6 +1115,30 @@
     if found:
       self.ops.insert(0, ZeroXRecords(self.amax_block, len(self.conv_amax)))
 
+  def _plan_gn_moments(self, lib):
+    if not getattr(lib, 'has_gn_moments', False) or self.precision != 'fp32':
+      return
+
+    def capable(t):
+      P = t.producer
+      return (isinstance(P, Conv) and P.y is t and P.pl_fwd and
+              bool(int(lib.conv2d_moments_ok(P.C1, P.N, P.H, P.W, P.Cout, P.KH, P.KW))))
+
+    for gn in list(self.ops):
+      if not isinstance(gn, GroupNormAct) or gn.y.pl_maker is not gn:
+        continue
+      if not int(lib.gn_moments_ok(gn.C1, gn.C2, gn.HW, gn.G)):
+        continue
+      srcs = [t for t in (gn.x1, gn.x2) if t is not None]
+      if not all(capable(t) for t in srcs):
+        continue
+      gn.moments = True
+      for t in srcs:
+        if t.mom is None:
+          n, c = t.shape[0], t.shape[1]
+          t.mom = self.new((int(lib.gn_moments_bytes(n, c, t.numel // (n * c))) // 4,), needs_grad=False, name=t.name + '.mom')
+          t.producer.mom_out = t.mom
+
   def _grad_writers(self):
     w = {}
     for op in self.ops:
diff --git a/soft-truncation_amd/engine/lib.py b/soft-truncation_amd/engine/lib.py
--- a/soft-truncation_amd/engine/lib.py
+++ b/soft-truncation_amd/engine/lib.py
@@ -121,6 +121,15 @@
   'stk_attention_long_fwd_f32': [P, P, P, L, P, P, P, I, I, I, F, P, L, S],
   'stk_attention_long_bwd_f32': [P, P, P, L, P, P, P, P, P, P, F, P, F, P, F, L, I, I, I, F, P, L, S],
 }
+SIGNATURES_GN_MOMENTS = {
+  'stk_conv2d_moments_ok': [I, I, I, I, I, I, I],
+  'stk_gn_moments_ok': [I, I, I, I],
+  'stk_gn_moments_bytes': [I, I, I],
+  'stk_conv2d_fwd_pl_mom_f32': SIGNATURES['stk_conv2d_fwd_pl_f32'][:-1] + [P, S],
+  'stk_gn_fwd_pl_mom_f32': [P, I, P, P, I, P, P, P, P, P, P, P, P, I, I, I, F, I, F, U64, P, P, P, S],
+}
+_RESTYPE_GN_MOMENTS = {'stk_gn_moments_bytes': c_long}
+_NO_CHECK_GN_MOMENTS = {'stk_conv2d_moments_ok', 'stk_gn_moments_ok', 'stk_gn_moments_bytes'}
 _RESTYPE = {'stk_strerror': c_char_p, 'stk_backend': c_char_p, 'stk_conv2d_wgrad_ws_bytes': c_long,
             'stk_conv2d_fwd_ws_bytes': c_long, 'stk_conv2d_dgrad_ws_bytes': c_long, 'stk_gn_ws_bytes': c_long,
             'stk_conv2d_wp_bytes': c_long, 'stk_conv2d_wp_desc': c_long, 'stk_planes_bytes': c_long, 'stk_conv2d_wgrad_pl_ws_bytes': c_long}
@@ -158,6 +167,8 @@
     self.has_blocks = self._bind_optional(SIGNATURES_BLOCKS, 'include/stk_blocks.h')
     self.has_attention_long = self._bind_optional(SIGNATURES_ATTN_LONG, 'include/stk_attention_long.h',
                                                   restype=_RESTYPE_ATTN_LONG, unchecked=_NO_CHECK_ATTN_LONG)
+    self.has_gn_moments = self._bind_optional(SIGNATURES_GN_MOMENTS, 'include/stk_gn_moments.h',
+                                              restype=_RESTYPE_GN_MOMENTS, unchecked=_NO_CHECK_GN_MOMENTS)
     self.backend = self._cdll.stk_backend().decode()
     self.is_device = self.backend.startswith('hip')
 
```

Result: faster. 3536 images/s (median of 6 runs) (+1.2%).
